# cisco/thor

Hardware: AMD Instinct MI355X
Metric: encoder Mpixels/s at fixed qp, bit-exact recon vs ref (higher is better)
Workload: dtype u8

## Files before the change

### include/thor_hip.h

```cpp
#ifndef THOR_HIP_H
#define THOR_HIP_H
#include <stddef.h>
#include <stdint.h>
#ifdef __cplusplus
extern "C" {
#endif

struct thor_encoder_info;
void encode_frame_lbd(struct thor_encoder_info* encoder_info);
void encode_frame_hbd(struct thor_encoder_info* encoder_info);

typedef struct thor_hip_params {
  int width, height, qp;
  int bitdepth, input_bitdepth;
  float frame_rate;
  float lambda_coeffI, lambda_coeffP;
  float early_skip_thr;
  int enable_tb_split, enable_pb_split, max_num_ref, HQperiod;
  int num_reorder_pics, interp_ref;
  int dqpP, dqpI;
  float mqpP;
  int intra_period, intra_rdo, encoder_speed;
  int deblocking, cdef, clpf, use_block_contexts, enable_bipred;
  int cfl_intra, cfl_inter;
  int dyadic_coding;
  float lambda_coeffB, lambda_coeffB0, lambda_coeffB1, lambda_coeffB2, lambda_coeffB3;
  int dqpB, dqpB0, dqpB1, dqpB2, dqpB3;
  float mqpB, mqpB0, mqpB1, mqpB2, mqpB3;
  int max_clpf_strength;
  int log2_sb_size;
} thor_hip_params;

typedef struct thor_hip_encoder thor_hip_encoder;

int thor_hip_params_from_config(thor_hip_params* p, const char* cfg_path);

int thor_hip_params_set(thor_hip_params* p, const char* name, const char* value);

int thor_hip_params_set_sb_size(thor_hip_params* p, int log2_sb_size);

int thor_hip_device_count(void);
thor_hip_encoder* thor_hip_open(const thor_hip_params* p, int num_streams, int device);
void thor_hip_close(thor_hip_encoder* e);

int thor_hip_begin_sequence(thor_hip_encoder* e, int stream, int skip, int num_frames, int file_frames);
int thor_hip_next_frame(thor_hip_encoder* e, int stream, int* display_index);

size_t thor_hip_frame_bytes(const thor_hip_encoder* e);
int thor_hip_stage_frame(thor_hip_encoder* e, int stream, int slot, const void* yuv);
int thor_hip_stage_frame_device(thor_hip_encoder* e, int stream, int slot, const void* dev_yuv);
int thor_hip_encode_staged(thor_hip_encoder* e, const int* slots);
typedef void (*thor_hip_frames_done_fn)(void* user, int first_stream, int num_streams);
int thor_hip_encode_staged_run(thor_hip_encoder* e, int nframes, thor_hip_frames_done_fn done, void* user);
int thor_hip_last_display_index(const thor_hip_encoder* e, int stream);
int thor_hip_encode_frame(thor_hip_encoder* e, const void* const* yuv_per_stream);

size_t thor_hip_stream_bytes(const thor_hip_encoder* e, int stream);
const uint8_t* thor_hip_stream_data(const thor_hip_encoder* e, int stream);
int thor_hip_get_recon(thor_hip_encoder* e, int stream, void* yuv_out);

enum { THOR_HIP_CHROMA_PLANAR = 0, THOR_HIP_CHROMA_UV = 1, THOR_HIP_CHROMA_VU = 2 };
typedef struct thor_hip_frame_layout {
  int    size;
  int    chroma;
  int    msb_aligned;
  int    pitch_y;
  int    pitch_c;
  size_t offset_u;
  size_t offset_v;
} thor_hip_frame_layout;
size_t thor_hip_layout_bytes(const thor_hip_encoder* e, const thor_hip_frame_layout* layout);
size_t thor_hip_layout_bytes_for(int width, int height, int input_bitdepth, const thor_hip_frame_layout* layout);
int thor_hip_stage_frame_layout(thor_hip_encoder* e, int stream, int slot, const void* frame, const thor_hip_frame_layout* layout, int on_device);
int thor_hip_get_recon_layout(thor_hip_encoder* e, int stream, void* frame, const thor_hip_frame_layout* layout, int on_device);

enum { THOR_HIP_RGB_RGBA = 0, THOR_HIP_RGB_BGRA = 1, THOR_HIP_RGB_ARGB = 2, THOR_HIP_RGB_ABGR = 3, THOR_HIP_RGB_RGB = 4, THOR_HIP_RGB_BGR = 5,
       THOR_HIP_RGB_PLANAR_RGB = 6 };
enum { THOR_HIP_MATRIX_BT601 = 0, THOR_HIP_MATRIX_BT709 = 1, THOR_HIP_MATRIX_BT2020 = 2 };
typedef struct thor_hip_rgb_format {
  int    size;
  int    order;
  int    depth;
  int    msb_aligned;
  int    matrix;
  int    full_range;
  int    chroma_site;
  int    pitch;
  size_t plane_stride;
} thor_hip_rgb_format;
size_t thor_hip_rgb_bytes(const thor_hip_encoder* e, const thor_hip_rgb_format* fmt);
size_t thor_hip_rgb_bytes_for(int width, int height, const thor_hip_rgb_format* fmt);
int thor_hip_stage_frame_rgb(thor_hip_encoder* e, int stream, int slot, const void* frame, const thor_hip_rgb_format* fmt, int on_device);
int thor_hip_get_recon_rgb(thor_hip_encoder* e, int stream, void* frame, const thor_hip_rgb_format* fmt, int on_device);

void thor_hip_kernel_time(thor_hip_encoder* e, double* sb_ms, long* sb_launches, double* filter_ms);
void thor_hip_kernel_time_reset(thor_hip_encoder* e);
void thor_hip_read_stats(thor_hip_encoder* e, unsigned long long out[4], int reset);
void thor_hip_set_frame_distortion(thor_hip_encoder* e, int on);
typedef struct thor_hip_frame_stats {
  int display_index;
  int frame_type;
  int qp;
  int num_bits;
  int num_ref;
  int ref_array[4];
  int ref_frame_num[4];
  int has_sse;
  unsigned long long sse[3];
  double psnr[3];
} thor_hip_frame_stats;
int thor_hip_frame_stats_count(const thor_hip_encoder* e, int stream);
int thor_hip_get_frame_stats(const thor_hip_encoder* e, int stream, int i, thor_hip_frame_stats* out);
int thor_hip_report(const thor_hip_encoder* e, int stream, char* buf, size_t n);
int thor_hip_stat_line(const thor_hip_encoder* e, int stream, int num_frames, char* buf, size_t n);

void thor_hip_read_prof(thor_hip_encoder* e, long long out[32]);

int thor_hip_sad_batch(const uint8_t* org, int w, int h, const uint8_t* ref_plane, int plane_w, int plane_h,
                       int rstride, int bx, int by, const int* cand, int n, uint32_t* out);
int thor_hip_interp_luma(const uint8_t* ref_plane, int plane_w, int plane_h, int rstride, int pad, int bx, int by,
                         int w, int h, const int16_t* mv, int n, int bipred, uint8_t* out);
int thor_hip_code_tu_batch(const uint8_t* org, const uint8_t* pred, int size, int qp, int coeff_type, int fast, int n,
                           int16_t* coefq, uint8_t* rec, int* cbp);
typedef struct thor_hip_cell {
  int16_t mv0x, mv0y, mv1x, mv1y;
  uint8_t mode, size, tbpb, cbp;
  int8_t ref0, ref1, dir;
  uint8_t pad;
} thor_hip_cell;
int thor_hip_deblock_frame(uint8_t* yuv, int width, int height, int qp, const thor_hip_cell* cells);

int thor_hip_sad_batch_hbd(const uint16_t* org, int w, int h, const uint16_t* ref_plane, int plane_w, int plane_h,
                           int rstride, int bx, int by, const int* cand, int n, uint32_t* out);
int thor_hip_interp_luma_hbd(const uint16_t* ref_plane, int plane_w, int plane_h, int rstride, int pad, int bx, int by,
                             int w, int h, const int16_t* mv, int n, int bipred, int bitdepth, uint16_t* out);
int thor_hip_code_tu_batch_hbd(const uint16_t* org, const uint16_t* pred, int size, int qp, int coeff_type, int fast, int n,
                               int bitdepth, int16_t* coefq, uint16_t* rec, int* cbp);
int thor_hip_deblock_frame_hbd(uint16_t* yuv, int width, int height, int qp, int bitdepth, const thor_hip_cell* cells);

int thor_hip_kat_intra(const void* plane, int width, int height, int stride, int bitdepth, int size, int tb_split, int n, const int* par,
                       const void* rblocks, void* out);
int thor_hip_kat_inter_yuv(const void* yuv, int width, int height, int bitdepth, int size, int n, const int* par, const int16_t* mv, void* out);
int thor_hip_kat_average(const void* a, const void* b, int size, int bitdepth, int n, void* out);
int thor_hip_kat_cfl(const void* y, void* uv, const void* ry, int n_luma, int bitdepth, int n);
int thor_hip_kat_cdef_dir(const void* blocks, int bitdepth, int n, int* dir, int* var);
int thor_hip_kat_cdef_filter(const void* plane, int width, int height, int stride, int bitdepth, int bsize, int n, const int* par, void* out);
int thor_hip_kat_cdef_frame(int n_jobs, const void* rec_yuv, const void* org_yuv, const uint8_t* mode, int width, int height, int bitdepth, const int* qp,
                            const int* speed, const int* cdef_bits, int8_t* dir, int* var, int* fb_compact, unsigned long long* mse, int* result, int* fb_sel, void* out_yuv);
int thor_hip_kat_clpf(const void* rec_yuv, const void* org_yuv, int width, int height, int bitdepth, int qp, const thor_hip_cell* cells,
                      const int* strength, int fb_log2, const uint8_t* fb_on, uint32_t* stats, void* out_yuv);
int thor_hip_kat_interpolate(const void* yuv0, const void* yuv1, int width, int height, int bitdepth, void* out_yuv);

int thor_hip_kat_motion_estimate(const void* cur, const void* ref, int width, int height, int bitdepth, int n, const int* par, const double* lambda,
                                 const int16_t* cand, int ncand_total, int* out);
int thor_hip_kat_motion_estimate_bi(const void* cur, const void* ref0, const void* ref1, int width, int height, int bitdepth, int n, const int* par,
                                    const double* lambda, const int16_t* cand, int* out, int16_t* list_out);
int thor_hip_kat_early_skip(const int* chroma, const void* org, const void* pred, const int* size, const int* qp, const float* thr, int bitdepth, int n, int* out);
int thor_hip_kat_block_ctx(const thor_hip_cell* cells, long long ncells, int cell_stride, int n, const int* par, int* out);
int thor_hip_kat_lds_block(void);
int thor_hip_kat_block_cost(int n, const int* par, const double* lambda, const void* org, const void* rec, long long nsamp, int bitdepth, unsigned long long* out);
int thor_hip_kat_intra_search(int n, const int* par, const void* plane, int width, int height, const void* org, long long nsamp, int bitdepth, int* out);
int thor_hip_kat_build_org8(int n, const int* par, const void* org, const void* pred, long long nsamp, int bitdepth, void* out_global, void* out_lds);
int thor_hip_kat_coeff_syntax(int n, const int* par, const int16_t* coef, int words, uint32_t* buf_single, uint32_t* buf_team, int* out);
int thor_hip_kat_block_syntax(int n, const int* par, const int16_t* pool, int npool, int words, uint32_t* buf_coop, uint32_t* buf_single, int* out);
int thor_hip_kat_gather_bits(int n, const uint32_t* src, int src_words, const int* src_off, const int* nbits, const long long* dst_bit, uint32_t* dst, int dst_words);

int thor_hip_frame_sse(const void* a, const void* b, int w, int h, int bitdepth, unsigned long long out[3]);
int thor_hip_kat_depth_up(const void* in, int w, int h, int bitdepth, int input_bitdepth, uint16_t* out);
int thor_hip_kat_depth_down(const uint16_t* in, int w, int h, int bitdepth, int input_bitdepth, void* out);
int thor_hip_frame_sse_depth(const void* a, const void* b, int w, int h, int bitdepth, int input_bitdepth, unsigned long long out[3]);
int thor_hip_kat_layout_in(const void* src, const thor_hip_frame_layout* layout, int w, int h, int input_bitdepth, int bitdepth, void* planar_out);
int thor_hip_kat_layout_out(const void* planar_in, const thor_hip_frame_layout* layout, int w, int h, int input_bitdepth, int bitdepth, void* dst);
int thor_hip_kat_rgb_in(const void* src, const thor_hip_rgb_format* fmt, int w, int h, int input_bitdepth, int bitdepth, void* planar_out);
int thor_hip_kat_rgb_out(const void* planar_in, const thor_hip_rgb_format* fmt, int w, int h, int input_bitdepth, int bitdepth, void* dst);

int thor_hip_superblock_kernel_info(int sample_bytes, int* num_regs, int* lds_bytes, int* private_bytes, int* workgroups_per_cu);
int thor_hip_superblock_kernel_in_use(void);

#ifdef __cplusplus
}
#endif
#endif
```

### thor_amd/binding.py

```python
import ctypes as C
import os
import subprocess
import numpy as np

REPO_ROOT = os.path.dirname(os.path.dirname(os.path.abspath(__file__)))
_LIB = None


def lib_path():
    return os.environ.get('THOR_HIP_LIB') or os.path.join(REPO_ROOT, 'thor_amd', 'libthor_hip.so')


HIPCC_FLAGS = ['--offload-arch=gfx950', '-O3', '-std=c++17', '-ffp-contract=off', '-fno-strict-aliasing', '-fPIC', '-pthread']
NATIVE_SOURCES = ['thor_hip.cpp', 'thor_hip_lat.cpp', 'thor_hip_wide.cpp', 'thor_hip_katbits.cpp']


def build_native(force=False):
    csrc = os.path.join(REPO_ROOT, 'thor_amd', 'csrc')
    out = os.path.join(REPO_ROOT, 'thor_amd', 'libthor_hip.so')
    hdrs = [os.path.join(csrc, f) for f in os.listdir(csrc)]
    hdrs += [os.path.join(REPO_ROOT, 'include', f) for f in os.listdir(os.path.join(REPO_ROOT, 'include'))]
    newest = max(os.path.getmtime(h) for h in hdrs)
    if force or not os.path.exists(out) or os.path.getmtime(out) < newest:
        hipcc = '/opt/rocm/bin/hipcc' if os.path.exists('/opt/rocm/bin/hipcc') else 'hipcc'
        import tempfile
        with tempfile.TemporaryDirectory() as d:
            objs = [os.path.join(d, f[:-4] + '.o') for f in NATIVE_SOURCES]
            procs = [subprocess.Popen([hipcc] + HIPCC_FLAGS + ['-c', '-o', o, os.path.join(csrc, f)]) for f, o in zip(NATIVE_SOURCES, objs)]
            rcs = [p.wait() for p in procs]
            if any(rcs):
                raise subprocess.CalledProcessError(max(rcs), 'hipcc -c ' + ' '.join(NATIVE_SOURCES))
            subprocess.check_call([hipcc, '--offload-arch=gfx950', '-shared', '-pthread', '-o', out] + objs)
    tool = os.path.join(REPO_ROOT, 'tools', 'thorenc_hip')
    tsrc = tool + '.c'
    if force or not os.path.exists(tool) or os.path.getmtime(tool) < os.path.getmtime(tsrc):
        subprocess.check_call(['gcc', '-O2', '-std=c99', '-D_POSIX_C_SOURCE=200809L', '-o', tool, tsrc,
                               '-L' + os.path.join(REPO_ROOT, 'thor_amd'), '-lthor_hip', '-Wl,-rpath,$ORIGIN/../thor_amd'])
    return out


class ThorParams(C.Structure):
    _fields_ = [('width', C.c_int), ('height', C.c_int), ('qp', C.c_int), ('bitdepth', C.c_int), ('input_bitdepth', C.c_int),
                ('frame_rate', C.c_float), ('lambda_coeffI', C.c_float), ('lambda_coeffP', C.c_float),
                ('early_skip_thr', C.c_float), ('enable_tb_split', C.c_int), ('enable_pb_split', C.c_int),
                ('max_num_ref', C.c_int), ('HQperiod', C.c_int), ('num_reorder_pics', C.c_int), ('interp_ref', C.c_int),
                ('dqpP', C.c_int), ('dqpI', C.c_int), ('mqpP', C.c_float), ('intra_period', C.c_int), ('intra_rdo', C.c_int),
                ('encoder_speed', C.c_int), ('deblocking', C.c_int), ('cdef', C.c_int), ('clpf', C.c_int),
                ('use_block_contexts', C.c_int), ('enable_bipred', C.c_int), ('cfl_intra', C.c_int), ('cfl_inter', C.c_int),
                ('dyadic_coding', C.c_int), ('lambda_coeffB', C.c_float), ('lambda_coeffB0', C.c_float), ('lambda_coeffB1', C.c_float),
                ('lambda_coeffB2', C.c_float), ('lambda_coeffB3', C.c_float), ('dqpB', C.c_int), ('dqpB0', C.c_int), ('dqpB1', C.c_int),
                ('dqpB2', C.c_int), ('dqpB3', C.c_int), ('mqpB', C.c_float), ('mqpB0', C.c_float), ('mqpB1', C.c_float),
                ('mqpB2', C.c_float), ('mqpB3', C.c_float), ('max_clpf_strength', C.c_int), ('log2_sb_size', C.c_int)]


FRAMES_DONE_FN = C.CFUNCTYPE(None, C.c_void_p, C.c_int, C.c_int)


class FrameStats(C.Structure):
    _fields_ = [('display_index', C.c_int), ('frame_type', C.c_int), ('qp', C.c_int), ('num_bits', C.c_int), ('num_ref', C.c_int),
                ('ref_array', C.c_int * 4), ('ref_frame_num', C.c_int * 4), ('has_sse', C.c_int), ('sse', C.c_ulonglong * 3),
                ('psnr', C.c_double * 3)]


CHROMA_PLANAR, CHROMA_UV, CHROMA_VU = 0, 1, 2


class FrameLayout(C.Structure):
    _fields_ = [('size', C.c_int), ('chroma', C.c_int), ('msb_aligned', C.c_int), ('pitch_y', C.c_int), ('pitch_c', C.c_int),
                ('offset_u', C.c_size_t), ('offset_v', C.c_size_t)]

    def __init__(self, chroma=CHROMA_PLANAR, msb_aligned=0, pitch_y=0, pitch_c=0, offset_u=0, offset_v=0):
        super().__init__(C.sizeof(FrameLayout), chroma, msb_aligned, pitch_y, pitch_c, offset_u, offset_v)

    @classmethod
    def planar(cls, pitch_y=0, pitch_c=0, offset_u=0, offset_v=0, msb_aligned=0):
        return cls(CHROMA_PLANAR, msb_aligned, pitch_y, pitch_c, offset_u, offset_v)

    @classmethod
    def nv12(cls, pitch=None, offset_uv=0):
        return cls(CHROMA_UV, 0, pitch or 0, pitch or 0, offset_uv)

    @classmethod
    def nv21(cls, pitch=None, offset_vu=0):
        return cls(CHROMA_VU, 0, pitch or 0, pitch or 0, offset_vu)

    @classmethod
    def p010(cls, pitch=None, offset_uv=0):
        return cls(CHROMA_UV, 1, pitch or 0, pitch or 0, offset_uv)


RGB_RGBA, RGB_BGRA, RGB_ARGB, RGB_ABGR, RGB_RGB, RGB_BGR, RGB_PLANAR = range(7)
MATRIX_BT601, MATRIX_BT709, MATRIX_BT2020 = 0, 1, 2


class RgbFormat(C.Structure):
    _fields_ = [('size', C.c_int), ('order', C.c_int), ('depth', C.c_int), ('msb_aligned', C.c_int), ('matrix', C.c_int), ('full_range', C.c_int),
                ('chroma_site', C.c_int), ('pitch', C.c_int), ('plane_stride', C.c_size_t)]

    def __init__(self, order=RGB_RGBA, depth=8, msb_aligned=0, matrix=MATRIX_BT709, full_range=0, chroma_site=1, pitch=0, plane_stride=0):
        super().__init__(C.sizeof(RgbFormat), order, depth, msb_aligned, matrix, full_range, chroma_site, pitch, plane_stride)

    @classmethod
    def rgba(cls, depth=8, matrix=MATRIX_BT709, full_range=0, chroma_site=1, pitch=0, msb_aligned=0):
        return cls(RGB_RGBA, depth, msb_aligned, matrix, full_range, chroma_site, pitch)

    @classmethod
    def bgra(cls, depth=8, matrix=MATRIX_BT709, full_range=0, chroma_site=1, pitch=0, msb_aligned=0):
        return cls(RGB_BGRA, depth, msb_aligned, matrix, full_range, chroma_site, pitch)

    @classmethod
    def rgb24(cls, depth=8, matrix=MATRIX_BT709, full_range=0, chroma_site=1, pitch=0, msb_aligned=0):
        return cls(RGB_RGB, depth, msb_aligned, matrix, full_range, chroma_site, pitch)

    @classmethod
    def bgr24(cls, depth=8, matrix=MATRIX_BT709, full_range=0, chroma_site=1, pitch=0, msb_aligned=0):
        return cls(RGB_BGR, depth, msb_aligned, matrix, full_range, chroma_site, pitch)

    @classmethod
    def planar(cls, depth=8, matrix=MATRIX_BT709, full_range=0, chroma_site=1, pitch=0, msb_aligned=0, plane_stride=0):
        return cls(RGB_PLANAR, depth, msb_aligned, matrix, full_range, chroma_site, pitch, plane_stride)


def lib():
    global _LIB
    if _LIB is None:
        p = lib_path()
        if not os.path.exists(p):
            raise RuntimeError(f'{p} is missing: run __graft_entry__.build() (hipcc --offload-arch=gfx950); there is no CPU path')
        L = C.CDLL(p)
        L.thor_hip_open.restype = C.c_void_p
        L.thor_hip_open.argtypes = [C.POINTER(ThorParams), C.c_int, C.c_int]
        L.thor_hip_close.argtypes = [C.c_void_p]
        L.thor_hip_begin_sequence.argtypes = [C.c_void_p, C.c_int, C.c_int, C.c_int, C.c_int]
        L.thor_hip_next_frame.argtypes = [C.c_void_p, C.c_int, C.POINTER(C.c_int)]
        L.thor_hip_stage_frame.argtypes = [C.c_void_p, C.c_int, C.c_int, C.c_void_p]
        L.thor_hip_stage_frame_device.argtypes = [C.c_void_p, C.c_int, C.c_int, C.c_void_p]
        L.thor_hip_encode_staged.argtypes = [C.c_void_p, C.POINTER(C.c_int)]
        L.thor_hip_encode_frame.argtypes = [C.c_void_p, C.POINTER(C.c_void_p)]
        L.thor_hip_encode_staged_run.argtypes = [C.c_void_p, C.c_int, FRAMES_DONE_FN, C.c_void_p]
        L.thor_hip_last_display_index.argtypes = [C.c_void_p, C.c_int]
        L.thor_hip_stream_bytes.restype = C.c_size_t
        L.thor_hip_stream_bytes.argtypes = [C.c_void_p, C.c_int]
        L.thor_hip_stream_data.restype = C.c_void_p
        L.thor_hip_stream_data.argtypes = [C.c_void_p, C.c_int]
        L.thor_hip_get_recon.argtypes = [C.c_void_p, C.c_int, C.c_void_p]
        L.thor_hip_frame_bytes.restype = C.c_size_t
        L.thor_hip_frame_bytes.argtypes = [C.c_void_p]
        L.thor_hip_kernel_time.argtypes = [C.c_void_p, C.POINTER(C.c_double), C.POINTER(C.c_long), C.POINTER(C.c_double)]
        L.thor_hip_kernel_time_reset.argtypes = [C.c_void_p]
        L.thor_hip_read_stats.argtypes = [C.c_void_p, C.POINTER(C.c_ulonglong), C.c_int]
        L.thor_hip_deblock_frame.argtypes = [C.c_void_p, C.c_int, C.c_int, C.c_int, C.c_void_p]
        L.thor_hip_deblock_frame_hbd.argtypes = [C.c_void_p, C.c_int, C.c_int, C.c_int, C.c_int, C.c_void_p]
        L.thor_hip_set_frame_distortion.argtypes = [C.c_void_p, C.c_int]
        L.thor_hip_frame_stats_count.argtypes = [C.c_void_p, C.c_int]
        L.thor_hip_get_frame_stats.argtypes = [C.c_void_p, C.c_int, C.c_int, C.POINTER(FrameStats)]
        L.thor_hip_report.argtypes = [C.c_void_p, C.c_int, C.c_char_p, C.c_size_t]
        L.thor_hip_stat_line.argtypes = [C.c_void_p, C.c_int, C.c_int, C.c_char_p, C.c_size_t]
        L.thor_hip_frame_sse.argtypes = [C.c_void_p, C.c_void_p, C.c_int, C.c_int, C.c_int, C.POINTER(C.c_ulonglong)]
        L.thor_hip_kat_depth_up.argtypes = [C.c_void_p, C.c_int, C.c_int, C.c_int, C.c_int, C.c_void_p]
        L.thor_hip_kat_depth_down.argtypes = [C.c_void_p, C.c_int, C.c_int, C.c_int, C.c_int, C.c_void_p]
        L.thor_hip_frame_sse_depth.argtypes = [C.c_void_p, C.c_void_p, C.c_int, C.c_int, C.c_int, C.c_int, C.POINTER(C.c_ulonglong)]
        LP = C.POINTER(FrameLayout)
        L.thor_hip_layout_bytes.restype = C.c_size_t
        L.thor_hip_layout_bytes.argtypes = [C.c_void_p, LP]
        L.thor_hip_layout_bytes_for.restype = C.c_size_t
        L.thor_hip_layout_bytes_for.argtypes = [C.c_int, C.c_int, C.c_int, LP]
        L.thor_hip_stage_frame_layout.argtypes = [C.c_void_p, C.c_int, C.c_int, C.c_void_p, LP, C.c_int]
        L.thor_hip_get_recon_layout.argtypes = [C.c_void_p, C.c_int, C.c_void_p, LP, C.c_int]
        L.thor_hip_kat_layout_in.argtypes = [C.c_void_p, LP, C.c_int, C.c_int, C.c_int, C.c_int, C.c_void_p]
        L.thor_hip_kat_layout_out.argtypes = [C.c_void_p, LP, C.c_int, C.c_int, C.c_int, C.c_int, C.c_void_p]
        RP = C.POINTER(RgbFormat)
        L.thor_hip_rgb_bytes.restype = C.c_size_t
        L.thor_hip_rgb_bytes.argtypes = [C.c_void_p, RP]
        L.thor_hip_rgb_bytes_for.restype = C.c_size_t
        L.thor_hip_rgb_bytes_for.argtypes = [C.c_int, C.c_int, RP]
        L.thor_hip_stage_frame_rgb.argtypes = [C.c_void_p, C.c_int, C.c_int, C.c_void_p, RP, C.c_int]
        L.thor_hip_get_recon_rgb.argtypes = [C.c_void_p, C.c_int, C.c_void_p, RP, C.c_int]
        L.thor_hip_kat_rgb_in.argtypes = [C.c_void_p, RP, C.c_int, C.c_int, C.c_int, C.c_int, C.c_void_p]
        L.thor_hip_kat_rgb_out.argtypes = [C.c_void_p, RP, C.c_int, C.c_int, C.c_int, C.c_int, C.c_void_p]
        L.thor_hip_params_from_config.argtypes = [C.POINTER(ThorParams), C.c_char_p]
        L.thor_hip_params_set.argtypes = [C.POINTER(ThorParams), C.c_char_p, C.c_char_p]
        L.thor_hip_params_set_sb_size.argtypes = [C.POINTER(ThorParams), C.c_int]
        _LIB = L
    return _LIB


def load_config(cfg_path=None, **overrides):
    p = ThorParams()
    rc = lib().thor_hip_params_from_config(C.byref(p), cfg_path.encode() if cfg_path else None)
    if rc:
        raise ValueError(f'{cfg_path}: unknown or unsupported option (rc={rc}); this path rejects what it cannot encode bit-exactly')
    for k, v in overrides.items():
        if k == 'log2_sb_size':
            rc = lib().thor_hip_params_set_sb_size(C.byref(p), int(v))
        else:
            rc = lib().thor_hip_params_set(C.byref(p), ('-' + k).encode(), str(v).encode())
        if rc:
            raise ValueError(f'option -{k} {v}: ' + {1: 'unknown', 2: 'not implemented by this path', 3: 'front-end option, not an encoder parameter'}.get(rc, f'rc={rc}'))
    return p


class Encoder:

    def __init__(self, params, num_streams=1, device=0):
        self.p = params
        self.S = num_streams
        self.h = lib().thor_hip_open(C.byref(params), num_streams, device)
        if not self.h:
            raise RuntimeError('thor_hip_open failed (unsupported parameters?)')
        self.dtype = _pix(params.input_bitdepth)
        self.sample_bytes = self.dtype().itemsize
        self.frame_bytes = lib().thor_hip_frame_bytes(self.h)

    def close(self):
        if self.h:
            lib().thor_hip_close(self.h)
            self.h = None

    def layout_bytes(self, layout):
        n = lib().thor_hip_layout_bytes(self.h, C.byref(layout))
        if not n:
            raise ValueError('frame layout refused (pitch below the row, pitch or offset no multiple of the sample size, msb_aligned with 8-bit input ...)')
        return n

    def stage(self, stream, slot, frame, layout=None):
        frame = np.ascontiguousarray(frame).view(np.uint8)
        if layout is not None:
            assert frame.size >= self.layout_bytes(layout)
            rc = lib().thor_hip_stage_frame_layout(self.h, stream, slot, frame.ctypes.data_as(C.c_void_p), C.byref(layout), 0)
            if rc:
                raise RuntimeError(f'thor_hip_stage_frame_layout rc={rc}')
            return
        assert frame.size == self.frame_bytes
        rc = lib().thor_hip_stage_frame(self.h, stream, slot, frame.ctypes.data_as(C.c_void_p))
        if rc:
            raise RuntimeError(f'thor_hip_stage_frame rc={rc}')

    def stage_device(self, stream, slot, dev_ptr, layout=None):
        if layout is not None:
            rc = lib().thor_hip_stage_frame_layout(self.h, stream, slot, C.c_void_p(dev_ptr), C.byref(layout), 1)
            if rc:
                raise RuntimeError(f'thor_hip_stage_frame_layout rc={rc}')
            return
        rc = lib().thor_hip_stage_frame_device(self.h, stream, slot, C.c_void_p(dev_ptr))
        if rc:
            raise RuntimeError(f'thor_hip_stage_frame_device rc={rc}')

    def rgb_bytes(self, fmt):
        n = lib().thor_hip_rgb_bytes(self.h, C.byref(fmt))
        if not n:
            raise ValueError('RGB format refused (unknown order / depth / matrix, msb_aligned with depth 8 or 16, pitch below the row ...)')
        return n

    def stage_rgb(self, stream, slot, array, fmt):
        frame = np.ascontiguousarray(array).view(np.uint8).reshape(-1)
        assert frame.size >= self.rgb_bytes(fmt)
        rc = lib().thor_hip_stage_frame_rgb(self.h, stream, slot, frame.ctypes.data_as(C.c_void_p), C.byref(fmt), 0)
        if rc:
            raise RuntimeError(f'thor_hip_stage_frame_rgb rc={rc}')

    def stage_rgb_device(self, stream, slot, dev_ptr, fmt):
        rc = lib().thor_hip_stage_frame_rgb(self.h, stream, slot, C.c_void_p(dev_ptr), C.byref(fmt), 1)
        if rc:
            raise RuntimeError(f'thor_hip_stage_frame_rgb rc={rc}')

    def recon_rgb(self, stream, fmt):
        out = np.zeros(self.rgb_bytes(fmt), dtype=np.uint8)
        rc = lib().thor_hip_get_recon_rgb(self.h, stream, out.ctypes.data_as(C.c_void_p), C.byref(fmt), 0)
        if rc:
            raise RuntimeError(f'thor_hip_get_recon_rgb rc={rc}')
        return out

    def recon_rgb_device(self, stream, dev_ptr, fmt):
        rc = lib().thor_hip_get_recon_rgb(self.h, stream, C.c_void_p(dev_ptr), C.byref(fmt), 1)
        if rc:
            raise RuntimeError(f'thor_hip_get_recon_rgb rc={rc}')

    def begin_sequence(self, stream, skip, num_frames, file_frames):
        rc = lib().thor_hip_begin_sequence(self.h, stream, skip, num_frames, file_frames)
        if rc:
            raise RuntimeError(f'thor_hip_begin_sequence rc={rc}')

    def next_frame(self, stream):
        d = C.c_int()
        return d.value if lib().thor_hip_next_frame(self.h, stream, C.byref(d)) else None

    def encode_run(self, nframes, on_done=None):
        err = []

        def _cb(_user, first, count):
            if on_done is not None and not err:
                try:
                    on_done(first, count)
                except BaseException as e:
                    err.append(e)
        cb = FRAMES_DONE_FN(_cb)
        rc = lib().thor_hip_encode_staged_run(self.h, nframes, cb, None)
        if err:
            raise err[0]
        if rc:
            raise RuntimeError(f'thor_hip_encode_staged_run rc={rc}')

    def last_display_index(self, stream):
        return lib().thor_hip_last_display_index(self.h, stream)

    def encode_clips(self, clips, want_recon=True, skips=None, file_frames=None, staggered=False):
        n = len(clips[0])
        for s in range(self.S):
            for f in range(n):
                self.stage(s, f, clips[s][f])
            sk = skips[s] if skips else 0
            self.begin_sequence(s, sk, n, file_frames if file_frames else sk + n)
        recs = [[None] * n for _ in range(self.S)]
        if staggered:
            def done(first, count):
                if want_recon:
                    for s in range(first, first + count):
                        recs[s][self.last_display_index(s)] = self.recon(s)
            self.encode_run(n, done)
            return [self.bitstream(s) for s in range(self.S)], recs
        while True:
            idx = [self.next_frame(s) for s in range(self.S)]
            if idx[0] is None:
                break
            self.encode_staged(idx)
            if want_recon:
                for s in range(self.S):
                    recs[s][idx[s]] = self.recon(s)
        return [self.bitstream(s) for s in range(self.S)], recs

    def encode_staged(self, slots):
        arr = (C.c_int * self.S)(*slots)
        rc = lib().thor_hip_encode_staged(self.h, arr)
        if rc:
            raise RuntimeError(f'thor_hip_encode_staged rc={rc}')

    def bitstream(self, stream):
        n = lib().thor_hip_stream_bytes(self.h, stream)
        return C.string_at(lib().thor_hip_stream_data(self.h, stream), n)

    def recon(self, stream, layout=None):
        if layout is not None:
            out = np.zeros(self.layout_bytes(layout), dtype=np.uint8)
            rc = lib().thor_hip_get_recon_layout(self.h, stream, out.ctypes.data_as(C.c_void_p), C.byref(layout), 0)
            if rc:
                raise RuntimeError(f'thor_hip_get_recon_layout rc={rc}')
            return out
        out = np.empty(self.frame_bytes, dtype=np.uint8)
        rc = lib().thor_hip_get_recon(self.h, stream, out.ctypes.data_as(C.c_void_p))
        if rc:
            raise RuntimeError(f'thor_hip_get_recon rc={rc}')
        return out

    def recon_device(self, stream, dev_ptr, layout):
        rc = lib().thor_hip_get_recon_layout(self.h, stream, C.c_void_p(dev_ptr), C.byref(layout), 1)
        if rc:
            raise RuntimeError(f'thor_hip_get_recon_layout rc={rc}')

    def recon_into(self, stream, ptr):
        rc = lib().thor_hip_get_recon(self.h, stream, C.c_void_p(ptr))
        if rc:
            raise RuntimeError(f'thor_hip_get_recon rc={rc}')

    def kernel_time(self):
        a, b, c = C.c_double(), C.c_long(), C.c_double()
        lib().thor_hip_kernel_time(self.h, C.byref(a), C.byref(b), C.byref(c))
        return a.value, b.value, c.value

    def kernel_time_reset(self):
        lib().thor_hip_kernel_time_reset(self.h)
        self.stats(reset=True)

    def stats(self, reset=False):
        a = (C.c_ulonglong * 4)()
        lib().thor_hip_read_stats(self.h, a, 1 if reset else 0)
        px, sb = max(int(a[3]), 1), max(int(a[2]), 1)
        return {'early_skip_pixel_fraction': round(int(a[0]) / px, 4), 'early_skip_sb128_fraction': round(int(a[1]) / sb, 4),
                'inter_superblocks': int(a[2]), 'inter_luma_pixels': int(a[3])}

    def set_frame_distortion(self, on=True):
        lib().thor_hip_set_frame_distortion(self.h, 1 if on else 0)

    def frame_stats(self, stream):
        L, out, f = lib(), [], FrameStats()
        for i in range(L.thor_hip_frame_stats_count(self.h, stream)):
            if L.thor_hip_get_frame_stats(self.h, stream, i, C.byref(f)):
                raise RuntimeError('thor_hip_get_frame_stats failed')
            nr = f.num_ref
            out.append({'display_index': f.display_index, 'type': 'IPB'[f.frame_type], 'qp': f.qp, 'num_bits': f.num_bits,
                        'ref_array': list(f.ref_array)[:nr], 'ref_frame_num': list(f.ref_frame_num)[:nr], 'has_sse': bool(f.has_sse),
                        'sse': [int(v) for v in f.sse], 'psnr': [float(v) for v in f.psnr]})
        return out

    def report(self, stream):
        n = lib().thor_hip_report(self.h, stream, None, 0)
        if n < 0:
            raise ValueError('bad stream')
        buf = C.create_string_buffer(n + 1)
        lib().thor_hip_report(self.h, stream, buf, n + 1)
        return buf.value.decode()

    def __enter__(self):
        return self

    def __exit__(self, *a):
        self.close()


def _vp(a):
    return a.ctypes.data_as(C.c_void_p)


def _pix(bitdepth):
    return np.uint16 if bitdepth > 8 else np.uint8


def sad_batch(org, ref_plane, bx, by, cand, bitdepth=8):
    T = _pix(bitdepth)
    org = np.ascontiguousarray(org, dtype=T); ref_plane = np.ascontiguousarray(ref_plane, dtype=T)
    cand = np.ascontiguousarray(cand, dtype=np.int32)
    out = np.zeros(len(cand), dtype=np.uint32)
    fn = lib().thor_hip_sad_batch_hbd if bitdepth > 8 else lib().thor_hip_sad_batch
    rc = fn(_vp(org), org.shape[1], org.shape[0], _vp(ref_plane), ref_plane.shape[1], ref_plane.shape[0], ref_plane.shape[1], bx, by,
            _vp(cand), len(cand), _vp(out))
    if rc:
        raise RuntimeError(f'thor_hip_sad_batch rc={rc}')
    return out


def interp_luma(ref_padded, pad, pic_w, pic_h, bx, by, w, h, mvs, bipred, bitdepth=8):
    T = _pix(bitdepth)
    ref_padded = np.ascontiguousarray(ref_padded, dtype=T); mvs = np.ascontiguousarray(mvs, dtype=np.int16)
    out = np.zeros((len(mvs), h, w), dtype=T)
    if bitdepth > 8:
        rc = lib().thor_hip_interp_luma_hbd(_vp(ref_padded), pic_w, pic_h, ref_padded.shape[1], pad, bx, by, w, h, _vp(mvs), len(mvs),
                                            bipred, bitdepth, _vp(out))
    else:
        rc = lib().thor_hip_interp_luma(_vp(ref_padded), pic_w, pic_h, ref_padded.shape[1], pad, bx, by, w, h, _vp(mvs), len(mvs),
                                        bipred, _vp(out))
    if rc:
        raise RuntimeError(f'thor_hip_interp_luma rc={rc}')
    return out


def code_tu_batch(org, pred, qp, coeff_type, fast, bitdepth=8):
    T = _pix(bitdepth)
    org = np.ascontiguousarray(org, dtype=T); pred = np.ascontiguousarray(pred, dtype=T)
    n, size = org.shape[0], org.shape[1]
    q = min(size, 16)
    coefq = np.zeros((n, q, q), dtype=np.int16); rec = np.zeros_like(org); cbp = np.zeros(n, dtype=np.int32)
    if bitdepth > 8:
        rc = lib().thor_hip_code_tu_batch_hbd(_vp(org), _vp(pred), size, qp, coeff_type, fast, n, bitdepth, _vp(coefq), _vp(rec), _vp(cbp))
    else:
        rc = lib().thor_hip_code_tu_batch(_vp(org), _vp(pred), size, qp, coeff_type, fast, n, _vp(coefq), _vp(rec), _vp(cbp))
    if rc:
        raise RuntimeError(f'thor_hip_code_tu_batch rc={rc}')
    return coefq, rec, cbp


def deblock_frame(yuv, width, height, qp, cells, bitdepth=8):
    yuv = np.ascontiguousarray(yuv, dtype=_pix(bitdepth)).copy()
    cells = np.ascontiguousarray(cells, dtype=np.uint8)
    assert yuv.size == width * height * 3 // 2 and cells.size == (width // 4) * (height // 4) * 16
    if bitdepth > 8:
        rc = lib().thor_hip_deblock_frame_hbd(_vp(yuv), width, height, qp, bitdepth, _vp(cells))
    else:
        rc = lib().thor_hip_deblock_frame(_vp(yuv), width, height, qp, _vp(cells))
    if rc:
        raise RuntimeError(f'thor_hip_deblock_frame rc={rc}')
    return yuv


def _kat(name, *args):
    fn = getattr(lib(), name)
    fn.restype = C.c_int
    rc = fn(*args)
    if rc:
        raise RuntimeError(f'{name} rc={rc}')


def kat_intra(plane, size, par, bitdepth=8, rblocks=None):
    T = _pix(bitdepth)
    plane = np.ascontiguousarray(plane, dtype=T); par = np.ascontiguousarray(par, dtype=np.int32)
    n = len(par)
    out = np.zeros((n, size, size), dtype=T)
    rb = np.ascontiguousarray(rblocks, dtype=T) if rblocks is not None else None
    _kat('thor_hip_kat_intra', _vp(plane), plane.shape[1], plane.shape[0], plane.shape[1], bitdepth, size, 1 if rb is not None else 0, n, _vp(par),
         _vp(rb) if rb is not None else None, _vp(out))
    return out


def kat_inter_yuv(yuv, width, height, size, par, mvs, bitdepth=8):
    T = _pix(bitdepth)
    yuv = np.ascontiguousarray(yuv, dtype=T); par = np.ascontiguousarray(par, dtype=np.int32); mvs = np.ascontiguousarray(mvs, dtype=np.int16)
    n = len(par)
    out = np.zeros((n, size * size * 3 // 2), dtype=T)
    _kat('thor_hip_kat_inter_yuv', _vp(yuv), width, height, bitdepth, size, n, _vp(par), _vp(mvs), _vp(out))
    return out


def kat_average(a, b, size, bitdepth=8):
    T = _pix(bitdepth)
    a = np.ascontiguousarray(a, dtype=T); b = np.ascontiguousarray(b, dtype=T)
    out = np.zeros_like(a)
    _kat('thor_hip_kat_average', _vp(a), _vp(b), size, bitdepth, len(a), _vp(out))
    return out


def kat_cfl(y, uv, ry, n_luma, bitdepth=8):
    T = _pix(bitdepth)
    y = np.ascontiguousarray(y, dtype=T); ry = np.ascontiguousarray(ry, dtype=T); uv = np.array(uv, dtype=T, order='C')
    _kat('thor_hip_kat_cfl', _vp(y), _vp(uv), _vp(ry), n_luma, bitdepth, len(y))
    return uv


def kat_cdef_dir(blocks, bitdepth=8):
    T = _pix(bitdepth)
    blocks = np.ascontiguousarray(blocks, dtype=T)
    n = len(blocks)
    d = np.zeros(n, dtype=np.int32); v = np.zeros(n, dtype=np.int32)
    _kat('thor_hip_kat_cdef_dir', _vp(blocks), bitdepth, n, _vp(d), _vp(v))
    return d, v


def kat_cdef_filter(plane, bsize, par, bitdepth=8):
    T = _pix(bitdepth)
    plane = np.ascontiguousarray(plane, dtype=T); par = np.ascontiguousarray(par, dtype=np.int32)
    out = np.zeros((len(par), bsize, bsize), dtype=T)
    _kat('thor_hip_kat_cdef_filter', _vp(plane), plane.shape[1], plane.shape[0], plane.shape[1], bitdepth, bsize, len(par), _vp(par), _vp(out))
    return out


def kat_cdef_frame(rec, org, mode, width, height, qp, speed, cdef_bits, bitdepth=8):
    T = _pix(bitdepth)
    rec = np.ascontiguousarray(rec, dtype=T); org = np.ascontiguousarray(org, dtype=T); mode = np.ascontiguousarray(mode, dtype=np.uint8)
    S = len(rec)
    nfb = ((width + 63) // 64) * ((height + 63) // 64)
    qp, speed, cdef_bits = (np.ascontiguousarray(a, dtype=np.int32) for a in (qp, speed, cdef_bits))
    assert rec.shape == org.shape == (S, width * height * 3 // 2) and mode.shape == (S, height // 4, width // 4) and len(qp) == len(speed) == len(cdef_bits) == S
    d = np.zeros((S, height // 8, width // 8), dtype=np.int8); v = np.zeros((S, height // 8, width // 8), dtype=np.int32)
    fbc = np.zeros((S, nfb), dtype=np.int32); fbs = np.zeros((S, nfb), dtype=np.int32)
    mse = np.zeros((S, 2, nfb, 64), dtype=np.uint64); res = np.zeros((S, 34), dtype=np.int32)
    out = np.zeros_like(rec)
    _kat('thor_hip_kat_cdef_frame', S, _vp(rec), _vp(org), _vp(mode), width, height, bitdepth, _vp(qp), _vp(speed), _vp(cdef_bits), _vp(d), _vp(v), _vp(fbc), _vp(mse), _vp(res), _vp(fbs),
         _vp(out))
    return dict(dir=d, var=v, fb_compact=fbc, fb_sel=fbs, mse=mse, nb_bits=res[:, 0], strengths=res[:, 1:9], uv_strengths=res[:, 9:17], sb_count=res[:, 17], out=out)


def kat_clpf(rec, org, width, height, qp, cells, strength, fb_log2, fb_on, bitdepth=8):
    T = _pix(bitdepth)
    rec = np.ascontiguousarray(rec, dtype=T); org = np.ascontiguousarray(org, dtype=T)
    cells = np.ascontiguousarray(cells, dtype=np.uint8); fb_on = np.ascontiguousarray(fb_on, dtype=np.uint8)
    st = np.ascontiguousarray(strength, dtype=np.int32)
    nblk = (width // 8) * (height // 8) + 2 * (width // 16) * (height // 16)
    stats = np.zeros((nblk, 4), dtype=np.uint32)
    out = np.zeros_like(rec)
    _kat('thor_hip_kat_clpf', _vp(rec), _vp(org), width, height, bitdepth, qp, _vp(cells), _vp(st), fb_log2, _vp(fb_on), _vp(stats), _vp(out))
    return stats, out


def kat_interpolate(yuv0, yuv1, width, height, bitdepth=8):
    T = _pix(bitdepth)
    a = np.ascontiguousarray(yuv0, dtype=T); b = np.ascontiguousarray(yuv1, dtype=T)
    out = np.zeros_like(a)
    _kat('thor_hip_kat_interpolate', _vp(a), _vp(b), width, height, bitdepth, _vp(out))
    return out


def kat_motion_estimate(cur, ref, par, lam, cand, bitdepth=8):
    T = _pix(bitdepth)
    cur = np.ascontiguousarray(cur, dtype=T); ref = np.ascontiguousarray(ref, dtype=T)
    par = np.ascontiguousarray(par, dtype=np.int32); lam = np.ascontiguousarray(lam, dtype=np.float64); cand = np.ascontiguousarray(cand, dtype=np.int16).reshape(-1, 2)
    assert cur.shape == ref.shape and par.shape[1] == 17 and len(lam) == len(par)
    out = np.full((len(par), 3), -1, dtype=np.int32)
    _kat('thor_hip_kat_motion_estimate', _vp(cur), _vp(ref), cur.shape[1], cur.shape[0], bitdepth, len(par), _vp(par), _vp(lam), _vp(cand), len(cand), _vp(out))
    return out


def kat_motion_estimate_bi(cur, ref0, ref1, par, lam, cand, bitdepth=8):
    T = _pix(bitdepth)
    cur, ref0, ref1 = (np.ascontiguousarray(a, dtype=T) for a in (cur, ref0, ref1))
    par = np.ascontiguousarray(par, dtype=np.int32); lam = np.ascontiguousarray(lam, dtype=np.float64); cand = np.ascontiguousarray(cand, dtype=np.int16)
    assert cur.shape == ref0.shape == ref1.shape and par.shape[1] == 17 and len(lam) == len(par) and cand.size == 12 * len(par)
    out = np.full((len(par), 3), -1, dtype=np.int32)
    lists = np.zeros((len(par), 6, 2), dtype=np.int16)
    _kat('thor_hip_kat_motion_estimate_bi', _vp(cur), _vp(ref0), _vp(ref1), cur.shape[1], cur.shape[0], bitdepth, len(par), _vp(par), _vp(lam), _vp(cand), _vp(out), _vp(lists))
    return out, lists


def kat_early_skip(chroma, org, pred, size, qp, thr, bitdepth=8):
    T = _pix(bitdepth)
    org = np.ascontiguousarray(org, dtype=T); pred = np.ascontiguousarray(pred, dtype=T)
    chroma, size, qp = (np.ascontiguousarray(a, dtype=np.int32) for a in (chroma, size, qp))
    thr = np.ascontiguousarray(thr, dtype=np.float32)
    n = len(org)
    assert org.shape == pred.shape == (n, 32, 32) and len(chroma) == len(size) == len(qp) == len(thr) == n
    out = np.full(n, -1, dtype=np.int32)
    _kat('thor_hip_kat_early_skip', _vp(chroma), _vp(org), _vp(pred), _vp(size), _vp(qp), _vp(thr), bitdepth, n, _vp(out))
    return out


def kat_block_ctx(cells, cell_stride, par):
    cells = np.ascontiguousarray(cells, dtype=np.uint8); par = np.ascontiguousarray(par, dtype=np.int32)
    assert cells.ndim == 2 and cells.shape[1] == 16 and par.ndim == 2 and par.shape[1] == 6
    out = np.full((len(par), 23), -77, dtype=np.int32)
    _kat('thor_hip_kat_block_ctx', _vp(cells), C.c_longlong(len(cells)), cell_stride, len(par), _vp(par), _vp(out))
    return out


def kat_lds_block():
    fn = lib().thor_hip_kat_lds_block
    fn.restype = C.c_int
    return fn()


def kat_block_cost(par, lam, org, rec, bitdepth=8):
    T = _pix(bitdepth)
    org = np.ascontiguousarray(org, dtype=T).ravel(); rec = np.ascontiguousarray(rec, dtype=T).ravel()
    par = np.ascontiguousarray(par, dtype=np.int32); lam = np.ascontiguousarray(lam, dtype=np.float64)
    assert par.ndim == 2 and par.shape[1] == 7 and len(lam) == len(par) and len(org) == len(rec)
    out = np.zeros((len(par), 4), dtype=np.uint64)
    _kat('thor_hip_kat_block_cost', len(par), _vp(par), _vp(lam), _vp(org), _vp(rec), C.c_longlong(len(org)), bitdepth, _vp(out))
    return out


def kat_intra_search(par, plane, org, bitdepth=8):
    T = _pix(bitdepth)
    plane = np.ascontiguousarray(plane, dtype=T); org = np.ascontiguousarray(org, dtype=T).ravel()
    par = np.ascontiguousarray(par, dtype=np.int32)
    assert plane.ndim == 2 and par.ndim == 2 and par.shape[1] == 6
    out = np.full((len(par), 2), -77, dtype=np.int32)
    _kat('thor_hip_kat_intra_search', len(par), _vp(par), _vp(plane), plane.shape[1], plane.shape[0], _vp(org), C.c_longlong(len(org)), bitdepth, _vp(out))
    return out


def kat_build_org8(par, org, pred, bitdepth=8, fill=0):
    T = _pix(bitdepth)
    org = np.ascontiguousarray(org, dtype=T).ravel(); pred = np.ascontiguousarray(pred, dtype=T).ravel()
    par = np.ascontiguousarray(par, dtype=np.int32)
    assert par.ndim == 2 and par.shape[1] == 4 and len(org) == len(pred)
    og = np.full(len(org), fill, dtype=T); ol = np.full(len(org), fill, dtype=T)
    _kat('thor_hip_kat_build_org8', len(par), _vp(par), _vp(org), _vp(pred), C.c_longlong(len(org)), bitdepth, _vp(og), _vp(ol))
    return og, ol


def kat_coeff_syntax(par, coef, words, buf_single, buf_team):
    par = np.ascontiguousarray(par, dtype=np.int32); coef = np.ascontiguousarray(coef, dtype=np.int16)
    n = len(par)
    b1 = np.ascontiguousarray(buf_single, dtype=np.uint32).copy(); bt = np.ascontiguousarray(buf_team, dtype=np.uint32).copy()
    assert par.shape == (n, 4) and coef.shape == (n, 256) and b1.shape == (n, words) and bt.shape == (n, words)
    out = np.zeros((n, 6), dtype=np.int32)
    _kat('thor_hip_kat_coeff_syntax', n, _vp(par), _vp(coef), words, _vp(b1), _vp(bt), _vp(out))
    return out, b1, bt


def kat_block_syntax(par, pool, words, fill=0):
    par = np.ascontiguousarray(par, dtype=np.int32); pool = np.ascontiguousarray(pool, dtype=np.int16)
    n = len(par)
    assert par.shape == (n, 57) and pool.ndim == 2 and pool.shape[1] == 256
    bc = np.full((n, words), fill, dtype=np.uint32); b1 = np.full((n, words), fill, dtype=np.uint32)
    out = np.zeros((n, 10), dtype=np.int32)
    _kat('thor_hip_kat_block_syntax', n, _vp(par), _vp(pool), len(pool), words, _vp(bc), _vp(b1), _vp(out))
    return out, bc, b1


def kat_gather_bits(src, src_off, nbits, dst_bit, dst_words):
    src = np.ascontiguousarray(src, dtype=np.uint32); src_off = np.ascontiguousarray(src_off, dtype=np.int32)
    nbits = np.ascontiguousarray(nbits, dtype=np.int32); dst_bit = np.ascontiguousarray(dst_bit, dtype=np.int64)
    dst = np.zeros(dst_words, dtype=np.uint32)
    _kat('thor_hip_kat_gather_bits', len(nbits), _vp(src), len(src), _vp(src_off), _vp(nbits), _vp(dst_bit), _vp(dst), dst_words)
    return dst


def frame_sse(a, b, width, height, bitdepth=8):
    T = _pix(bitdepth)
    a = np.ascontiguousarray(a, dtype=T).reshape(-1); b = np.ascontiguousarray(b, dtype=T).reshape(-1)
    if a.size != width * height * 3 // 2 or b.size != a.size:
        raise ValueError('frame size does not match width x height 4:2:0')
    out = (C.c_ulonglong * 3)()
    rc = lib().thor_hip_frame_sse(_vp(a), _vp(b), width, height, bitdepth, out)
    if rc:
        raise RuntimeError(f'thor_hip_frame_sse returned {rc}')
    return [int(v) for v in out]


def _depth_frame(a, depth, width, height):
    a = np.ascontiguousarray(a, dtype=_pix(depth)).reshape(-1)
    if a.size != width * height * 3 // 2:
        raise ValueError('frame size does not match width x height 4:2:0')
    return a


def kat_depth_up(frame, width, height, bitdepth, input_bitdepth):
    a = _depth_frame(frame, input_bitdepth, width, height)
    out = np.zeros(a.size, dtype=np.uint16)
    _kat('thor_hip_kat_depth_up', _vp(a), width, height, bitdepth, input_bitdepth, _vp(out))
    return out


def kat_depth_down(frame, width, height, bitdepth, input_bitdepth):
    a = _depth_frame(frame, 16, width, height)
    out = np.zeros(a.size, dtype=_pix(input_bitdepth))
    _kat('thor_hip_kat_depth_down', _vp(a), width, height, bitdepth, input_bitdepth, _vp(out))
    return out


def frame_sse_depth(a, b, width, height, bitdepth, input_bitdepth):
    T = 16 if bitdepth > input_bitdepth else bitdepth
    a = _depth_frame(a, T, width, height); b = _depth_frame(b, T, width, height)
    out = (C.c_ulonglong * 3)()
    _kat('thor_hip_frame_sse_depth', _vp(a), _vp(b), width, height, bitdepth, input_bitdepth, out)
    return [int(v) for v in out]


def layout_bytes(layout, width, height, input_bitdepth):
    return lib().thor_hip_layout_bytes_for(width, height, input_bitdepth, C.byref(layout))


def kat_layout_in(src, layout, width, height, input_bitdepth, bitdepth):
    assert src.dtype == np.uint8 and src.flags.c_contiguous and src.size >= layout_bytes(layout, width, height, input_bitdepth) > 0
    out = np.zeros(width * height * 3 // 2, dtype=_pix(bitdepth))
    _kat('thor_hip_kat_layout_in', _vp(src), C.byref(layout), width, height, input_bitdepth, bitdepth, _vp(out))
    return out


def kat_layout_out(planar, layout, width, height, input_bitdepth, bitdepth, dst):
    a = _depth_frame(planar, bitdepth, width, height)
    assert dst.dtype == np.uint8 and dst.flags.c_contiguous and dst.size == layout_bytes(layout, width, height, input_bitdepth) + 64 > 64
    _kat('thor_hip_kat_layout_out', _vp(a), C.byref(layout), width, height, input_bitdepth, bitdepth, _vp(dst))
    return dst


def rgb_bytes(fmt, width, height):
    return lib().thor_hip_rgb_bytes_for(width, height, C.byref(fmt))


def kat_rgb_in(src, fmt, width, height, input_bitdepth, bitdepth):
    assert src.dtype == np.uint8 and src.flags.c_contiguous and src.size >= rgb_bytes(fmt, width, height) > 0
    out = np.zeros(width * height * 3 // 2, dtype=_pix(bitdepth))
    _kat('thor_hip_kat_rgb_in', _vp(src), C.byref(fmt), width, height, input_bitdepth, bitdepth, _vp(out))
    return out


def kat_rgb_out(planar, fmt, width, height, input_bitdepth, bitdepth, dst):
    a = _depth_frame(planar, bitdepth, width, height)
    assert dst.dtype == np.uint8 and dst.flags.c_contiguous and dst.size == rgb_bytes(fmt, width, height) + 64 > 64
    _kat('thor_hip_kat_rgb_out', _vp(a), C.byref(fmt), width, height, input_bitdepth, bitdepth, _vp(dst))
    return dst
```

### thor_amd/csrc/hip_kat_block.h

```cpp
#pragma once
#include "tk_kat_block.h"
namespace tk {
__global__ __launch_bounds__(64) void k_kat_block_ctx(const DbCell* cells, int cs, const int* par, int* out) {
  const int it = (int)blockIdx.x;
  int o[kKatCtxOut];
  kat_ctx_item(cells, cs, par + kKatCtxPar * it, o);
  if (threadIdx.x == 0)
    for (int k = 0; k < kKatCtxOut; k++) out[(size_t)kKatCtxOut * it + k] = o[k];
}
template <typename PIX>
__global__ __launch_bounds__(kWgThreads, (sizeof(PIX) == 1 ? (int)kOcc : 2)) void k_kat_block_cost(const int* par, const double* lam, const int* lay, const PIX* orgp, const PIX* recp,
                                                                                                   int bitdepth, unsigned char* big, unsigned long long* out) {
  __shared__ FrameJob<PIX> sJ;
  __shared__ WgShared sh;
  __shared__ SmallWs<PIX> sws;
  __shared__ TeamWs<PIX> s_view;
  const int lane = (int)threadIdx.x, it = (int)blockIdx.x;
  const Team t = mk_team(lane, 64, sh.tabs.izz);
  const int* q = par + kKatCostPar * it;
  const int size = __builtin_amdgcn_readfirstlane(q[0]), bw = __builtin_amdgcn_readfirstlane(q[1]), bh = __builtin_amdgcn_readfirstlane(q[2]);
  const int nbits = __builtin_amdgcn_readfirstlane(q[3]), off = __builtin_amdgcn_readfirstlane(q[4]), sy = __builtin_amdgcn_readfirstlane(q[6]);
  const int n = size * size, c = n >> 2, sc = size >> 1;
  const PIX* gy = orgp + lay[3 * it];
  const PIX* gu = orgp + lay[3 * it + 1];
  const PIX* gv = orgp + lay[3 * it + 2];
  const PIX* ry = recp + off;
  const int lds_blk = size <= kLdsBlk;
  TeamWs<PIX> w = make_ws(&sws, &sh, (BigWs<PIX>*)big);
  ws_select(&w, size);
  if (lds_blk) {
    PIX* ob = (PIX*)sh.org_raw;
    for (int k = lane; k < bw * bh; k += 64) ob[(k / bw) * size + k % bw] = gy[(k / bw) * sy + k % bw];
    for (int k = lane; k < (bw >> 1) * (bh >> 1); k += 64) {
      const int i = k / (bw >> 1), j = k % (bw >> 1);
      ob[n + i * sc + j] = gu[i * (sy >> 1) + j];
      ob[n + c + i * sc + j] = gv[i * (sy >> 1) + j];
    }
    for (int k = lane; k < n; k += 64) w.rec_y[k] = ry[k];
    for (int k = lane; k < c; k += 64) { w.rec_u[k] = ry[n + k]; w.rec_v[k] = ry[n + c + k]; }
    w.org_y = ob; w.org_u = ob + n; w.org_v = ob + n + c; w.org_sy = size; w.org_sc = sc;
  } else {
    w.rec_y = const_cast<PIX*>(ry); w.rec_u = const_cast<PIX*>(ry) + n; w.rec_v = const_cast<PIX*>(ry) + n + c;
    w.org_y = gy; w.org_u = gu; w.org_v = gv; w.org_sy = sy; w.org_sc = sy >> 1;
  }
  lds_st(&s_view, w);
  if (lane == 0) {
    sJ.cfg.bitdepth = bitdepth;
    sh.stack[0].size = size; sh.stack[0].bw = bw; sh.stack[0].bh = bh;
  }
  __syncthreads();
  WsP<PIX> ws = ldsc(&s_view);
  JobR<PIX> J = *ldsc(&sJ);
  const double lambda = lam[it];
  const unsigned long long ssd_g = ssd_total(t, ssd_part<SP_GLOBAL>(t, gy, sy, ry, size, bw, bh));
  unsigned long long ssd_l = ~0ull, cost, cost_y;
  if (lds_blk) {
    ssd_l = ssd_total(t, ssd_part<SP_LDS>(t, w.org_y, size, w.rec_y, size, bw, bh));
    cost = rd_cost<PIX, SP_LDS>(t, J, ws, sh.stack[0], nbits, lambda);
    cost_y = rd_cost<PIX, SP_LDS>(t, J, ws, sh.stack[0], nbits, lambda, (long long)ssd_l);
  } else {
    cost = rd_cost<PIX, SP_GLOBAL>(t, J, ws, sh.stack[0], nbits, lambda);
    cost_y = rd_cost<PIX, SP_GLOBAL>(t, J, ws, sh.stack[0], nbits, lambda, (long long)ssd_g);
  }
  if (lane == 0) {
    unsigned long long* o = out + (size_t)kKatCostOut * it;
    o[0] = ssd_g; o[1] = ssd_l; o[2] = cost; o[3] = cost_y;
  }
}
template <typename PIX>
__global__ __launch_bounds__(kWgThreads, (sizeof(PIX) == 1 ? (int)kOcc : 2)) void k_kat_intra_search(const int* par, const int* slot, const PIX* plane, int fw, int fh, int bitdepth,
                                                                                                     const PIX* orgp, unsigned char* big, int* out) {
  __shared__ FrameJob<PIX> sJ;
  __shared__ WgShared sh;
  __shared__ SmallWs<PIX> sws;
  __shared__ TeamWs<PIX> s_view;
  const int lane = (int)threadIdx.x, it = (int)blockIdx.x;
  const Team t = mk_team(lane, 64, sh.tabs.izz);
  const int* q = par + kKatIntraPar * it;
  const int ypos = __builtin_amdgcn_readfirstlane(q[0]), xpos = __builtin_amdgcn_readfirstlane(q[1]), size = __builtin_amdgcn_readfirstlane(q[2]);
  const int sb = __builtin_amdgcn_readfirstlane(q[3]), nm = __builtin_amdgcn_readfirstlane(q[4]), off = __builtin_amdgcn_readfirstlane(q[5]);
  const PIX* go = orgp + off;
  const int lds_blk = size <= kLdsBlk;
  TeamWs<PIX> w = make_ws(&sws, &sh, (BigWs<PIX>*)big + __builtin_amdgcn_readfirstlane(slot[it]));
  ws_select(&w, size);
  if (lds_blk) {
    PIX* ob = (PIX*)sh.org_raw;
    for (int k = lane; k < size * size; k += 64) ob[k] = go[k];
    w.org_y = ob;
  } else {
    w.org_y = go;
  }
  w.org_sy = size;
  lds_st(&s_view, w);
  if (lane == 0) {
    sJ.cfg.width = fw; sJ.cfg.height = fh; sJ.cfg.bitdepth = bitdepth; sJ.cfg.sb_shift = sb == kMaxSb ? 0 : 1;
    sJ.rec.y = const_cast<PIX*>(plane); sJ.rec.sy = fw;
    sh.stack[0].size = size; sh.stack[0].ypos = ypos; sh.stack[0].xpos = xpos; sh.stack[0].bw = size; sh.stack[0].bh = size;
  }
  __syncthreads();
  WsP<PIX> ws = ldsc(&s_view);
  JobR<PIX> J = *ldsc(&sJ);
  int mode = -1;
  const unsigned sad = lds_blk ? intra_sad_search<PIX, SP_LDS>(t, J, ws, sh.stack[0], nm, &mode) : intra_sad_search<PIX, SP_GLOBAL>(t, J, ws, sh.stack[0], nm, &mode);
  if (lane == 0) { out[kKatIntraOut * it] = mode; out[kKatIntraOut * it + 1] = (int)sad; }
}
template <typename PIX>
__global__ __launch_bounds__(64) void k_kat_build_org8(const int* par, const int* lay, const PIX* orgp, const PIX* predp, int bitdepth, unsigned char* big, PIX* outg, PIX* outl) {
  __shared__ WgShared sh;
  __shared__ SmallWs<PIX> sws;
  const int lane = (int)threadIdx.x, it = (int)blockIdx.x;
  const Team t = mk_team(lane, 64, sh.tabs.izz);
  const int* q = par + kKatOrg8Par * it;
  const int size = __builtin_amdgcn_readfirstlane(q[0]), off = __builtin_amdgcn_readfirstlane(q[1]), sy = __builtin_amdgcn_readfirstlane(q[3]);
  const int n = size * size;
  const PIX* gy = orgp + lay[it];
  const PIX* gp = predp + off;
  build_org8<PIX, SP_GLOBAL>(t, outg + off, gy, sy, gp, size, bitdepth);
  if (size <= kLdsBlk) {
    TeamWs<PIX> w = make_ws(&sws, &sh, (BigWs<PIX>*)big);
    ws_select(&w, size);
    PIX* ob = (PIX*)sh.org_raw;
    for (int k = lane; k < n; k += 64) { ob[k] = gy[(k / size) * sy + k % size]; w.pred_y[k] = gp[k]; }
    __syncthreads();
    build_org8<PIX, SP_LDS>(t, w.org8, ob, size, w.pred_y, size, bitdepth);
    __syncthreads();
    for (int k = lane; k < n; k += 64) outl[off + k] = w.org8[k];
  }
}
}

namespace {
template <typename PIX>
int kat_intra_search(int n, const int* par, const PIX* plane, int fw, int fh, const PIX* org, long long nsamp, int bitdepth, int* out) {
  if (n <= 0 || n > 4096 || !par || !plane || !org || !out || fw < 8 || fh < 8 || fw > 4096 || fh > 4096 || fw % 8 || fh % 8 || nsamp <= 0 || nsamp > (1ll << 30)) return 1;
  std::vector<int> slot(n, 0);
  int nbig = 0;
  for (int i = 0; i < n; i++) {
    if (int r = kat_intra_check(par + kKatIntraPar * i, fw, fh, nsamp)) return r;
    if (par[kKatIntraPar * i + 2] > kLdsBlk) slot[i] = nbig++;
  }
  if (!ensure_init_any()) return 3;
  DevBuf<int> d_par((size_t)kKatIntraPar * n, par), d_slot(n, slot.data()), d_o((size_t)kKatIntraOut * n);
  DevBuf<PIX> d_plane((size_t)fw * fh, plane), d_org((size_t)nsamp, org);
  DevBuf<unsigned char> d_big(sizeof(BigWs<PIX>) * (size_t)(nbig > 0 ? nbig : 1));
  hipLaunchKernelGGL(k_kat_intra_search<PIX>, dim3(n), dim3(64), 0, g_stream, d_par, d_slot, d_plane, fw, fh, bitdepth, d_org, d_big, d_o);
  HIPCHECK(hipGetLastError());
  backend::d2h(out, d_o, (size_t)kKatIntraOut * n * 4);
  return 0;
}
template <typename PIX>
int kat_build_org8(int n, const int* par, const PIX* org, const PIX* pred, long long nsamp, int bitdepth, PIX* outg, PIX* outl) {
  const int S = (int)sizeof(PIX);
  if (n <= 0 || !par || !org || !pred || !outg || !outl || nsamp <= 0 || nsamp > (1ll << 28)) return 1;
  for (int i = 0; i < n; i++)
    if (int r = kat_org8_check(par + kKatOrg8Par * i, nsamp, S)) return r;
  std::vector<PIX> planes;
  std::vector<int> lay(n);
  for (int i = 0; i < n; i++) {
    const int* q = par + kKatOrg8Par * i;
    const int size = q[0], sk = q[2] / S, st = q[3];
    const size_t base = (planes.size() * S + 15) / 16 * 16 / S;
    planes.resize(base + sk + (size_t)(size - 1) * st + size, (PIX)0);
    lay[i] = (int)(base + sk);
    for (int r = 0; r < size; r++) memcpy(&planes[base + sk + (size_t)r * st], org + q[1] + (size_t)r * size, (size_t)size * S);
  }
  if (planes.size() > (1u << 30)) return 2;
  if (!ensure_init_any()) return 3;
  DevBuf<int> d_par((size_t)kKatOrg8Par * n, par), d_lay(n, lay.data());
  DevBuf<PIX> d_org(planes.size(), planes.data()), d_pred((size_t)nsamp, pred), d_g((size_t)nsamp, outg), d_l((size_t)nsamp, outl);
  DevBuf<unsigned char> d_big(sizeof(BigWs<PIX>));
  hipLaunchKernelGGL(k_kat_build_org8<PIX>, dim3(n), dim3(64), 0, g_stream, d_par, d_lay, d_org, d_pred, bitdepth, d_big, d_g, d_l);
  HIPCHECK(hipGetLastError());
  backend::d2h(outg, d_g, (size_t)nsamp * S);
  backend::d2h(outl, d_l, (size_t)nsamp * S);
  return 0;
}
template <typename PIX>
int kat_block_cost(int n, const int* par, const double* lambda, const PIX* org, const PIX* rec, long long nsamp, int bitdepth, unsigned long long* out) {
  const int S = (int)sizeof(PIX);
  if (n <= 0 || !par || !lambda || !org || !rec || !out || nsamp <= 0 || nsamp > (1ll << 30)) return 1;
  for (int i = 0; i < n; i++)
    if (int r = kat_cost_check(par + kKatCostPar * i, lambda[i], nsamp, S)) return r;
  std::vector<PIX> planes;
  std::vector<int> lay((size_t)3 * n);
  for (int i = 0; i < n; i++) {
    const int* q = par + kKatCostPar * i;
    const int size = q[0], bw = q[1], bh = q[2], skew = q[5], sy = q[6];
    const PIX* src = org + q[4];
    for (int pl = 0; pl < 3; pl++) {
      const int w = pl ? bw / 2 : bw, h = pl ? bh / 2 : bh, st = pl ? sy / 2 : sy, cst = pl ? size / 2 : size;
      const int sk = (pl ? skew / 2 : skew) / S;
      const PIX* s = src + (pl == 0 ? 0 : pl == 1 ? size * size : size * size * 5 / 4);
      const size_t base = (planes.size() * S + 15) / 16 * 16 / S;
      planes.resize(base + sk + (size_t)(h - 1) * st + w, (PIX)0);
      lay[3 * i + pl] = (int)(base + sk);
      for (int r = 0; r < h; r++) memcpy(&planes[base + sk + (size_t)r * st], s + (size_t)r * cst, (size_t)w * S);
    }
  }
  if (planes.size() > (1u << 30)) return 2;
  if (!ensure_init_any()) return 3;
  DevBuf<int> d_par((size_t)kKatCostPar * n, par), d_lay((size_t)3 * n, lay.data());
  DevBuf<double> d_lam(n, lambda);
  DevBuf<PIX> d_org(planes.size(), planes.data()), d_rec((size_t)nsamp, rec);
  DevBuf<unsigned char> d_big(sizeof(BigWs<PIX>));
  DevBuf<unsigned long long> d_o((size_t)kKatCostOut * n);
  hipLaunchKernelGGL(k_kat_block_cost<PIX>, dim3(n), dim3(64), 0, g_stream, d_par, d_lam, d_lay, d_org, d_rec, bitdepth, d_big, d_o);
  HIPCHECK(hipGetLastError());
  backend::d2h(out, d_o, (size_t)kKatCostOut * n * 8);
  return 0;
}
}

extern "C" int thor_hip_kat_block_ctx(const thor_hip_cell* cells, long long ncells, int cell_stride, int n, const int* par, int* out) {
  static_assert(sizeof(thor_hip_cell) == sizeof(DbCell), "thor_hip_cell must mirror tk::DbCell");
  if (!cells || !par || !out || n <= 0 || ncells <= 0 || ncells > (1ll << 26) || cell_stride < 2 || cell_stride > 2048) return 1;
  for (int i = 0; i < n; i++) {
    if (par[kKatCtxPar * i + 3] != 4 * cell_stride) return 1;
    if (int r = kat_ctx_check(par + kKatCtxPar * i, ncells)) return r;
  }
  if (!ensure_init_any()) return 3;
  const size_t pad = (size_t)cell_stride + 1;
  DevBuf<DbCell> d_cells(pad + (size_t)ncells);
  backend::h2d(d_cells.get() + pad, cells, (size_t)ncells * sizeof(DbCell));
  DevBuf<int> d_par((size_t)kKatCtxPar * n, par), d_o((size_t)kKatCtxOut * n);
  hipLaunchKernelGGL(k_kat_block_ctx, dim3(n), dim3(64), 0, g_stream, d_cells.get() + pad, cell_stride, d_par, d_o);
  HIPCHECK(hipGetLastError());
  backend::d2h(out, d_o, (size_t)kKatCtxOut * n * 4);
  return 0;
}
extern "C" int thor_hip_kat_lds_block(void) { return kLdsBlk; }
extern "C" int thor_hip_kat_block_cost(int n, const int* par, const double* lambda, const void* org, const void* rec, long long nsamp, int bitdepth, unsigned long long* out) {
  KAT_BD(kat_block_cost<uint8_t>(n, par, lambda, (const uint8_t*)org, (const uint8_t*)rec, nsamp, 8, out),
         kat_block_cost<uint16_t>(n, par, lambda, (const uint16_t*)org, (const uint16_t*)rec, nsamp, bitdepth, out));
}
extern "C" int thor_hip_kat_intra_search(int n, const int* par, const void* plane, int width, int height, const void* org, long long nsamp, int bitdepth, int* out) {
  KAT_BD(kat_intra_search<uint8_t>(n, par, (const uint8_t*)plane, width, height, (const uint8_t*)org, nsamp, 8, out),
         kat_intra_search<uint16_t>(n, par, (const uint16_t*)plane, width, height, (const uint16_t*)org, nsamp, bitdepth, out));
}
extern "C" int thor_hip_kat_build_org8(int n, const int* par, const void* org, const void* pred, long long nsamp, int bitdepth, void* out_global, void* out_lds) {
  KAT_BD(kat_build_org8<uint8_t>(n, par, (const uint8_t*)org, (const uint8_t*)pred, nsamp, 8, (uint8_t*)out_global, (uint8_t*)out_lds),
         kat_build_org8<uint16_t>(n, par, (const uint16_t*)org, (const uint16_t*)pred, nsamp, bitdepth, (uint16_t*)out_global, (uint16_t*)out_lds));
}
```

### thor_amd/csrc/tk_block_queue.h

```cpp
#pragma once
#include "tk_block_md.h"

namespace tk {
TK_DEV BlkParam blank_param() {
  BlkParam p;
  p.mode = M_SKIP; p.intra_mode = 0; p.skip_idx = 0; p.pb_part = P_NONE; p.ref0 = p.ref1 = 0; p.dir = 0;
  p.tb_param = 0; p.tb_split = 0; p.cbp_y = p.cbp_u = p.cbp_v = 0;
  for (int i = 0; i < 4; i++) { p.mv0[i] = mk_mv(0, 0); p.mv1[i] = mk_mv(0, 0); }
  return p;
}

template <typename PIX, int SP>
TK_DEV void snapshot_trial(const Team t, WsP<PIX> ws, int size, const BlkParam& p) {
  BigWs<PIX>* g = ws->big;
  const int sc = size >> 1;
  copy_block<SP_GLOBAL, SP>(t, g->best_y, size, ws->rec_y, size, size, size);
  copy_block<SP_GLOBAL, SP>(t, g->best_u, sc, ws->rec_u, sc, sc, sc);
  copy_block<SP_GLOBAL, SP>(t, g->best_v, sc, ws->rec_v, sc, sc, sc);
  if (TKU(p.cbp_y) | TKU(p.cbp_u) | TKU(p.cbp_v)) {
    const int tbs = TKU(p.tb_split);
    const int qy = tbs ? tmin(size >> 1, (int)kMaxQuant) : tmin(size, (int)kMaxQuant);
    const int ny = (tbs ? 4 : 1) * qy * qy;
    const int csplit = tbs && sc > 4;
    const int qc = csplit ? tmin(sc >> 1, (int)kMaxQuant) : tmin(sc, (int)kMaxQuant);
    const int nc = (csplit ? 4 : 1) * qc * qc;
    const int16_t *cy = ws->coef_y, *cu = ws->coef_u, *cv = ws->coef_v;
    TK_GLOBAL int16_t* dy = gptr(g->best_cy);
    TK_GLOBAL int16_t* du = gptr(g->best_cu);
    TK_GLOBAL int16_t* dv = gptr(g->best_cv);
    for (int k = t.rank; k < ny; k += t.size) dy[k] = cy[k];
    for (int k = t.rank; k < nc; k += t.size) { du[k] = cu[k]; dv[k] = cv[k]; }
  }
}

template <typename PIX> struct MdCtx {
  Wg wg;
  WgShared* sh;
  Node* nd;
  unsigned long long mykey;
};

template <typename PIX, int SP>
TK_DEV int par_trial(const Team t, JobR<PIX> J, WsP<PIX> ws, MdCtx<PIX>& M, BlkParam& p, unsigned order, int reuse_pred) {
  int untouched = 0;
  const unsigned cost = rdo_trial<PIX, SP>(t, J, ws, *M.nd, p, J.lambda, reuse_pred, 0xffffffffu, &M.sh->bestkey, order, nullptr, &untouched);
  if (cost == (unsigned)kCostInit) return !untouched;
  const unsigned long long key = ((unsigned long long)cost << 32) | order;
  if (key < M.mykey) {
    M.mykey = key;
    if (t.rank == 0) {
      lds_st(&M.sh->wbest[M.wg.wave], normalize_best(*M.nd, p));
      *ldsc(&M.sh->wkey[M.wg.wave]) = key;
      wg_min64(&M.sh->bestkey, key);
    }
    snapshot_trial<PIX, SP>(t, ws, tk_uniform(ldsc(M.nd)->size), p);
    t.sync();
  }
  return 1;
}

TK_DEV void wg_wait_at_least(const Team t, int* p, int at_least) {
  const unsigned long long w0 = wg_clock();
  for (unsigned spins = 1;; spins++) {
    const int d = wg_load_acquire(p);
    if (team_bcast0(t, d) >= at_least) break;
    if ((spins & 1023u) == 0 && tk_uniform64(wg_clock() - w0) > (unsigned long long)kWgWaitLimit) wg_wait_failed();
    wg_pause();
  }
}
template <typename PIX, int SP>
TK_DEVNI int md_bijoint_telescope(const Team t, JobR<PIX> J, WsP<PIX> ws, MdCtx<PIX>& M) {
  const auto& c = J.cfg;
  WgShared* const sh_ = tk_uniform_ptr(M.sh);
  int mine = 0;
  if (t.rank == 0) mine = wg_cas(&sh_->bj_state, 0, 1);
  if (!team_bcast0(t, mine)) return 0;
  const NodePos nd = node_pos(M.nd);
  const int ri0 = J.interp_ref ? 1 : 0, ri1 = J.interp_ref ? 2 : 1;
  const Plane3<PIX> f0 = lds_ld(&J.ref[ri0]);
  const Plane3<PIX> f1 = lds_ld(&J.ref[ri1]);
  MeArgs a;
  a.cb_size = nd.size; a.ostride = ws->org_sy; a.width = nd.size; a.height = nd.size; a.rstride = f0.sy; a.sign = 0;
  a.fwidth = c.width; a.fheight = c.height; a.xpos = nd.xpos; a.ypos = nd.ypos; a.enable_bipred = 1;
  a.bitdepth = c.bitdepth; a.lam = J.sqrt_lambda; a.speed = c.encoder_speed; a.pu_x = nd.xpos; a.pu_y = nd.ypos;
  mv_t mvb = mk_mv(0, 0);
  const mv_t ctr = lds_ld(&sh_->ref_mv[ri0][0][0]);
  const unsigned sad = motion_estimate_bi<PIX, SP>(t, ws->mep, ws->org_y, f0.y + nd.ypos * f0.sy + nd.xpos, f1.y + nd.ypos * f1.sy + nd.xpos, a, ctr,
                                                   lds_ld(&sh_->mvp), ri0, &mvb, 1);
  t.sync();
  if (t.rank == 0) {
    *ldsc(&sh_->bj_sad) = sad;
    lds_st(&sh_->bj_mv, mvb);
    wg_store_release(&sh_->bj_state, 2);
  }
  t.sync();
  return 1;
}

template <typename PIX, int SP>
TK_DEVNI void md_item_bipred(const Team t, JobR<PIX> J, WsP<PIX> ws, MdCtx<PIX>& M) {
  const auto& c = J.cfg;
  Node& nd_ = *M.nd;
  const NodePos nd = node_pos(&nd_);
  const int size = nd.size;
  const int max_tb = c.enable_tb_split == 1 ? 2 : 1;
  const mv_t mvp = lds_ld(&M.sh->mvp);
  mv_t mv_center[kMaxRefs];
  for (int r = 0; r < kMaxRefs; r++) mv_center[r] = lds_ld(&M.sh->mv_center[r]);
  int r0, r1;
  mv_t a0[4], a1[4];
  search_bipred<PIX, SP>(t, J, ws, nd_, 0, mv_center, mvp, &r0, &r1, a0, a1);
  BlkParam p = blank_param();
  p.mode = M_BIPRED; p.pb_part = P_NONE;
  p.ref0 = (int8_t)r0; p.ref1 = (int8_t)r1;
  for (int i = 0; i < 4; i++) { p.mv0[i] = a0[i]; p.mv1[i] = a1[i]; }
  for (int tb = 0, have_pred = 0; tb <= max_tb - 1; tb++) {
    p.tb_param = (int8_t)tb;
    have_pred |= par_trial<PIX, SP>(t, J, ws, M, p, 54u + (unsigned)tb, have_pred);
  }
  if (J.frame_type == F_B) {
    const int ri0 = J.interp_ref ? 1 : 0, ri1 = J.interp_ref ? 2 : 1;
    const Plane3<PIX> f0 = lds_ld(&J.ref[ri0]);
    const Plane3<PIX> f1 = lds_ld(&J.ref[ri1]);
    const PIX* oy = ws->org_y;
    MeArgs a;
    a.cb_size = size; a.ostride = ws->org_sy; a.width = size; a.height = size; a.rstride = f0.sy; a.sign = 0;
    a.fwidth = c.width; a.fheight = c.height; a.xpos = nd.xpos; a.ypos = nd.ypos; a.enable_bipred = 1;
    a.bitdepth = c.bitdepth; a.lam = J.sqrt_lambda; a.speed = c.encoder_speed; a.pu_x = nd.xpos; a.pu_y = nd.ypos;
    WgShared* const sh_ = tk_uniform_ptr(M.sh);
    if (!md_bijoint_telescope<PIX, SP>(t, J, ws, M)) wg_wait_at_least(t, &sh_->bj_state, 2);
    mv_t mvb = lds_ld(&sh_->bj_mv);
    const unsigned sad0 = (unsigned)tk_uniform((int)*ldsc(&sh_->bj_sad));
    motion_estimate_bi<PIX, SP>(t, ws->mep, oy, f0.y + nd.ypos * f0.sy + nd.xpos, f1.y + nd.ypos * f1.sy + nd.xpos, a, mv_center[ri0], mvp, ri0, &mvb, 2, sad0);
    p.mode = M_BIPRED; p.pb_part = P_NONE;
    p.ref0 = (int8_t)ri0; p.ref1 = (int8_t)ri1;
    for (int i = 0; i < 4; i++) { p.mv0[i] = mvb; p.mv1[i] = mvb; }
    p.tb_param = 0;
    par_trial<PIX, SP>(t, J, ws, M, p, 56u, 0);
  }
}

template <typename PIX, int SP>
TK_DEVNI void md_item_ref(const Team t, JobR<PIX> J, WsP<PIX> ws, MdCtx<PIX>& M, int r) {
  const auto& c = J.cfg;
  const NodePos nd = node_pos(M.nd);
  const int size = nd.size;
  const int max_pb = c.enable_pb_split ? 4 : 1;
  const mv_t mvp = lds_ld(&M.sh->mvp);
  const PIX* oy = ws->org_y;
  if (t.rank == 0) add_mvcand(ws->mep, r, mvp);
  t.sync();
  mv_t mv_center = mvp;
  if (t.rank == 0) ldsc(ws->mep)->cwin_valid = 0;
  t.sync();
  for (int part = 0; part < max_pb; part++) {
    mv_t mv_all[4];
    search_inter<PIX, SP>(t, J, ws, nd.ypos, nd.xpos, size, oy, ws->org_sy, r, mv_center, mvp, mv_all, part, J.sign[r]);
    add_cands4(t, ws, r, mv_all);
    if (part == 0) {
      mv_center = mv_all[0];
      if (max_pb > 1) {
        const Plane3<PIX> rp = lds_ld(&J.ref[r]);
        me_stage_cb_window<PIX>(t, ws->mep, rp.y + nd.ypos * rp.sy + nd.xpos, rp.sy, nd.xpos, nd.ypos, size, mv_center, J.sign[r], c.width, c.height, r);
      }
    }
    if (t.rank == 0) {
      for (int i = 0; i < 4; i++) lds_st(&M.sh->ref_mv[r][part][i], mv_all[i]);
      if (part == max_pb - 1) lds_st(&M.sh->mv_center[r], mv_center);
      wg_fetch_add(&M.sh->parts_done[r], 1);
    }
    t.sync();
  }
  if (t.rank == 0) ldsc(ws->mep)->cwin_valid = 0;
  t.sync();
}

template <typename PIX, int SP>
TK_DEVNI void md_item_trial(const Team t, JobR<PIX> J, WsP<PIX> ws, MdCtx<PIX>& M, int r, int part) {
  const auto& c = J.cfg;
  const int max_tb = c.enable_tb_split == 1 ? 2 : 1;
  r = tk_uniform(r); part = tk_uniform(part);
  WgShared* const sh_ = tk_uniform_ptr(M.sh);
  TK_PROFMD_MARK(pwt_);
  wg_wait_at_least(t, &sh_->parts_done[r], part + 1);
  if (TK_PROFMD_ON(2)) TK_PROFMD_ACC(ws, 20, pwt_);
  mv_t mv_all[4][4];
  for (int q = 0; q <= part; q++)
    for (int i = 0; i < 4; i++) mv_all[q][i] = lds_ld(&sh_->ref_mv[r][q][i]);
  int dup = 0;
  for (int q = 0; q < part && c.enable_pb_split; q++) {
    int eq = 1;
    for (int i = 0; i < 4; i++) eq = eq && mv_all[q][i].x == mv_all[part][i].x && mv_all[q][i].y == mv_all[part][i].y;
    dup = dup || eq;
  }
  if (tk_uniform(dup)) return;
  BlkParam p = blank_param();
  p.mode = M_INTER;
  p.ref0 = p.ref1 = (int8_t)r;
  p.pb_part = (int8_t)part;
  for (int i = 0; i < 4; i++) { p.mv0[i] = mv_all[part][i]; p.mv1[i] = mv_all[part][i]; }
  for (int tb = -1, have_pred = 0; tb <= max_tb - 1; tb++) {
    p.tb_param = (int8_t)tb;
    have_pred |= par_trial<PIX, SP>(t, J, ws, M, p, 6u + 12u * (unsigned)r + 3u * (unsigned)part + (unsigned)(tb + 1), have_pred);
  }
}

template <typename PIX, int SP>
TK_DEVNI void bipred_par(const Wg wg, const Team t, JobR<PIX> J, WsP<PIX> ws, MdCtx<PIX>& M) {
  const auto& c = J.cfg;
  WgShared* sh_ = M.sh;
  const auto sh = ldsc(sh_);
  const NodePos nd = node_pos(M.nd);
  const auto lists = ldsc(lds_ld(&ws->mep->lists));
  const int size = nd.size;
  const int num_iter = c.encoder_speed == 0 ? 2 : 1;
  const int max_tb = c.enable_tb_split == 1 ? 2 : 1;
  const mv_t mvp = lds_ld(&sh_->mvp);
  int prev_ref[2] = {-1, -1}, prev_cnt[2][kMaxRefs];
  mv_t prev_mv[2][4];
  mv_t min0[4], min1[4];
  for (int i = 0; i < 4; i++) { min0[i] = mvp; min1[i] = mvp; }
  int ref0 = 0, ref1 = 0;
  unsigned min_sad = 1u << 30;
  if (wg.wave == 0 && t.rank == 0) sh->bp_org8 = ws->org8;
  t.sync();
  wg.barrier();
  PIX* const org8 = (PIX*)sh->bp_org8;
  const int whole = nd.bw == size && nd.bh == size;
  for (int n = 0; n < num_iter; n++)
    for (int list = 1; list >= 0; list--) {
      const int buf = (2 * n + (1 - list)) & 1;
      const mv_t* mo = list ? min0 : min1;
      const int ref_o = list ? ref0 : ref1;
      int same = n > 0 && prev_ref[list] == ref_o;
      for (int i = 0; i < 4; i++) same = same && prev_mv[list][i].x == mo[i].x && prev_mv[list][i].y == mo[i].y;
      for (int r = 0; r < J.num_ref; r++) {
        const int cnt = lists->mvcand_num[r];
        same = same && prev_cnt[list][r] == cnt;
        prev_cnt[list][r] = cnt;
      }
      prev_ref[list] = ref_o;
      for (int i = 0; i < 4; i++) prev_mv[list][i] = mo[i];
      if (tk_uniform(same)) continue;
      if (whole) {
        const Plane3<PIX> rp = lds_ld(&J.ref[ref_o]);
        const int sgn = J.sign[ref_o];
        const mv_t mvc_ = clip_mv(mo[0], nd.ypos, nd.xpos, c.width, c.height, size, size, sgn);
        const SubPel sp = luma_setup(mvc_, sgn, size, size, c.width, c.height, nd.xpos, nd.ypos, c.enable_bipred);
        const PIX* ry = rp.y + nd.ypos * rp.sy + nd.xpos;
        const int rows = (size + wg.nwaves - 1) / wg.nwaves, r0 = tmin(size, wg.wave * rows), r1 = tmin(size, r0 + rows);
        const auto o8 = spc<SP>(org8);
        const auto oys = spc<SP>(ws->org_y);
        const int osy = ws->org_sy;
        const Pow2 pw = mk_pow2(size);
        for (int k = r0 * size + t.rank; k < r1 * size; k += t.size) {
          int i, j;
          split2(pw, k, i, j);
          o8[k] = (PIX)sat_pix(2 * (int)oys[i * osy + j] - luma_sample(ry, rp.sy, i, j, sp, c.enable_bipred, c.bitdepth), c.bitdepth);
        }
      } else if (wg.wave == 0) {
        pred_inter_yuv<SP>(t, lds_ld(&J.ref[ref_o]), ws->pred_y, ws->pred_u, ws->pred_v, nd.ypos, nd.xpos, size, nd.bw, nd.bh, mo, J.sign[ref_o], c.width,
                           c.height, c.enable_bipred, 0, c.bitdepth, 1);
        t.sync();
        build_org8<PIX, SP>(t, org8, ws->org_y, ws->org_sy, ws->pred_y, size, c.bitdepth);
      }
      t.sync();
      wg.barrier();
      for (int r = wg.wave; r < J.num_ref; r += wg.nwaves) {
        mv_t mv_all[4];
        const unsigned sad = search_inter<PIX, SP>(t, J, ws, nd.ypos, nd.xpos, size, org8, size, r, lds_ld(&sh_->mv_center[r]), mvp, mv_all, 0, J.sign[r]);
        add_cands4(t, ws, r, mv_all);
        if (t.rank == 0) { sh->bp_sad2[buf][r] = sad; for (int i = 0; i < 4; i++) lds_st(&sh_->bp_mv2[buf][r][i], mv_all[i]); }
      }
      t.sync();
      wg.barrier();
      for (int r = 0; r < J.num_ref; r++) {
        const unsigned sd = (unsigned)tk_uniform((int)sh->bp_sad2[buf][r]);
        if (sd < min_sad) {
          min_sad = sd;
          if (list) { ref1 = r; for (int i = 0; i < 4; i++) min1[i] = lds_ld(&sh_->bp_mv2[buf][r][i]); }
          else { ref0 = r; for (int i = 0; i < 4; i++) min0[i] = lds_ld(&sh_->bp_mv2[buf][r][i]); }
        }
      }
    }
  for (int tb = 0; tb <= max_tb - 1; tb++)
    if (wg.wave == tb % wg.nwaves) {
      BlkParam p = blank_param();
      p.mode = M_BIPRED; p.pb_part = P_NONE;
      p.ref0 = (int8_t)ref0; p.ref1 = (int8_t)ref1;
      for (int i = 0; i < 4; i++) { p.mv0[i] = min0[i]; p.mv1[i] = min1[i]; }
      p.tb_param = (int8_t)tb;
      par_trial<PIX, SP>(t, J, ws, M, p, 54u + (unsigned)tb, 0);
    }
}

template <typename PIX, int SP>
TK_MDW void md_worker_sp(const Wg wg, const Team t, JobR<PIX> J, WsP<PIX> ws) {
  WgShared* sh_ = ws->sh;
  const auto sh = ldsc(sh_);
  MdCtx<PIX> M;
  M.wg = wg; M.sh = sh_; M.nd = &sh_->stack[sh->node]; M.mykey = ~0ull;
  if (t.rank == 0) sh->wsnap[wg.wave] = (void*)ws->big;
  const auto ndl = ldsc(M.nd);
  ws_select(ws, tk_uniform(ndl->size));
  org_select(t, J, ws, tk_uniform(ndl->size), ndl->ypos, ndl->xpos, ndl->bw, ndl->bh, 0);
  const auto& c = J.cfg;
  const int max_tb = c.enable_tb_split == 1 ? 2 : 1;
  const int n_items = sh->n_items;
#if TK_PROF_MD
  long long pmd_acc_[4] = {0, 0, 0, 0};
#endif
  for (;;) {
    int i = 0;
    if (t.rank == 0) i = wg_fetch_add(&sh_->next_item, 1);
    i = team_bcast0(t, i);
    if (i >= n_items) break;
    const int kind = team_bcast0(t, sh->items[i].kind), ia = team_bcast0(t, sh->items[i].a), ib = team_bcast0(t, sh->items[i].b);
    TK_PROFMD_MARK(pk_);
    if (kind == MD_SKIP) {
      BlkParam p = blank_param();
      set_cand(p, lds_ld(&M.nd->skip[ia]), ia, M_SKIP);
      par_trial<PIX, SP>(t, J, ws, M, p, (unsigned)ia, 0);
    } else if (kind == MD_MERGE) {
      BlkParam p = blank_param();
      set_cand(p, lds_ld(&M.nd->merge[ia]), ia, M_MERGE);
      for (int tb = 0, have_pred = 0; tb <= max_tb - 1; tb++) {
        p.tb_param = (int8_t)tb;
        have_pred |= par_trial<PIX, SP>(t, J, ws, M, p, 2u + 2u * (unsigned)ia + (unsigned)tb, have_pred);
      }
    } else if (kind == MD_INTRA) {
      BlkParam p = blank_param();
      p.mode = M_INTRA; p.intra_mode = (int8_t)ia; p.tb_param = (int8_t)ib;
      par_trial<PIX, SP>(t, J, ws, M, p, 57u + 2u * (unsigned)ia + (unsigned)ib, 0);
    } else if (kind == MD_REF) {
      md_item_ref<PIX, SP>(t, J, ws, M, ia);
      t.sync();
      int done = 0;
      if (t.rank == 0) done = wg_fetch_add(&sh_->refs_done, 1) + 1;
      done = team_bcast0(t, done);
      if (done == sh->n_ref_items && sh->do_bipred == 1) {
        md_item_bipred<PIX, SP>(t, J, ws, M);
      }
    } else if (kind == MD_TRIAL) {
      md_item_trial<PIX, SP>(t, J, ws, M, ia, ib);
    } else if (kind == MD_BIJOINT) {
      wg_wait_at_least(t, &sh_->parts_done[J.interp_ref ? 1 : 0], 1);
      md_bijoint_telescope<PIX, SP>(t, J, ws, M);
    }
#if TK_PROF_MD
    if (TK_PROFMD_ON(1)) {
      const int slot_ = (kind == MD_SKIP || kind == MD_MERGE) ? 0 : kind == MD_INTRA ? 1 : (kind == MD_REF || kind == MD_BIJOINT) ? 2 : 3;
      if (TK_PROFMD_ON(8)) { const long long d_ = TK_CYC() - pk_; pmd_acc_[0] += slot_ == 0 ? d_ : 0; pmd_acc_[1] += slot_ == 1 ? d_ : 0; pmd_acc_[2] += slot_ == 2 ? d_ : 0; pmd_acc_[3] += slot_ == 3 ? d_ : 0; }
      else TK_PROF_ACC(ws, 16 + slot_, pk_);
    }
#endif
  }
#if TK_PROF_MD
  if (TK_PROFMD_ON(8) && t.rank == 0) for (int q_ = 0; q_ < 4; q_++) ws->prof[16 + q_] += pmd_acc_[q_];
#endif
  if (tk_uniform(sh->do_bipred) == 2) {
    t.sync();
    TK_PROF_MARK(pb_);
    wg.barrier();
    bipred_par<PIX, SP>(wg, t, J, ws, M);
    TK_PROF_ACC(ws, 27, pb_);
  }
}
template <typename PIX>
TK_DEV void md_worker(const Wg wg, const Team t, JobR<PIX> J, WsP<PIX> ws) {
  const auto sh = ldsc(ws->sh);
  const int size = tk_uniform(ldsc(&ws->sh->stack[sh->node])->size);
  if (size <= kLdsBlk) md_worker_sp<PIX, SP_LDS>(wg, t, J, ws);
  else md_worker_sp<PIX, SP_GLOBAL>(wg, t, J, ws);
}

template <typename PIX>
TK_DEV void wg_helper_loop(const Wg wg, const Team t, JobR<PIX> J, WsP<PIX> ws) {
  for (;;) {
    TK_PROF_MARK(ph_);
    wg.barrier();
    TK_PROF_ACC(ws, 28, ph_);
    const int cmd = team_bcast0(t, ws->sh->cmd);
    if (cmd == WG_CMD_EXIT) { wg.barrier(); break; }
#ifdef THOR_PROF
    { TK_PROF_MARK(pw_); md_worker(wg, t, J, ws); TK_PROF_ACC(ws, 5, pw_); }
#else
    md_worker(wg, t, J, ws);
#endif
    t.sync();
    wg.barrier();
  }
}

template <typename PIX>
TK_MDW unsigned mode_decision_par(const Wg wg, const Team t, JobR<PIX> J, WsP<PIX> ws, int node, int* win_wave) {
  const auto& c = J.cfg;
  WgShared* sh_ = ws->sh;
  const auto sh = ldsc(sh_);
  const auto nd = ldsc(&sh_->stack[node]);
  const int max_tb = c.enable_tb_split == 1 ? 2 : 1;
  const int inter = J.frame_type != F_I;
  TK_PROFMD_MARK(pqs_);
  mv_t mvp = mk_mv(0, 0);
  if (inter) mvp = get_mv_pred(J.cells, J.cell_stride, nd->ypos, nd->xpos, c.width, c.height, nd->size, sb_size_of(c));
  t.sync();
  if (t.rank == 0) {
    int n = 0;
    auto push = [&](int kind, int a, int b) { sh->items[n].kind = (int8_t)kind; sh->items[n].a = (int8_t)a; sh->items[n].b = (int8_t)b; sh->items[n].pad = 0; n++; };
    static_assert(2 + 2 + kMaxRefs + 1 + 2 * kNumIntraModes + 4 * kMaxRefs <= kMdMaxItems, "work queue too small");
    static_assert(6 + 12 * kMaxRefs <= 54, "evaluation-order layout: the reference trials must end before the bi-prediction trials");
    if (inter) {
      for (int k = 0; k < nd->syn.num_skip; k++) push(MD_SKIP, k, 0);
      for (int k = 0; k < nd->syn.num_merge; k++) push(MD_MERGE, k, 0);
      for (int r = 0; r < J.num_ref; r++) push(MD_REF, r, 0);
      if (J.num_ref > 1 && c.enable_bipred && J.frame_type == F_B) push(MD_BIJOINT, 0, 0);
      nd->syn.mvp.x = mvp.x; nd->syn.mvp.y = mvp.y;
    }
    for (int m = 0; m < J.num_intra_modes; m++)
      for (int tb = 0; tb <= max_tb - 1; tb++) push(MD_INTRA, m, tb);
    if (inter)
      for (int part = 0; part < (c.enable_pb_split ? 4 : 1); part++)
        for (int r = 0; r < J.num_ref; r++) { push(MD_TRIAL, r, part); sh->parts_done[r] = 0; }
    sh->n_items = n; sh->next_item = 0;
    sh->refs_done = 0; sh->n_ref_items = inter ? J.num_ref : 0;
    sh->do_bipred = (inter && J.num_ref > 1 && c.enable_bipred) ? (J.frame_type == F_P ? 2 : 1) : 0;
    sh->bj_state = 0;
    sh->node = node; lds_st(&sh_->mvp, mvp);
    sh->bestkey = ~0ull;
    for (int w = 0; w < kWaves; w++) sh->wkey[w] = ~0ull;
    sh->cmd = WG_CMD_MD;
  }
  t.sync();
  if (TK_PROFMD_ON(4)) TK_PROFMD_ACC(ws, 21, pqs_);
  wg.barrier();
#ifdef THOR_PROF
  { TK_PROF_MARK(pw_); md_worker(wg, t, J, ws); TK_PROF_ACC(ws, 5, pw_); t.sync(); wg.barrier(); TK_PROF_ACC(ws, 29, pw_); }
#else
  md_worker(wg, t, J, ws);
  t.sync();
  wg.barrier();
#endif
  unsigned long long best = ~0ull;
  int bw = 0;
  for (int w = 0; w < wg.nwaves; w++) {
    const unsigned long long k = sh->wkey[w];
    if (k < best) { best = k; bw = w; }
  }
  if (best == ~0ull) return kCostInit;
  if (t.rank == 0) lds_st(&sh_->stack[node].best, lds_ld(&sh_->wbest[bw]));
  t.sync();
  *win_wave = bw;
  return (unsigned)(best >> 32);
}
}
```

### thor_amd/csrc/tk_block_rd.h

```cpp
#pragma once
#include "tk_block_ctx.h"

namespace tk {
template <typename PIX> struct SsdT { typedef unsigned long long type; };
template <> struct SsdT<uint8_t> { typedef unsigned type; };
TK_DEV unsigned udot4_u8(unsigned a, unsigned b, unsigned c) {
#if TK_HOST
  for (int k = 0; k < 4; k++) c += ((a >> (8 * k)) & 0xffu) * ((b >> (8 * k)) & 0xffu);
  return c;
#else
  return __builtin_amdgcn_udot4(a, b, c, false);
#endif
}
TK_DEV unsigned udot2_u16(unsigned a, unsigned b, unsigned c) {
#if TK_HOST
  return c + (a & 0xffffu) * (b & 0xffffu) + (a >> 16) * (b >> 16);
#else
  typedef unsigned short __attribute__((ext_vector_type(2))) u16x2;
  u16x2 x, y;
  __builtin_memcpy(&x, &a, 4); __builtin_memcpy(&y, &b, 4);
  return __builtin_amdgcn_udot2(x, y, c, false);
#endif
}
template <int SP, typename PIX, int NW> TK_DEV unsigned ssd_rows(const Team t, const PIX* a_, int as, const PIX* b_, int bs, int w, int h) {
  const int spp = 4 * NW / (int)sizeof(PIX);
  const int ppr = w / spp;
  const int lg = (ppr & (ppr - 1)) ? -1 : ilog2((unsigned)ppr);
  unsigned sq = 0, ab = 0;
  for (int k = t.rank; k < ppr * h; k += t.size) {
    int i, j;
    if (lg >= 0) { i = k >> lg; j = k & (ppr - 1); } else { i = k / ppr; j = k - i * ppr; }
    uint32_t x[NW], y[NW];
#if TK_HOST
    __builtin_memcpy(x, a_ + i * as + j * spp, 4 * NW);
    __builtin_memcpy(y, b_ + i * bs + j * spp, 4 * NW);
#else
    typedef uint32_t __attribute__((ext_vector_type(NW))) vec_t;
    const vec_t xv = *(typename SpT<SP, const vec_t>::ptr)(spc<SP>(a_) + i * as + j * spp);
    const vec_t yv = *(typename SpT<SP, const vec_t>::ptr)(spc<SP>(b_) + i * bs + j * spp);
    __builtin_memcpy(x, &xv, 4 * NW);
    __builtin_memcpy(y, &yv, 4 * NW);
#endif
    TK_UNROLL
    for (int q = 0; q < NW; q++) {
      if constexpr (sizeof(PIX) == 1) { sq = udot4_u8(x[q], x[q], udot4_u8(y[q], y[q], sq)); ab = udot4_u8(x[q], y[q], ab); }
      else { sq = udot2_u16(x[q], x[q], udot2_u16(y[q], y[q], sq)); ab = udot2_u16(x[q], y[q], ab); }
    }
  }
  return sq - 2u * ab;
}
template <int SP, typename PIX>
TK_DEV typename SsdT<PIX>::type ssd_part(const Team t, const PIX* a_, int as, const PIX* b_, int bs, int w, int h) {
  a_ = tk_uniform_ptr(a_); b_ = tk_uniform_ptr(b_); as = tk_uniform(as); bs = tk_uniform(bs); w = tk_uniform(w); h = tk_uniform(h);
#ifndef TK_NOVEC
  if (!(TK_HOST && sizeof(PIX) == 2 && (w * h) / t.size > 256)) {
    const int S = (int)sizeof(PIX);
    const unsigned al = (unsigned)(uintptr_t)a_ | (unsigned)(uintptr_t)b_ | (unsigned)(as * S) | (unsigned)(bs * S) | (unsigned)(w * S);
    if (!(al & 15u)) return ssd_rows<SP, PIX, 4>(t, a_, as, b_, bs, w, h);
    if (!(al & 7u)) return ssd_rows<SP, PIX, 2>(t, a_, as, b_, bs, w, h);
    if (!(al & 3u)) return ssd_rows<SP, PIX, 1>(t, a_, as, b_, bs, w, h);
  }
#endif
  const auto a = spc<SP>(a_);
  const auto b = spc<SP>(b_);
  typename SsdT<PIX>::type local = 0;
  if ((w & (w - 1)) == 0) {
    const Pow2 pw = mk_pow2(w);
    for (int k = t.rank; k < w * h; k += t.size) {
      int i, j;
      split2(pw, k, i, j);
      int d = (int)a[i * as + j] - (int)b[i * bs + j];
      local += (typename SsdT<PIX>::type)(d * d);
    }
  } else {
    for (int k = t.rank; k < w * h; k += t.size) {
      int i = k / w, j = k - i * w;
      int d = (int)a[i * as + j] - (int)b[i * bs + j];
      local += (typename SsdT<PIX>::type)(d * d);
    }
  }
  return local;
}
TK_DEV unsigned long long ssd_total(const Team t, unsigned v) { return (unsigned long long)(unsigned)team_sum(t, (int)v); }
TK_DEV unsigned long long ssd_total(const Team t, unsigned long long v) { return team_sum64(t, v); }

template <typename PIX, int SP>
TK_DEVNI unsigned rd_cost(const Team t, JobR<PIX> J, WsP<PIX> ws, const Node& nd_, int nbits, double lambda,
                         long long ssd_y = -1) {
  TK_PROF_T0();
  const auto nd = ldsc(&nd_);
  const int size = TKU(nd->size), bw = TKU(nd->bw), bh = TKU(nd->bh);
  const int sc = size >> 1;
  typename SsdT<PIX>::type part = 0;
  if (ssd_y < 0) part += ssd_part<SP>(t, ws->org_y, ws->org_sy, ws->rec_y, size, bw, bh);
  part += ssd_part<SP>(t, ws->org_u, ws->org_sc, ws->rec_u, sc, bw >> 1, bh >> 1);
  part += ssd_part<SP>(t, ws->org_v, ws->org_sc, ws->rec_v, sc, bw >> 1, bh >> 1);
  const unsigned long long ssd = ssd_total(t, part) + (ssd_y >= 0 ? (unsigned long long)ssd_y : 0ull);
  unsigned long long cost = (ssd >> (J.cfg.bitdepth * 2 - 16)) + (unsigned long long)(long long)mul_add_nofma(lambda, (double)nbits, 0.5);
  if (cost > (1ull << 30)) cost = 1ull << 30;
  TK_PROF_ADD(ws, PF_COST);
  return (unsigned)cost;
}

template <typename PIX, int SP>
TK_DEVNI void improve_uv(const Team t, WsP<PIX> ws, const PIX* y_, PIX* u_, PIX* v_, const PIX* ry_, int n, int cstride,
                       int stride, int bitdepth) {
  const auto y = spc<SP>(y_); const auto u = spc<SP>(u_); const auto v = spc<SP>(v_); const auto ry = spc<SP>(ry_);
  (void)ws;
  const int nc = n >> 1, lognc = ilog2(nc), cs = cstride >> 1;
  long long tot8[8];
  typedef typename SsdT<PIX>::type sum_t;
  long long sq;
  {
    sum_t local = 0;
    for (int k = t.rank; k < n * n; k += t.size) {
      int i, j;
      split2(mk_pow2(n), k, i, j);
      int d = (int)ry[i * stride + j] - (int)y[i * n + j];
      local += (sum_t)(d * d);
    }
    sq = (long long)ssd_total(t, local);
  }
  if ((sq >> (2 * ilog2(n))) <= (64ll << (2 * (bitdepth - 8)))) { t.sync(); return; }
  {
    sum_t ls[8] = {0, 0, 0, 0, 0, 0, 0, 0};
    for (int k = t.rank; k < nc * nc; k += t.size) {
      int i, j;
      split2(mk_pow2(nc), k, i, j);
      int us = u[i * cs + j], vs = v[i * cs + j];
      int ys = (y[(i * 2) * n + j * 2] + y[(i * 2) * n + j * 2 + 1] + y[(i * 2 + 1) * n + j * 2] + y[(i * 2 + 1) * n + j * 2 + 1] + 2) >> 2;
      ls[0] += ys; ls[1] += us; ls[2] += vs;
      ls[3] += (unsigned)(ys * ys); ls[4] += (unsigned)(ys * us); ls[5] += (unsigned)(ys * vs);
      ls[6] += (unsigned)(us * us); ls[7] += (unsigned)(vs * vs);
    }
    for (int q = 0; q < 8; q++) ls[q] = (sum_t)ssd_total(t, ls[q]);
    tot8[0] = (long long)ls[0]; tot8[1] = (long long)ls[1]; tot8[2] = (long long)ls[2]; tot8[3] = (long long)ls[3];
    tot8[4] = (long long)ls[4]; tot8[5] = (long long)ls[5]; tot8[6] = (long long)ls[6]; tot8[7] = (long long)ls[7];
  }
  const long long ysum = tot8[0], usum = tot8[1], vsum = tot8[2], yysum = tot8[3], yusum = tot8[4],
                  yvsum = tot8[5], uusum = tot8[6], vvsum = tot8[7];
  const long long ssyy = yysum - ((ysum * ysum) >> (lognc * 2));
  const long long ssuu = uusum - ((usum * usum) >> (lognc * 2));
  const long long ssvv = vvsum - ((vsum * vsum) >> (lognc * 2));
  const long long ssyu = yusum - ((ysum * usum) >> (lognc * 2));
  const long long ssyv = yvsum - ((ysum * vsum) >> (lognc * 2));
  if (!ssyy) return;
  for (int pl = 0; pl < 2; pl++) {
    const long long ssyc = pl ? ssyv : ssyu, sscc = pl ? ssvv : ssuu, csum = pl ? vsum : usum;
    const auto c = pl ? v : u;
    if (ssyc * ssyc * 2 > ssyy * sscc) {
      long long a64 = (ssyc << 16) / ssyy;
      long long b64 = ((csum << 16) - a64 * ysum) >> (lognc * 2);
      const long long alim = 1ll << (31 - bitdepth);
      int a = (int)(a64 < -alim ? -alim : (a64 > alim ? alim : a64));
      long long bb = b64 + (1 << 15);
      int b = (int)(bb < -(1ll << 31) ? -(1ll << 31) : (bb > ((1ll << 31) - 1) ? ((1ll << 31) - 1) : bb));
      for (int k = t.rank; k < nc * nc; k += t.size) {
        int i, j;
        split2(mk_pow2(nc), k, i, j);
        int s = 2;
        for (int q = 0; q < 4; q++) {
          int r = ry[(i * 2 + (q >> 1)) * stride + j * 2 + (q & 1)];
          int m = (int)((unsigned)a * (unsigned)r + (unsigned)b);
          s += sat_pix(m >> 16, bitdepth);
        }
        c[i * cs + j] = (PIX)(s >> 2);
      }
    }
  }
  t.sync();
}

template <typename PIX, int SP>
TK_DEV void predict_inter(const Team t, JobR<PIX> J, WsP<PIX> ws, const Node& nd_, const BlkParam& p,
                          int split) {
  const auto ndl = ldsc(&nd_);
  struct { int ypos, xpos, size, bw, bh; } nd = {TKU(ndl->ypos), TKU(ndl->xpos), TKU(ndl->size), TKU(ndl->bw), TKU(ndl->bh)};
  TK_PROF_T0();
  const auto& c = J.cfg;
  const int bi = (p.mode == M_BIPRED) || ((p.mode == M_SKIP || p.mode == M_MERGE) && p.dir == 2);
  if (bi) {
    pred_inter_yuv<SP>(t, lds_ld(&J.ref[p.ref0]), ws->p0_y, ws->p0_u, ws->p0_v, nd.ypos, nd.xpos, nd.size, nd.bw, nd.bh, p.mv0,
                   J.sign[p.ref0], c.width, c.height, c.enable_bipred, split, c.bitdepth);
    pred_inter_yuv<SP>(t, lds_ld(&J.ref[p.ref1]), ws->p1_y, ws->p1_u, ws->p1_v, nd.ypos, nd.xpos, nd.size, nd.bw, nd.bh, p.mv1,
                   J.sign[p.ref1], c.width, c.height, c.enable_bipred, split, c.bitdepth);
    t.sync();
    average_yuv<SP>(t, ws->pred_y, ws->pred_u, ws->pred_v, ws->p0_y, ws->p0_u, ws->p0_v, ws->p1_y, ws->p1_u, ws->p1_v,
                nd.size, nd.bw, nd.bh);
  } else {
    pred_inter_yuv<SP>(t, lds_ld(&J.ref[p.ref0]), ws->pred_y, ws->pred_u, ws->pred_v, nd.ypos, nd.xpos, nd.size, nd.bw, nd.bh,
                   p.mv0, J.sign[p.ref0], c.width, c.height, c.enable_bipred, split, c.bitdepth);
  }
  t.sync();
  TK_PROF_ADD(ws, PF_PRED_INTER);
}

struct PruneCtx {
  unsigned thr;
  const unsigned long long* bestkey;
  unsigned order;
  double lambda;
  long long ssd_y;
  int ybits[4];
  int have_ybits;
  int pruned;
  long long ssd_part;
  int bits_part;
  int head_bits;
};

TK_DEV int prune_active(const PruneCtx* pc) { return pc && (pc->bestkey || pc->thr != 0xffffffffu); }
TK_DEV int prune_hit(const PruneCtx* pc, unsigned long long lb) {
  if (pc->bestkey) return ((lb << 32) | (unsigned long long)pc->order) > wg_load64(pc->bestkey);
  return lb >= (unsigned long long)pc->thr;
}

template <typename PIX, int SP>
TK_DEV int prune_after_quadrant(const Team t, JobR<PIX> J, WsP<PIX> ws, int nd_size, int intra, int tu, int i, int j,
                                int s2, int bit, const int16_t* coef, PruneCtx* pc) {
  if (!prune_active(pc)) return 0;
  t.sync();
  pc->ssd_part += (long long)ssd_total(t, ssd_part<SP>(t, ws->org_y + i * ws->org_sy + j, ws->org_sy, ws->rec_y + i * nd_size + j, nd_size, s2, s2));
  pc->ybits[tu] = bit ? coeff_bits_team<SP_LDS>(t, coef, s2, intra << 1) : 0;
  pc->bits_part += pc->ybits[tu];
  if (tu == 3) { pc->ssd_y = pc->ssd_part; pc->have_ybits = 1; }
  unsigned long long lb = ((unsigned long long)pc->ssd_part >> (J.cfg.bitdepth * 2 - 16)) + (unsigned long long)(long long)mul_add_nofma(pc->lambda, (double)(pc->bits_part + pc->head_bits), 0.5);
  if (lb > (1ull << 30)) lb = 1ull << 30;
#if TK_HOST
  { extern long long g_prune_stat[8]; g_prune_stat[4] += 1; if (prune_hit(pc, lb)) g_prune_stat[5 + (tu == 3)] += 1; }
#endif
  if (team_bcast0(t, prune_hit(pc, lb))) { pc->pruned = 1; return 1; }
  return 0;
}

template <typename PIX, int SP>
TK_DEV int prune_after_luma(const Team t, JobR<PIX> J, WsP<PIX> ws, int size, int bw, int bh, const BlkParam& p, int cbp_y,
                            int tb_split, PruneCtx* pc) {
  if (!prune_active(pc)) return 0;
  if (pc->pruned) return 1;
  if (pc->have_ybits) return 0;
  t.sync();
  const unsigned long long ssd = ssd_total(t, ssd_part<SP>(t, ws->org_y, ws->org_sy, ws->rec_y, size, bw, bh));
  pc->ssd_y = (long long)ssd;
  const int coeff_type = (p.mode == M_INTRA) << 1;
  int bits = 0;
  if (!tb_split) {
    pc->ybits[0] = cbp_y ? coeff_bits_team<SP_LDS>(t, ws->coef_y, size, coeff_type) : 0;
    bits = pc->ybits[0];
  } else {
    const int qy = size / 2 < kMaxQuant ? size / 2 : kMaxQuant;
    for (int tu = 0; tu < 4; tu++) {
      pc->ybits[tu] = ((cbp_y >> (3 - tu)) & 1) ? coeff_bits_team<SP_LDS>(t, ws->coef_y + tu * qy * qy, size / 2, coeff_type) : 0;
      bits += pc->ybits[tu];
    }
  }
  pc->have_ybits = 1;
  unsigned long long lb = (ssd >> (J.cfg.bitdepth * 2 - 16)) + (unsigned long long)(long long)mul_add_nofma(pc->lambda, (double)(bits + pc->head_bits), 0.5);
  if (lb > (1ull << 30)) lb = 1ull << 30;
#if TK_HOST
  { extern long long g_prune_stat[8]; g_prune_stat[p.mode == M_INTRA ? 0 : 2] += 1; if (prune_hit(pc, lb)) g_prune_stat[p.mode == M_INTRA ? 1 : 3] += 1; }
#endif
  if (team_bcast0(t, prune_hit(pc, lb))) { pc->pruned = 1; return 1; }
  return 0;
}

template <typename PIX, int SP, int SC>
TK_DEV int code_inter_plane(const Team t, JobR<PIX> J, WsP<PIX> ws, const PIX* org, int ostride,
                            const PIX* pred, PIX* rec, int size, int qp, int coeff_type, int tb_split, int16_t* coef,
                            int nd_size = 0, PruneCtx* pc = nullptr) {
  const int bd = J.cfg.bitdepth;
  if (!tb_split) {
    int fast = (size == 64 && J.cfg.encoder_speed > 0) || J.cfg.encoder_speed > 1;
    return code_tu_sp<PIX, SP, SC>(t, ws->xfp, org, ostride, pred, size, rec, size, size, qp, coeff_type, fast, coef, bd);
  }
  const int s2 = size / 2;
  int cbp = 0, index = 0;
  for (int i = 0; i < size; i += s2)
    for (int j = 0; j < size; j += s2) {
      int fast = size == 64 || J.cfg.encoder_speed > 1;
      int bit = code_tu_sp<PIX, SP, SC>(t, ws->xfp, org + i * ostride + j, ostride, pred + i * size + j, size, rec + i * size + j, size,
                        s2, qp, coeff_type, fast, coef + index, bd);
      cbp = (cbp << 1) + bit;
      if (nd_size && prune_after_quadrant<PIX, SP>(t, J, ws, nd_size, 0, (i ? 2 : 0) + (j ? 1 : 0), i, j, s2, bit, coef + index, pc)) return cbp;
      index += tmin(s2, 16) * tmin(s2, 16);
    }
  return cbp;
}

template <typename PIX, int SP>
TK_DEVNI int encode_block(const Team t, JobR<PIX> J, WsP<PIX> ws, Node& nd_, BlkParam& p, BitSink& bs,
                          int reuse_pred = 0, PruneCtx* pc = nullptr) {
  const auto& c = J.cfg;
  const NodePos nd = node_pos(&nd_);
  const int size = nd.size, sizeC = size >> 1;
  const int yc = nd.ypos >> 1, xc = nd.xpos >> 1;
  const int qpY = TKU(J.qp), qpC = TK_TAB.chroma_qp[qpY];
  const int tb_split = TKU(p.tb_param) > 0 ? TKU(p.tb_param) : 0;
  const int zero_block = TKU(p.tb_param) == -1;
  const int ftI = (TKU(J.frame_type) == F_I) << 1;
  const int bd = TKU(c.bitdepth);
  p.tb_split = (int8_t)tb_split;
  const int bigc = SP == SP_GLOBAL && tb_split && sizeC >= 32;
  ws->coef_u = bigc ? ws->coef_u_big : ws->coef_u_small;
  ws->coef_v = bigc ? ws->coef_v_big : ws->coef_v_small;
  const PIX* oy = ws->org_y;
  const PIX* ou = ws->org_u;
  const PIX* ov = ws->org_v;
  const int osy = TKU(ws->org_sy), osc = TKU(ws->org_sc);
  int cbp_y = 0, cbp_u = 0, cbp_v = 0;

  if (TKU(p.mode) == M_INTRA) {
    const int ur = upright_avail(nd.ypos, nd.xpos, size, size, c.width, sb_size_of(c));
    const int dl = downleft_avail(nd.ypos, nd.xpos, size, size, c.height, sb_size_of(c));
    const PIX* fy = J.rec.y + nd.ypos * J.rec.sy + nd.xpos;
    const PIX* fu = J.rec.u + yc * J.rec.sc + xc;
    const PIX* fv = J.rec.v + yc * J.rec.sc + xc;
    if (tb_split) {
      const int s2 = size / 2;
      int index = 0;
      for (int i = 0; i < size; i += s2)
        for (int j = 0; j < size; j += s2) {
          make_edges<SP>(t, ws->edgep, fy, J.rec.sy, ws->rec_y + i * size + j, size, i, j, nd.ypos, nd.xpos, s2, ur, dl, 1, bd);
          pred_intra<SP>(t, ws->edgep, nd.ypos + i, nd.xpos + j, s2, ws->pred_y + i * size + j, size, p.intra_mode, bd);
          t.sync();
          int bit = code_tu_sp<PIX, SP, SP_LDS>(t, ws->xfp, oy + i * osy + j, osy, ws->pred_y + i * size + j, size,
                            ws->rec_y + i * size + j, size, s2, qpY, ftI | 0, c.encoder_speed > 1, ws->coef_y + index, bd);
          cbp_y = (cbp_y << 1) + bit;
          if (prune_after_quadrant<PIX, SP>(t, J, ws, size, 1, (i ? 2 : 0) + (j ? 1 : 0), i, j, s2, bit, ws->coef_y + index, pc)) return 0;
          index += tmin(s2, 16) * tmin(s2, 16);
        }
    } else {
      make_edges<SP>(t, ws->edgep, fy, J.rec.sy, (const PIX*)nullptr, 0, 0, 0, nd.ypos, nd.xpos, size, ur, dl, 0, bd);
      pred_intra<SP>(t, ws->edgep, nd.ypos, nd.xpos, size, ws->pred_y, size, p.intra_mode, bd);
      t.sync();
      cbp_y = code_tu_sp<PIX, SP, SP_LDS>(t, ws->xfp, oy, osy, ws->pred_y, size, ws->rec_y, size, size, qpY, ftI | 0,
                      c.encoder_speed > 1, ws->coef_y, bd);
    }
    if (prune_after_luma<PIX, SP>(t, J, ws, size, nd.bw, nd.bh, p, cbp_y, tb_split, pc)) return 0;
    const int csplit = tb_split && sizeC > 4;
    if (csplit) {
      const int s2 = sizeC / 2;
      int index = 0;
      for (int i = 0; i < sizeC; i += s2)
        for (int j = 0; j < sizeC; j += s2) {
          make_edges<SP>(t, ws->edgep, fu, J.rec.sc, ws->rec_u + i * sizeC + j, sizeC, i, j, yc, xc, s2, ur, dl, 1, bd);
          pred_intra<SP>(t, ws->edgep, yc + i, xc + j, s2, ws->pred_u + i * sizeC + j, sizeC, p.intra_mode, bd);
          t.sync();
          make_edges<SP>(t, ws->edgep, fv, J.rec.sc, ws->rec_v + i * sizeC + j, sizeC, i, j, yc, xc, s2, ur, dl, 1, bd);
          pred_intra<SP>(t, ws->edgep, yc + i, xc + j, s2, ws->pred_v + i * sizeC + j, sizeC, p.intra_mode, bd);
          t.sync();
          if (c.cfl_intra)
            improve_uv<PIX, SP>(t, ws, ws->pred_y + i * sizeC + j, ws->pred_u + i * sizeC + j, ws->pred_v + i * sizeC + j,
                       ws->rec_y + (i << 1) * size + (j << 1), s2 << 1, sizeC << 1, size, bd);
          int bu, bv;
          if (bigc) {
            bu = code_tu_sp<PIX, SP, SP_GLOBAL>(t, ws->xfp, ou + i * osc + j, osc, ws->pred_u + i * sizeC + j, sizeC,
                             ws->rec_u + i * sizeC + j, sizeC, s2, qpC, ftI | 1, c.encoder_speed > 1, ws->coef_u + index, bd);
            bv = code_tu_sp<PIX, SP, SP_GLOBAL>(t, ws->xfp, ov + i * osc + j, osc, ws->pred_v + i * sizeC + j, sizeC,
                             ws->rec_v + i * sizeC + j, sizeC, s2, qpC, ftI | 1, c.encoder_speed > 1, ws->coef_v + index, bd);
          } else {
            bu = code_tu_sp<PIX, SP, SP_LDS>(t, ws->xfp, ou + i * osc + j, osc, ws->pred_u + i * sizeC + j, sizeC,
                             ws->rec_u + i * sizeC + j, sizeC, s2, qpC, ftI | 1, c.encoder_speed > 1, ws->coef_u + index, bd);
            bv = code_tu_sp<PIX, SP, SP_LDS>(t, ws->xfp, ov + i * osc + j, osc, ws->pred_v + i * sizeC + j, sizeC,
                             ws->rec_v + i * sizeC + j, sizeC, s2, qpC, ftI | 1, c.encoder_speed > 1, ws->coef_v + index, bd);
          }
          cbp_u = (cbp_u << 1) + bu;
          cbp_v = (cbp_v << 1) + bv;
          index += tmin(s2, 16) * tmin(s2, 16);
        }
    } else {
      make_edges<SP>(t, ws->edgep, fu, J.rec.sc, (const PIX*)nullptr, 0, 0, 0, yc, xc, sizeC, ur, dl, 0, bd);
      pred_intra<SP>(t, ws->edgep, yc, xc, sizeC, ws->pred_u, sizeC, p.intra_mode, bd);
      t.sync();
      make_edges<SP>(t, ws->edgep, fv, J.rec.sc, (const PIX*)nullptr, 0, 0, 0, yc, xc, sizeC, ur, dl, 0, bd);
      pred_intra<SP>(t, ws->edgep, yc, xc, sizeC, ws->pred_v, sizeC, p.intra_mode, bd);
      t.sync();
      if (c.cfl_intra) improve_uv<PIX, SP>(t, ws, ws->pred_y, ws->pred_u, ws->pred_v, ws->rec_y, size, size, size, bd);
      cbp_u = code_tu_sp<PIX, SP, SP_LDS>(t, ws->xfp, ou, osc, ws->pred_u, sizeC, ws->rec_u, sizeC, sizeC, qpC, ftI | 1,
                      c.encoder_speed > 1, ws->coef_u, bd);
      cbp_v = code_tu_sp<PIX, SP, SP_LDS>(t, ws->xfp, ov, osc, ws->pred_v, sizeC, ws->rec_v, sizeC, sizeC, qpC, ftI | 1,
                      c.encoder_speed > 1, ws->coef_v, bd);
    }
  } else {
    const int split = (TKU(p.mode) == M_INTER || TKU(p.mode) == M_BIPRED) ? c.enable_pb_split : 0;
    if (!(reuse_pred == 2 || (reuse_pred && !c.cfl_inter))) predict_inter<PIX, SP>(t, J, ws, nd_, p, split);
    if (TKU(p.mode) == M_SKIP || zero_block) {
      copy_block<SP, SP>(t, ws->rec_y, size, ws->pred_y, size, nd.bw, nd.bh);
      copy_block<SP, SP>(t, ws->rec_u, sizeC, ws->pred_u, sizeC, nd.bw >> 1, nd.bh >> 1);
      copy_block<SP, SP>(t, ws->rec_v, sizeC, ws->pred_v, sizeC, nd.bw >> 1, nd.bh >> 1);
      t.sync();
    } else {
      cbp_y = code_inter_plane<PIX, SP, SP_LDS>(t, J, ws, oy, osy, ws->pred_y, ws->rec_y, size, qpY, ftI | 0, tb_split, ws->coef_y, size, pc);
      if (prune_after_luma<PIX, SP>(t, J, ws, size, nd.bw, nd.bh, p, cbp_y, tb_split, pc)) return 0;
      if (c.cfl_inter) improve_uv<PIX, SP>(t, ws, ws->pred_y, ws->pred_u, ws->pred_v, ws->rec_y, size, size, size, bd);
      const int csplit = tb_split && sizeC > 4;
      if (bigc) {
        cbp_u = code_inter_plane<PIX, SP, SP_GLOBAL>(t, J, ws, ou, osc, ws->pred_u, ws->rec_u, sizeC, qpC, ftI | 1, csplit, ws->coef_u);
        cbp_v = code_inter_plane<PIX, SP, SP_GLOBAL>(t, J, ws, ov, osc, ws->pred_v, ws->rec_v, sizeC, qpC, ftI | 1, csplit, ws->coef_v);
      } else {
        cbp_u = code_inter_plane<PIX, SP, SP_LDS>(t, J, ws, ou, osc, ws->pred_u, ws->rec_u, sizeC, qpC, ftI | 1, csplit, ws->coef_u);
        cbp_v = code_inter_plane<PIX, SP, SP_LDS>(t, J, ws, ov, osc, ws->pred_v, ws->rec_v, sizeC, qpC, ftI | 1, csplit, ws->coef_v);
      }
    }
  }
  p.cbp_y = (uint8_t)cbp_y;
  p.cbp_u = (uint8_t)cbp_u;
  p.cbp_v = (uint8_t)cbp_v;
  TK_PROF_T0();
  const SynCtx syn = lds_ld(&nd_.syn);
  const int* yb = (pc && pc->have_ybits) ? pc->ybits : nullptr;
  int nb_ = bigc ? bs_block_t<false, SP_GLOBAL>(bs, syn, p, ws->coef_y, ws->coef_u, ws->coef_v, &t, yb)
                 : bs_block_t<false, SP_LDS>(bs, syn, p, ws->coef_y, ws->coef_u, ws->coef_v, &t, yb);
  TK_PROF_ADD(ws, PF_BITS);
  return nb_;
}

template <typename PIX, int SP>
TK_DEV unsigned rdo_trial(const Team t, JobR<PIX> J, WsP<PIX> ws, Node& nd, BlkParam& p, double lambda,
                          int reuse_pred = 0, unsigned prune_thr = 0xffffffffu, const unsigned long long* bestkey = nullptr,
                          unsigned order = 0, int* nbits_out = nullptr, int* untouched = nullptr) {
  BitSink cnt;
  cnt.buf = nullptr; cnt.pos = 0; cnt.cap = 0; cnt.emit = 0; cnt.ovf = 0;
  PruneCtx pc;
  pc.thr = prune_thr; pc.bestkey = bestkey; pc.order = order; pc.lambda = lambda; pc.ssd_y = -1; pc.have_ybits = 0; pc.pruned = 0; pc.ssd_part = 0; pc.bits_part = 0;
  pc.head_bits = 0;
  if (bestkey || prune_thr != 0xffffffffu) {
    BitSink hb = cnt;
    bs_block_head_t<false>(hb, uniform_syn(lds_ld(&nd.syn)), uniform_blk(p));
    pc.head_bits = hb.pos;
    unsigned long long lb0 = (unsigned long long)(long long)mul_add_nofma(lambda, (double)hb.pos, 0.5);
    if (lb0 > (1ull << 30)) lb0 = 1ull << 30;
#if TK_HOST
    { extern long long g_prune_stat[8]; g_prune_stat[7] += prune_hit(&pc, lb0); }
#endif
    if (team_bcast0(t, prune_hit(&pc, lb0))) {
      if (untouched) *untouched = 1;
      return kCostInit;
    }
  }
  int nbits = encode_block<PIX, SP>(t, J, ws, nd, p, cnt, reuse_pred, &pc);
  if (nbits_out) *nbits_out = nbits;
  if (pc.pruned) return kCostInit;
  return rd_cost<PIX, SP>(t, J, ws, nd, nbits, lambda, pc.ssd_y);
}

TK_DEV BlkParam normalize_best(const Node& nd, const BlkParam& p) {
  BlkParam b = p;
  if (p.mode == M_SKIP || p.mode == M_MERGE) {
    const InterPred c = lds_ld((p.mode == M_SKIP) ? &nd.skip[p.skip_idx] : &nd.merge[p.skip_idx]);
    b.ref0 = c.ref0; b.ref1 = c.ref1; b.dir = c.dir;
    for (int i = 0; i < 4; i++) { b.mv0[i] = c.mv0; b.mv1[i] = c.mv1; }
  } else if (p.mode == M_INTRA) {
    b.ref0 = b.ref1 = 0; b.dir = -1;
    for (int i = 0; i < 4; i++) { b.mv0[i] = mk_mv(0, 0); b.mv1[i] = mk_mv(0, 0); }
  } else if (p.mode == M_INTER) b.dir = 0;
  else b.dir = 2;
  return b;
}
TK_DEV void keep_best(Node& nd, const BlkParam& p) { lds_st(&nd.best, normalize_best(nd, p)); }

TK_DEV void set_cand(BlkParam& p, const InterPred& c, int idx, int mode) {
  p.mode = (int8_t)mode;
  p.skip_idx = (int8_t)idx;
  p.ref0 = c.ref0; p.ref1 = c.ref1; p.dir = c.dir;
  for (int i = 0; i < 4; i++) { p.mv0[i] = c.mv0; p.mv1[i] = c.mv1; }
}
}
```

### thor_amd/csrc/tk_block_ws.h

```cpp
#pragma once
#include "tk_common.h"
#include "tk_bits.h"
#include "tk_pred.h"
#include "tk_xform.h"
#include "tk_me.h"

namespace tk {
struct Node {
  int size, ypos, xpos, bw, bh;
  int stage, child;
  int md_done;
  unsigned cost_this;
  unsigned cost_small;
  int bitpos0;
  int encode_this_size, encode_rect;
  SynCtx syn;
  InterPred skip[2], merge[2];
  BlkParam best;
};
struct NodePos { int size, ypos, xpos, bw, bh; };
TK_DEV NodePos node_pos(const Node* n) {
  const auto l = ldsc(n);
  return {TKU(l->size), TKU(l->ypos), TKU(l->xpos), TKU(l->bw), TKU(l->bh)};
}

enum { kProfSlots = 32 };
enum { kMdMaxItems = 48 };
#ifndef TK_LDSBLK
#define TK_LDSBLK 16
#endif
enum { kLdsBlk = TK_LDSBLK };
enum { MD_SKIP = 0, MD_MERGE, MD_REF, MD_INTRA, MD_BIPRED, MD_TRIAL, MD_BIJOINT };
enum { WG_CMD_EXIT = 0, WG_CMD_MD = 1 };
struct MdItem { int8_t kind, a, b, pad; };
struct WgShared {
  XformTabs tabs;
  MeLists lists;
  Node stack[5];
  int cmd;
  int next_item, n_items;
  int refs_done, n_ref_items;
  int do_bipred;
  int parts_done[kMaxRefs];
  mv_t ref_mv[kMaxRefs][4][4];
  const void* bp_org8;
  unsigned bp_sad2[2][kMaxRefs];
  mv_t bp_mv2[2][kMaxRefs][4];
  int bj_state;
  unsigned bj_sad;
  mv_t bj_mv;
  int node;
  mv_t mvp;
  mv_t mv_center[kMaxRefs];
  unsigned long long bestkey;
  unsigned long long wkey[kWaves];
  BlkParam wbest[kWaves];
  void* wsnap[kWaves];
  MdItem items[kMdMaxItems];
  alignas(16) unsigned char org_raw[kLdsBlk * kLdsBlk * 3];
};
template <typename PIX> struct WinExtra { enum { bytes = sizeof(PIX) == 1 ? (TK_OCC == 2 ? 7680 : 944) : 5376 }; };
template <typename PIX> struct SmallWs {
  XformWs xf;
  alignas(16) unsigned char win_extra[WinExtra<PIX>::bytes];
  MeWs me;
  IntraEdge<PIX> edge;
  int16_t coef_y[4 * 256], coef_u[256], coef_v[256];
  unsigned long long acc[12];
  alignas(16) PIX lbuf[7 * kLdsBlk * kLdsBlk];
#if defined(THOR_PROF)
  long long prof[kProfSlots];
#else
  long long prof[1];
#endif
};
static_assert(offsetof(SmallWs<uint8_t>, lbuf) % 16 == 0 && offsetof(SmallWs<uint16_t>, lbuf) % 16 == 0 && sizeof(SmallWs<uint8_t>) % 16 == 0 &&
              sizeof(SmallWs<uint16_t>) % 16 == 0 && offsetof(WgShared, org_raw) % 16 == 0, "LDS sample blocks must be 16-byte aligned");
template <typename PIX> struct BigWs {
  PIX pred_y[kMaxSb * kMaxSb], pred_u[kMaxSb * kMaxSb / 4], pred_v[kMaxSb * kMaxSb / 4];
  PIX p0_y[kMaxSb * kMaxSb], p0_u[kMaxSb * kMaxSb / 4], p0_v[kMaxSb * kMaxSb / 4];
  PIX p1_y[kMaxSb * kMaxSb], p1_u[kMaxSb * kMaxSb / 4], p1_v[kMaxSb * kMaxSb / 4];
  PIX rec_y[kMaxSb * kMaxSb], rec_u[kMaxSb * kMaxSb / 4], rec_v[kMaxSb * kMaxSb / 4];
  PIX org8[kMaxSb * kMaxSb];
  int16_t coef_u_big[4 * 256], coef_v_big[4 * 256];
  PIX best_y[kMaxSb * kMaxSb], best_u[kMaxSb * kMaxSb / 4], best_v[kMaxSb * kMaxSb / 4];
  int16_t best_cy[4 * 256], best_cu[4 * 256], best_cv[4 * 256];
};
template <typename PIX> struct TeamWs {
  XformWs* xfp;
  MeWs* mep;
  IntraEdge<PIX>* edgep;
  int16_t *coef_y, *coef_u, *coef_v;
  int16_t *coef_u_small, *coef_v_small, *coef_u_big, *coef_v_big;
  unsigned long long* acc;
  WgShared* sh;
  Node* stack;
  long long* prof;
  PIX *pred_y, *pred_u, *pred_v, *p0_y, *p0_u, *p0_v, *p1_y, *p1_u, *p1_v, *rec_y, *rec_u, *rec_v, *org8;
  BigWs<PIX>* big;
  PIX* lbuf;
  const PIX *org_y, *org_u, *org_v;
  int org_sy, org_sc;
};
#if TK_HOST
template <typename PIX> using WsP = TeamWs<PIX>*;
template <typename PIX> using JobR = const FrameJob<PIX>&;
#else
template <typename PIX> using WsP = TK_LDS TeamWs<PIX>*;
template <typename PIX> using JobR = const TK_LDS FrameJob<PIX>&;
#endif
template <class WP> TK_DEV void ws_select(WP w, int size) {
  if (size <= kLdsBlk) {
    auto b = w->lbuf;
    const int n = size * size, c = n >> 2;
    w->pred_y = b; w->pred_u = b + n; w->pred_v = b + n + c; b += n + 2 * c;
    w->p0_y = b; w->p0_u = b + n; w->p0_v = b + n + c; b += n + 2 * c;
    w->p1_y = b; w->p1_u = b + n; w->p1_v = b + n + c; b += n + 2 * c;
    w->rec_y = b; w->rec_u = b + n; w->rec_v = b + n + c; b += n + 2 * c;
    w->org8 = b;
  } else {
    auto g = w->big;
    w->pred_y = g->pred_y; w->pred_u = g->pred_u; w->pred_v = g->pred_v;
    w->p0_y = g->p0_y; w->p0_u = g->p0_u; w->p0_v = g->p0_v;
    w->p1_y = g->p1_y; w->p1_u = g->p1_u; w->p1_v = g->p1_v;
    w->rec_y = g->rec_y; w->rec_u = g->rec_u; w->rec_v = g->rec_v; w->org8 = g->org8;
  }
}
template <typename PIX>
TK_DEV void org_select(const Team t, JobR<PIX> J, WsP<PIX> w, int size, int ypos, int xpos, int bw, int bh, int load) {
  if (size <= kLdsBlk) {
    PIX* b = (PIX*)w->sh->org_raw;
    const int n = size * size, sc = size >> 1;
    if (load) {
      t.sync();
      const Div2 dw = mk_div(bw), dc = mk_div(bw >> 1);
      const TK_GLOBAL PIX* gy = gptr(J.orig.y + ypos * J.orig.sy + xpos);
      const TK_GLOBAL PIX* gu = gptr(J.orig.u + (ypos >> 1) * J.orig.sc + (xpos >> 1));
      const TK_GLOBAL PIX* gv = gptr(J.orig.v + (ypos >> 1) * J.orig.sc + (xpos >> 1));
      const auto bl = ldsc(b);
      for (int k = t.rank; k < bw * bh; k += t.size) { int i, j; split2(dw, k, i, j); bl[i * size + j] = gy[i * J.orig.sy + j]; }
      for (int k = t.rank; k < (bw >> 1) * (bh >> 1); k += t.size) {
        int i, j;
        split2(dc, k, i, j);
        bl[n + i * sc + j] = gu[i * J.orig.sc + j];
        bl[n + (n >> 2) + i * sc + j] = gv[i * J.orig.sc + j];
      }
      t.sync();
    }
    w->org_y = b; w->org_u = b + n; w->org_v = b + n + (n >> 2);
    w->org_sy = size; w->org_sc = sc;
  } else {
    w->org_y = J.orig.y + ypos * J.orig.sy + xpos;
    w->org_u = J.orig.u + (ypos >> 1) * J.orig.sc + (xpos >> 1);
    w->org_v = J.orig.v + (ypos >> 1) * J.orig.sc + (xpos >> 1);
    w->org_sy = J.orig.sy; w->org_sc = J.orig.sc;
  }
}

template <typename PIX> TK_DEV TeamWs<PIX> make_ws(SmallWs<PIX>* s, WgShared* sh, BigWs<PIX>* g) {
  TeamWs<PIX> w;
  w.xfp = &s->xf; w.mep = &s->me; w.edgep = &s->edge;
  w.sh = sh; s->xf.tabs = &sh->tabs; s->me.lists = &sh->lists;
  static_assert(offsetof(SmallWs<PIX>, win_extra) == offsetof(SmallWs<PIX>, xf) + sizeof(XformWs), "win_extra must directly follow the transform workspace");
  s->me.win = (uint32_t*)s->xf.in;
  s->me.win_cap = (int)(sizeof(XformWs) - offsetof(XformWs, in)) + (int)WinExtra<PIX>::bytes;
  s->me.cwin_valid = 0;
  w.coef_y = s->coef_y; w.coef_u = s->coef_u; w.coef_v = s->coef_v;
  w.coef_u_small = s->coef_u; w.coef_v_small = s->coef_v; w.coef_u_big = g->coef_u_big; w.coef_v_big = g->coef_v_big;
  w.acc = s->acc; w.stack = sh->stack; w.prof = s->prof;
  s->xf.prof = s->prof; s->me.prof = s->prof;
  w.big = g; w.lbuf = s->lbuf;
  w.org_y = w.org_u = w.org_v = nullptr; w.org_sy = w.org_sc = 0;
  ws_select(&w, kMaxSb);
  return w;
}

#if TK_PROF_MD
#ifndef THOR_PROF_MD_PARTS
#define THOR_PROF_MD_PARTS 7
#endif
#define TK_PROFMD_MARK(v) TK_PROF_MARK(v)
#define TK_PROFMD_ACC(ws, id, v) TK_PROF_ACC(ws, id, v)
#define TK_PROFMD_CNT(ws, id) TK_PROF_CNT(ws, id)
#define TK_PROFMD_ON(bit) ((THOR_PROF_MD_PARTS) & (bit))
#else
#define TK_PROFMD_ON(bit) 0
#define TK_PROFMD_MARK(v) do {} while (0)
#define TK_PROFMD_ACC(ws, id, v) do {} while (0)
#define TK_PROFMD_CNT(ws, id) do {} while (0)
#endif
enum { PF_SB = 0, PF_ESKIP, PF_ME_FULL, PF_ME_SUB, PF_PRED_INTER, PF_PRED_INTRA, PF_TU, PF_BITS, PF_COST, PF_FINAL,
       PF_CFL, PF_BIPRED_PREP, PF_QUANT };
}
```

### thor_amd/csrc/tk_kat_block.h

```cpp
#pragma once
#include "tk_block_search.h"

namespace tk {
enum { kKatCtxPar = 6, kKatCtxOut = 23 };
TK_DEV void kat_ctx_item(const DbCell* cells, int cs, const int* q, int* o) {
  const int ypos = q[0], xpos = q[1], size = q[2], fw = q[3], fh = q[4], sb = q[5];
  const mv_t p = get_mv_pred(cells, cs, ypos, xpos, fw, fh, size, sb);
  InterPred c[2];
  c[0] = zero_pred(); c[1] = zero_pred();
  const int n = get_mv_cands(cells, cs, ypos, xpos, fw, fh, size, sb, c);
  o[0] = p.x; o[1] = p.y; o[2] = n;
  for (int k = 0; k < 2; k++) {
    const InterPred z = k < n ? c[k] : zero_pred();
    int* r = o + 3 + 7 * k;
    r[0] = z.mv0.x; r[1] = z.mv0.y; r[2] = z.mv1.x; r[3] = z.mv1.y; r[4] = z.ref0; r[5] = z.ref1; r[6] = z.dir;
  }
  for (int enable = 0; enable < 2; enable++) {
    SynCtx s;
    find_contexts(cells, cs, ypos, xpos, fh, fw, size, enable, &s);
    o[17 + 2 * enable] = s.ctx_cbp; o[18 + 2 * enable] = s.ctx_index;
  }
  o[21] = upright_avail(ypos, xpos, size, size, fw, sb);
  o[22] = downleft_avail(ypos, xpos, size, size, fh, sb);
}
static inline int kat_ctx_check(const int* q, long long ncells) {
  const int ypos = q[0], xpos = q[1], size = q[2], fw = q[3], fh = q[4], sb = q[5];
  if ((sb != 64 && sb != 128) || size < 8 || size > sb || (size & (size - 1)) || fw < 8 || fh < 8 || fw > 8192 || fh > 8192 || fw % 8 || fh % 8) return 1;
  if (ypos < 0 || xpos < 0 || ypos >= fh || xpos >= fw || ypos % size || xpos % size) return 1;
  const long long cs = fw / 4, bi = (long long)(ypos / 4) * cs + xpos / 4;
  return bi + cs * (size / 4) <= ncells ? 0 : 2;
}

enum { kKatCostPar = 7, kKatCostOut = 4 };
static inline int kat_cost_check(const int* q, double lambda, long long nsamp, int sample_bytes) {
  const int size = q[0], bw = q[1], bh = q[2], nbits = q[3], off = q[4], skew = q[5], stride = q[6];
  if (size < 8 || size > kMaxSb || (size & (size - 1)) || bw < 8 || bh < 8 || bw > size || bh > size || bw % 8 || bh % 8) return 1;
  if (nbits < 0 || nbits > (1 << 20) || !(lambda >= 0.0 && lambda <= 1e6)) return 1;
  if (skew < 0 || skew >= 16 || skew % sample_bytes || stride < bw || stride > 4096 || stride % 2) return 1;
  if (off < 0 || off % 16 || (long long)off + size * size * 3 / 2 > nsamp) return 2;
  return 0;
}

enum { kKatIntraPar = 6, kKatIntraOut = 2 };
static inline int kat_intra_check(const int* q, int fw, int fh, long long nsamp) {
  const int ypos = q[0], xpos = q[1], size = q[2], sb = q[3], nm = q[4], off = q[5];
  if ((sb != 64 && sb != 128) || size < 8 || size > 64 || (size & (size - 1)) || (nm != 4 && nm != 10)) return 1;
  if (ypos < 0 || xpos < 0 || ypos % size || xpos % size || ypos + size > fh || xpos + size > fw) return 2;
  if (off < 0 || off % 16 || (long long)off + size * size > nsamp) return 2;
  return 0;
}
enum { kKatOrg8Par = 4 };
static inline int kat_org8_check(const int* q, long long nsamp, int sample_bytes) {
  const int size = q[0], off = q[1], skew = q[2], stride = q[3];
  if (size < 8 || size > kMaxSb || (size & (size - 1)) || skew < 0 || skew >= 16 || skew % sample_bytes || stride < size || stride > 4096) return 1;
  if (off < 0 || off % 16 || (long long)off + size * size > nsamp) return 2;
  return 0;
}
}
```

### thor_amd/csrc/tk_pred.h

```cpp
#pragma once
#include "tk_common.h"

namespace tk {

TK_DEV constexpr unsigned long long pack_taps6(int a, int b, int c, int d, int e, int f) {
  return (unsigned long long)(unsigned)(a & 0xff) | ((unsigned long long)(unsigned)(b & 0xff) << 8) | ((unsigned long long)(unsigned)(c & 0xff) << 16) |
         ((unsigned long long)(unsigned)(d & 0xff) << 24) | ((unsigned long long)(unsigned)(e & 0xff) << 32) | ((unsigned long long)(unsigned)(f & 0xff) << 40);
}
TK_DEV unsigned long long luma_taps8(int bipred, int frac) {
  const unsigned long long z = pack_taps6(0, 0, 64, 0, 0, 0);
  const unsigned long long s1 = pack_taps6(1, -7, 55, 19, -5, 1), s2 = pack_taps6(1, -7, 38, 38, -7, 1), s3 = pack_taps6(1, -5, 19, 55, -7, 1);
  const unsigned long long b1 = pack_taps6(2, -10, 59, 17, -5, 1), b2 = pack_taps6(1, -8, 39, 39, -8, 1), b3 = pack_taps6(1, -5, 17, 59, -10, 2);
  const unsigned long long s = frac == 1 ? s1 : frac == 2 ? s2 : s3, b = frac == 1 ? b1 : frac == 2 ? b2 : b3;
  return frac == 0 ? z : (bipred ? b : s);
}
TK_DEV int luma_tap(int bipred, int frac, int m) { return (int)(int8_t)(luma_taps8(bipred, frac) >> (8 * m)); }
TK_DEV unsigned chroma_taps8(int frac) {
  auto pk = [](int a, int b, int c, int d) -> unsigned { return (unsigned)(a & 0xff) | ((unsigned)(b & 0xff) << 8) | ((unsigned)(c & 0xff) << 16) | ((unsigned)(d & 0xff) << 24); };
  const unsigned lo = frac == 0 ? pk(0, 64, 0, 0) : frac == 1 ? pk(-2, 58, 10, -2) : frac == 2 ? pk(-4, 54, 16, -2) : pk(-4, 44, 28, -4);
  const unsigned hi = frac == 4 ? pk(-4, 36, 36, -4) : frac == 5 ? pk(-4, 28, 44, -4) : frac == 6 ? pk(-2, 16, 54, -4) : pk(-2, 10, 58, -2);
  return frac < 4 ? lo : hi;
}
TK_DEV int chroma_tap(int frac, int m) { return (int)(int8_t)(chroma_taps8(frac) >> (8 * m)); }

TK_DEV mv_t clip_mv(mv_t mv, int ypos, int xpos, int fwidth, int fheight, int bwidth, int bheight, int sign) {
  const int ext = kPadY - 16;
  int mvy = sign ? -mv.y : mv.y;
  int mvx = sign ? -mv.x : mv.x;
  if (ypos + mvy / 4 < -ext) mvy = 4 * (-ext - ypos);
  if (ypos + mvy / 4 + bheight > fheight + ext) mvy = 4 * (fheight + ext - ypos - bheight);
  if (xpos + mvx / 4 < -ext) mvx = 4 * (-ext - xpos);
  if (xpos + mvx / 4 + bwidth > fwidth + ext) mvx = 4 * (fwidth + ext - xpos - bwidth);
  return mk_mv(sign ? -mvx : mvx, sign ? -mvy : mvy);
}

struct SubPel {
  int hor_int, ver_int, hor_frac, ver_frac;
  int th[6], tv[6];
  unsigned long long ph, pv;
};
TK_DEV SubPel luma_setup(mv_t mv, int sign, int width, int height, int pic_w, int pic_h, int xpos, int ypos, int bipred = 0) {
  int mx = sign ? -mv.x : mv.x, my = sign ? -mv.y : mv.y;
  SubPel s;
  s.ver_frac = my & 3;
  s.hor_frac = mx & 3;
  int vi = my >> 2, hi = mx >> 2;
  vi = tmin(vi, pic_h - ypos);
  vi = tmax(vi, -xpos - height);
  hi = tmin(hi, pic_w - xpos);
  hi = tmax(hi, -xpos - width);
  s.ver_int = vi;
  s.hor_int = hi;
  const unsigned long long ph = luma_taps8(bipred, s.hor_frac), pv = luma_taps8(bipred, s.ver_frac);
  s.ph = ph; s.pv = pv;
  for (int m = 0; m < 6; m++) {
    s.th[m] = (int)(int8_t)(ph >> (8 * m));
    s.tv[m] = (int)(int8_t)(pv >> (8 * m));
  }
  return s;
}

template <typename PIX> TK_DEV void load6(const PIX* p, int r[6]) {
  if (sizeof(PIX) == 1) {
    const unsigned long long v = gload64(p);
    for (int m = 0; m < 6; m++) r[m] = (int)((v >> (8 * m)) & 0xffu);
  } else {
    const unsigned long long v0 = gload64(p);
    const unsigned v1 = gload32((const char*)p + 8);
    for (int m = 0; m < 4; m++) r[m] = (int)((v0 >> (16 * m)) & 0xffffu);
    r[4] = (int)(v1 & 0xffffu);
    r[5] = (int)(v1 >> 16);
  }
}

template <typename PIX> TK_DEV void load4(const PIX* p, int r[4]) {
  if (sizeof(PIX) == 1) {
    const unsigned v = gload32(p);
    for (int m = 0; m < 4; m++) r[m] = (int)((v >> (8 * m)) & 0xffu);
  } else {
    const unsigned long long v = gload64(p);
    for (int m = 0; m < 4; m++) r[m] = (int)((v >> (16 * m)) & 0xffffu);
  }
}

template <typename PIX>
TK_DEV int luma_sample(const PIX* ref, int stride, int i, int j, const SubPel& s, int bipred, int bitdepth) {
  const TK_GLOBAL PIX* p = gptr(ref) + (i + s.ver_int) * stride + (j + s.hor_int);
  if (s.ver_frac == 0 && s.hor_frac == 0) return p[0];
  if (s.ver_frac == 2 && s.hor_frac == 2 && bipred < 2) {
    int a[4], b[4], c[4], d[4];
    load4((const PIX*)(p - stride - 1), a); load4((const PIX*)(p - 1), b); load4((const PIX*)(p + stride - 1), c); load4((const PIX*)(p + 2 * stride - 1), d);
    int sum = a[1] + a[2] + b[0] + 2 * b[1] + 2 * b[2] + b[3] + c[0] + 2 * c[1] + 2 * c[2] + c[3] + d[1] + d[2];
    return sat_pix((sum + 8) >> 4, bitdepth);
  }
  if (s.hor_frac == 0) {
    int sum = 0;
    for (int m = 0; m < 6; m++) sum += s.tv[m] * p[(m - 2) * stride];
    return sat_pix((sum * 64 + 2048) >> 12, bitdepth);
  }
  if (s.ver_frac == 0) {
    int r[6];
    load6((const PIX*)(p - 2), r);
    int sum = 0;
    for (int m = 0; m < 6; m++) sum += s.th[m] * r[m];
    return sat_pix((sum * 64 + 2048) >> 12, bitdepth);
  }
  int r[6][6];
  for (int m = 0; m < 6; m++) load6((const PIX*)(p + (m - 2) * stride - 2), r[m]);
  int sum = 0;
  for (int n = 0; n < 6; n++) {
    int col = 0;
    for (int m = 0; m < 6; m++) col += s.tv[m] * r[m][n];
    sum += s.th[n] * col;
  }
  return sat_pix((sum + 2048) >> 12, bitdepth);
}

template <typename PIX> struct WinRow;
template <> struct WinRow<uint8_t> { unsigned long long a; };
template <> struct WinRow<uint16_t> { unsigned long long a, b; };
TK_DEV void win_load(const uint8_t* p, WinRow<uint8_t>& r) { r.a = gload64(p); }
TK_DEV void win_load(const uint16_t* p, WinRow<uint16_t>& r) { r.a = gload64(p); r.b = gload64(p + 4); }
TK_DEV WinRow<uint8_t> win_pick(const WinRow<uint8_t>& r0, const WinRow<uint8_t>& r1, const WinRow<uint8_t>& r2, int dy, int dx) {
  WinRow<uint8_t> o;
  o.a = (dy == 0 ? r0.a : (dy == 1 ? r1.a : r2.a)) >> (8 * dx);
  return o;
}
TK_DEV WinRow<uint16_t> win_pick(const WinRow<uint16_t>& r0, const WinRow<uint16_t>& r1, const WinRow<uint16_t>& r2, int dy, int dx) {
  const unsigned long long a = dy == 0 ? r0.a : (dy == 1 ? r1.a : r2.a), b = dy == 0 ? r0.b : (dy == 1 ? r1.b : r2.b);
  WinRow<uint16_t> o;
  if (dx == 0) { o.a = a; o.b = b; }
  else { o.a = (a >> (16 * dx)) | (b << (64 - 16 * dx)); o.b = b >> (16 * dx); }
  return o;
}
TK_DEV int win_at(const WinRow<uint8_t>& r, int n) { return (int)((r.a >> (8 * n)) & 0xffu); }
TK_DEV int win_at(const WinRow<uint16_t>& r, int n) { return n < 4 ? (int)((r.a >> (16 * n)) & 0xffffu) : (int)((r.b >> (16 * (n - 4))) & 0xffffu); }

template <typename PIX> TK_DEV int luma_sample_win(const WinRow<PIX> w[6], const SubPel& s, int bipred, int bitdepth) {
  if (s.ver_frac == 0 && s.hor_frac == 0) return win_at(w[2], 2);
  if (s.ver_frac == 2 && s.hor_frac == 2 && bipred < 2) {
    int sum = win_at(w[1], 2) + win_at(w[1], 3) + win_at(w[2], 1) + 2 * win_at(w[2], 2) + 2 * win_at(w[2], 3) + win_at(w[2], 4) +
              win_at(w[3], 1) + 2 * win_at(w[3], 2) + 2 * win_at(w[3], 3) + win_at(w[3], 4) + win_at(w[4], 2) + win_at(w[4], 3);
    return sat_pix((sum + 8) >> 4, bitdepth);
  }
  if (s.hor_frac == 0) {
    int sum = 0;
    for (int m = 0; m < 6; m++) sum += s.tv[m] * win_at(w[m], 2);
    return sat_pix((sum * 64 + 2048) >> 12, bitdepth);
  }
  if (s.ver_frac == 0) {
    int sum = 0;
    for (int n = 0; n < 6; n++) sum += s.th[n] * win_at(w[2], n);
    return sat_pix((sum * 64 + 2048) >> 12, bitdepth);
  }
  int sum = 0;
  for (int n = 0; n < 6; n++) {
    int col = 0;
    for (int m = 0; m < 6; m++) col += s.tv[m] * win_at(w[m], n);
    sum += s.th[n] * col;
  }
  return sat_pix((sum + 2048) >> 12, bitdepth);
}

TK_DEV int dot4_i8(int a, int b, int c) {
#if TK_HOST
  for (int k = 0; k < 4; k++) c += (int)(int8_t)(a >> (8 * k)) * (int)(int8_t)(b >> (8 * k));
  return c;
#else
  return __builtin_amdgcn_sdot4(a, b, c, false);
#endif
}
struct SubK8 {
  unsigned long long th8;
  int tv[6];
  int centre, dy, dx;
};
TK_DEV SubK8 subk8_make(const SubPel& s, int dy, int dx, int bipred) {
  SubK8 k;
  k.th8 = s.ph << (8 * dx);
  for (int m = 0; m < 6; m++) k.tv[m] = (int)(int8_t)(s.pv >> (8 * m));
  k.centre = s.ver_frac == 2 && s.hor_frac == 2 && bipred < 2;
  k.dy = dy; k.dx = dx;
  return k;
}
TK_DEV int mul24(int a, int b) {
#if TK_HOST
  return a * b;
#else
  return __mul24(a, b);
#endif
}
template <int DY> TK_DEV int subk8_sample_dy(const unsigned long long* wr, const SubK8& k) {
  if (k.centre) {
    const unsigned long long wA = 0x0000000001010000ull << (8 * k.dx), wB = 0x0000000102020100ull << (8 * k.dx);
    int sum = 128 * 16;
    sum = dot4_i8((int)(unsigned)wA, (int)(unsigned)wr[DY + 1], dot4_i8((int)(unsigned)(wA >> 32), (int)(unsigned)(wr[DY + 1] >> 32), sum));
    sum = dot4_i8((int)(unsigned)wB, (int)(unsigned)wr[DY + 2], dot4_i8((int)(unsigned)(wB >> 32), (int)(unsigned)(wr[DY + 2] >> 32), sum));
    sum = dot4_i8((int)(unsigned)wB, (int)(unsigned)wr[DY + 3], dot4_i8((int)(unsigned)(wB >> 32), (int)(unsigned)(wr[DY + 3] >> 32), sum));
    sum = dot4_i8((int)(unsigned)wA, (int)(unsigned)wr[DY + 4], dot4_i8((int)(unsigned)(wA >> 32), (int)(unsigned)(wr[DY + 4] >> 32), sum));
    return sat_pix((sum + 8) >> 4, 8);
  }
  int sum = 0;
  TK_UNROLL
  for (int m = 0; m < 6; m++) {
    const unsigned long long row = wr[DY + m];
    const int h = dot4_i8((int)(unsigned)k.th8, (int)(unsigned)row, dot4_i8((int)(unsigned)(k.th8 >> 32), (int)(unsigned)(row >> 32), 128 * 64));
    sum += mul24(k.tv[m], h);
  }
  return sat_pix((sum + 2048) >> 12, 8);
}
TK_DEV int subk8_sample(const unsigned long long* wr, const SubK8& k) {
  if (k.dy == 0) return subk8_sample_dy<0>(wr, k);
  if (k.dy == 1) return subk8_sample_dy<1>(wr, k);
  return subk8_sample_dy<2>(wr, k);
}

template <int DY> TK_DEV int subk8_strip_dy(const unsigned long long* wb, const SubK8& k, const int* o, int sad) {
  auto ad = [](int x, int y) -> int { const unsigned a = (unsigned)x, b = (unsigned)y; return (int)((a > b ? a : b) - (a < b ? a : b)); };
  if (k.centre) {
    const unsigned long long wA = 0x0000000001010000ull << (8 * k.dx), wB = 0x0000000102020100ull << (8 * k.dx);
    int ra[12], rb[12];
    TK_UNROLL
    for (int q = 1; q < 12; q++) {
      const unsigned long long row = wb[DY + q];
      ra[q] = dot4_i8((int)(unsigned)wA, (int)(unsigned)row, dot4_i8((int)(unsigned)(wA >> 32), (int)(unsigned)(row >> 32), 0));
      rb[q] = dot4_i8((int)(unsigned)wB, (int)(unsigned)row, dot4_i8((int)(unsigned)(wB >> 32), (int)(unsigned)(row >> 32), 0));
    }
    TK_UNROLL
    for (int p = 0; p < 8; p++) sad += ad(o[p], sat_pix((128 * 16 + ra[p + 1] + rb[p + 2] + rb[p + 3] + ra[p + 4] + 8) >> 4, 8));
    return sad;
  }
  int hs[13];
  TK_UNROLL
  for (int q = 0; q < 13; q++) {
    const unsigned long long row = wb[DY + q];
    hs[q] = dot4_i8((int)(unsigned)k.th8, (int)(unsigned)row, dot4_i8((int)(unsigned)(k.th8 >> 32), (int)(unsigned)(row >> 32), 128 * 64));
  }
  TK_UNROLL
  for (int p = 0; p < 8; p++) {
    int sum = 0;
    TK_UNROLL
    for (int m = 0; m < 6; m++) sum += mul24(k.tv[m], hs[p + m]);
    sad += ad(o[p], sat_pix((sum + 2048) >> 12, 8));
  }
  return sad;
}
TK_DEV int subk8_strip(const unsigned long long* wb, const SubK8& k, const int* o, int sad) {
  if (k.dy == 0) return subk8_strip_dy<0>(wb, k, o, sad);
  if (k.dy == 1) return subk8_strip_dy<1>(wb, k, o, sad);
  return subk8_strip_dy<2>(wb, k, o, sad);
}

struct SubK16 {
  uint32_t th2[3];
  int tv[6];
  int centre, dy, dx;
};
TK_DEV SubK16 subk16_make(const SubPel& s, int dy, int dx, int bipred) {
  SubK16 k;
  for (int q = 0; q < 3; q++) k.th2[q] = (uint32_t)(uint16_t)(int16_t)s.th[2 * q] | ((uint32_t)(uint16_t)(int16_t)s.th[2 * q + 1] << 16);
  for (int m = 0; m < 6; m++) k.tv[m] = s.tv[m];
  k.centre = s.ver_frac == 2 && s.hor_frac == 2 && bipred < 2;
  k.dy = dy; k.dx = dx;
  return k;
}
TK_DEV int dot2_i16(uint32_t a, uint32_t b, int c) {
#if TK_HOST
  return c + (int)(int16_t)(a & 0xffffu) * (int)(int16_t)(b & 0xffffu) + (int)(int16_t)(a >> 16) * (int)(int16_t)(b >> 16);
#else
  typedef short __attribute__((ext_vector_type(2))) s16x2;
  s16x2 x, y;
  __builtin_memcpy(&x, &a, 4); __builtin_memcpy(&y, &b, 4);
  return __builtin_amdgcn_sdot2(x, y, c, false);
#endif
}
template <int DX> TK_DEV uint32_t row_pair16(const uint32_t* d, int q) {
  if constexpr (DX == 0) return d[q];
  else if constexpr (DX == 2) return d[q + 1];
  else {
#if TK_HOST
    return (d[q] >> 16) | (d[q + 1] << 16);
#else
    return __builtin_amdgcn_alignbyte(d[q + 1], d[q], 2);
#endif
  }
}
template <int DY, int DX> TK_DEV int subk16_sample_t(const uint32_t (*rows)[4], const SubK16& k, int bitdepth) {
  if (k.centre) {
    int sum = 8;
    sum = dot2_i16(0x00010001u, row_pair16<DX>(rows[DY + 1], 1), sum);
    sum = dot2_i16(0x00010001u, row_pair16<DX>(rows[DY + 4], 1), sum);
    TK_UNROLL
    for (int m = 2; m <= 3; m++) {
      sum = dot2_i16(0x00010000u, row_pair16<DX>(rows[DY + m], 0), sum);
      sum = dot2_i16(0x00020002u, row_pair16<DX>(rows[DY + m], 1), sum);
      sum = dot2_i16(0x00000001u, row_pair16<DX>(rows[DY + m], 2), sum);
    }
    return sat_pix(sum >> 4, bitdepth);
  }
  int sum = 2048;
  TK_UNROLL
  for (int m = 0; m < 6; m++) {
    const uint32_t* d = rows[DY + m];
    const int h = dot2_i16(k.th2[0], row_pair16<DX>(d, 0), dot2_i16(k.th2[1], row_pair16<DX>(d, 1), dot2_i16(k.th2[2], row_pair16<DX>(d, 2), 0)));
    sum += mul24(k.tv[m], h);
  }
  return sat_pix(sum >> 12, bitdepth);
}
TK_DEV int subk16_sample(const uint32_t (*rows)[4], const SubK16& k, int bitdepth) {
  switch (k.dy * 3 + k.dx) {
    case 0: return subk16_sample_t<0, 0>(rows, k, bitdepth);
    case 1: return subk16_sample_t<0, 1>(rows, k, bitdepth);
    case 2: return subk16_sample_t<0, 2>(rows, k, bitdepth);
    case 3: return subk16_sample_t<1, 0>(rows, k, bitdepth);
    case 4: return subk16_sample_t<1, 1>(rows, k, bitdepth);
    case 5: return subk16_sample_t<1, 2>(rows, k, bitdepth);
    case 6: return subk16_sample_t<2, 0>(rows, k, bitdepth);
    case 7: return subk16_sample_t<2, 1>(rows, k, bitdepth);
    default: return subk16_sample_t<2, 2>(rows, k, bitdepth);
  }
}

template <int DY, int DX> TK_DEV int subk16_strip_t(const uint32_t (*wb)[4], const SubK16& k, const int* o, int sad, int bitdepth) {
  if (k.centre) {
    int ra[12], rb[12];
    TK_UNROLL
    for (int q = 1; q < 12; q++) {
      const uint32_t* d = wb[DY + q];
      ra[q] = dot2_i16(0x00010001u, row_pair16<DX>(d, 1), 0);
      rb[q] = dot2_i16(0x00010000u, row_pair16<DX>(d, 0), dot2_i16(0x00020002u, row_pair16<DX>(d, 1), dot2_i16(0x00000001u, row_pair16<DX>(d, 2), 0)));
    }
    TK_UNROLL
    for (int p = 0; p < 8; p++) sad += iabs(o[p] - sat_pix((8 + ra[p + 1] + rb[p + 2] + rb[p + 3] + ra[p + 4]) >> 4, bitdepth));
    return sad;
  }
  int hs[13];
  TK_UNROLL
  for (int q = 0; q < 13; q++) {
    const uint32_t* d = wb[DY + q];
    hs[q] = dot2_i16(k.th2[0], row_pair16<DX>(d, 0), dot2_i16(k.th2[1], row_pair16<DX>(d, 1), dot2_i16(k.th2[2], row_pair16<DX>(d, 2), 0)));
  }
  TK_UNROLL
  for (int p = 0; p < 8; p++) {
    int sum = 2048;
    TK_UNROLL
    for (int m = 0; m < 6; m++) sum += mul24(k.tv[m], hs[p + m]);
    sad += iabs(o[p] - sat_pix(sum >> 12, bitdepth));
  }
  return sad;
}
TK_DEV int subk16_strip(const uint32_t (*wb)[4], const SubK16& k, const int* o, int sad, int bitdepth) {
  switch (k.dy * 3 + k.dx) {
    case 0: return subk16_strip_t<0, 0>(wb, k, o, sad, bitdepth);
    case 1: return subk16_strip_t<0, 1>(wb, k, o, sad, bitdepth);
    case 2: return subk16_strip_t<0, 2>(wb, k, o, sad, bitdepth);
    case 3: return subk16_strip_t<1, 0>(wb, k, o, sad, bitdepth);
    case 4: return subk16_strip_t<1, 1>(wb, k, o, sad, bitdepth);
    case 5: return subk16_strip_t<1, 2>(wb, k, o, sad, bitdepth);
    case 6: return subk16_strip_t<2, 0>(wb, k, o, sad, bitdepth);
    case 7: return subk16_strip_t<2, 1>(wb, k, o, sad, bitdepth);
    default: return subk16_strip_t<2, 2>(wb, k, o, sad, bitdepth);
  }
}

template <int SP, typename PIX>
TK_DEV void pred_luma(const Team t, PIX* dst_, int dstride, const PIX* ref, int rstride, int width, int height, mv_t mv,
                      int sign, int bipred, int pic_w, int pic_h, int xpos, int ypos, int bitdepth) {
  const auto dst = spc<SP>(dst_);
  SubPel s = luma_setup(mv, sign, width, height, pic_w, pic_h, xpos, ypos, bipred);
  const Div2 pw = mk_div(width);
  for (int k = t.rank; k < width * height; k += t.size) {
    int i, j;
    split2(pw, k, i, j);
    dst[i * dstride + j] = (PIX)luma_sample(ref, rstride, i, j, s, bipred, bitdepth);
  }
}

template <int SP, typename PIX>
TK_DEV void pred_chroma(const Team t, PIX* dst_, int dstride, const PIX* ref, int rstride, int width, int height,
                        mv_t mv, int sign, int pic_w2, int pic_h2, int xpos, int ypos, int bitdepth) {
  const auto dst = spc<SP>(dst_);
  int mx = sign ? -mv.x : mv.x, my = sign ? -mv.y : mv.y;
  int vf = my & 7, hf = mx & 7;
  int vi = my >> 3, hi = mx >> 3;
  vi = tmin(vi, pic_h2 - ypos);
  vi = tmax(vi, -xpos - height);
  hi = tmin(hi, pic_w2 - xpos);
  hi = tmax(hi, -xpos - width);
  int th[4], tv[4];
  {
    const unsigned ph = chroma_taps8(hf), pv = chroma_taps8(vf);
    for (int n = 0; n < 4; n++) { th[n] = (int)(int8_t)(ph >> (8 * n)); tv[n] = (int)(int8_t)(pv >> (8 * n)); }
  }
  for (int k = t.rank; k < width * height; k += t.size) {
    int i, j;
    split2(mk_div(width), k, i, j);
    const TK_GLOBAL PIX* p = gptr(ref) + (i + vi) * rstride + (j + hi);
    int v;
    if (vf == 0 && hf == 0) {
      v = p[0];
    } else {
      int sum = 0;
      for (int n = 0; n < 4; n++) {
        const TK_GLOBAL PIX* q = p + (n - 1) * rstride;
        int row = th[0] * q[-1] + th[1] * q[0] + th[2] * q[1] + th[3] * q[2];
        sum += tv[n] * row;
      }
      v = sat_pix((sum + 2048) >> 12, bitdepth);
    }
    dst[i * dstride + j] = (PIX)v;
  }
}

#if defined(TK_PIY_INLINE)
#define TK_PIY TK_DEV
#else
#define TK_PIY TK_DEVNI
#endif
template <int SP, typename PIX>
TK_PIY void pred_inter_yuv(const Team t, const Plane3<PIX> ref, PIX* py, PIX* pu, PIX* pv, int ypos, int xpos,
                           int size, int bw, int bh, const mv_t* mv_arr, int sign, int pic_w, int pic_h,
                           int enable_bipred, int split, int bitdepth, int luma_only = 0) {
  const int div = split + 1;
  const int bwidth = bw / div, bheight = bh / div;
  const int pstride = size;
  const int yc = ypos >> 1, xc = xpos >> 1;
  const PIX* ry = ref.y + ypos * ref.sy + xpos;
  const PIX* ru = ref.u + yc * ref.sc + xc;
  const PIX* rv = ref.v + yc * ref.sc + xc;
  for (int index = 0; index < div * div; index++) {
    int idx = index & 1, idy = (index >> 1) & 1;
    int offpY = idy * bheight * pstride + idx * bwidth;
    int offpC = ((idy * bheight * pstride) >> 2) + ((idx * bwidth) >> 1);
    int offrY = idy * bheight * ref.sy + idx * bwidth;
    int offrC = ((idy * bheight * ref.sc) >> 1) + ((idx * bwidth) >> 1);
    mv_t mv = clip_mv(mv_arr[index], ypos, xpos, pic_w, pic_h, bwidth, bheight, sign);
    pred_luma<SP>(t, py + offpY, pstride, ry + offrY, ref.sy, bwidth, bheight, mv, sign, enable_bipred, pic_w, pic_h,
              xpos, ypos, bitdepth);
    if (luma_only) continue;
    pred_chroma<SP>(t, pu + offpC, pstride >> 1, ru + offrC, ref.sc, bwidth >> 1, bheight >> 1, mv, sign, pic_w >> 1,
                pic_h >> 1, xc, yc, bitdepth);
    pred_chroma<SP>(t, pv + offpC, pstride >> 1, rv + offrC, ref.sc, bwidth >> 1, bheight >> 1, mv, sign, pic_w >> 1,
                pic_h >> 1, xc, yc, bitdepth);
  }
}

template <int SP, typename PIX> TK_DEV void average_rows(const Team t, PIX* d_, const PIX* a_, const PIX* b_, int stride, int w, int h) {
  const int spp = 4 / (int)sizeof(PIX);
  const uint32_t M = sizeof(PIX) == 1 ? 0x7f7f7f7fu : 0x7fff7fffu;
  const int ppr = w / spp;
  for (int k = t.rank; k < ppr * h; k += t.size) {
    const int i = k / ppr, j = k - i * ppr;
    const int o = i * stride + spp * j;
#if TK_HOST
    uint32_t x, y;
    __builtin_memcpy(&x, a_ + o, 4); __builtin_memcpy(&y, b_ + o, 4);
    const uint32_t r = (x & y) + (((x ^ y) >> 1) & M);
    __builtin_memcpy(d_ + o, &r, 4);
#else
    const uint32_t x = *(typename SpT<SP, const uint32_t>::ptr)(spc<SP>(a_) + o), y = *(typename SpT<SP, const uint32_t>::ptr)(spc<SP>(b_) + o);
    *(typename SpT<SP, uint32_t>::ptr)(spc<SP>(d_) + o) = (x & y) + (((x ^ y) >> 1) & M);
#endif
  }
}
template <int SP, typename PIX>
TK_DEV void average_yuv(const Team t, PIX* dy_, PIX* du_, PIX* dv_, const PIX* ay_, const PIX* au_, const PIX* av_,
                        const PIX* by_, const PIX* bu_, const PIX* bv_, int size, int bw, int bh) {
#ifndef TK_NOVEC
  if (tk_uniform(!((bw | size) & 7))) {
    average_rows<SP>(t, dy_, ay_, by_, size, bw, bh);
    average_rows<SP>(t, du_, au_, bu_, size >> 1, bw >> 1, bh >> 1);
    average_rows<SP>(t, dv_, av_, bv_, size >> 1, bw >> 1, bh >> 1);
    return;
  }
#endif
  const auto dy = spc<SP>(dy_); const auto du = spc<SP>(du_); const auto dv = spc<SP>(dv_);
  const auto ay = spc<SP>(ay_); const auto au = spc<SP>(au_); const auto av = spc<SP>(av_);
  const auto by = spc<SP>(by_); const auto bu = spc<SP>(bu_); const auto bv = spc<SP>(bv_);
  for (int k = t.rank; k < bw * bh; k += t.size) {
    int i, j;
    split2(mk_div(bw), k, i, j);
    int o = i * size + j;
    dy[o] = (PIX)(((int)ay[o] + (int)by[o]) >> 1);
  }
  int cw = bw >> 1, ch = bh >> 1, cs = size >> 1;
  for (int k = t.rank; k < cw * ch; k += t.size) {
    int i, j;
    split2(mk_div(cw), k, i, j);
    int o = i * cs + j;
    du[o] = (PIX)(((int)au[o] + (int)bu[o]) >> 1);
    dv[o] = (PIX)(((int)av[o] + (int)bv[o]) >> 1);
  }
}

template <typename PIX> struct IntraEdge {
  PIX left[2 * kMaxSb];
  PIX top[2 * kMaxSb];
  PIX top_left;
};

template <int SP, typename PIX>
TK_DEV void make_edges(const Team t, IntraEdge<PIX>* e, const PIX* rec_frame, int fstride, const PIX* rblock,
                       int rbstride, int i, int j, int ypos, int xpos, int size, int cb_upright, int cb_downleft,
                       int tb_split, int bitdepth) {
  e = tk_uniform_ptr(e); rec_frame = tk_uniform_ptr(rec_frame); rblock = tk_uniform_ptr(rblock); fstride = tk_uniform(fstride);
  rbstride = tk_uniform(rbstride); i = tk_uniform(i); j = tk_uniform(j); ypos = tk_uniform(ypos); xpos = tk_uniform(xpos); size = tk_uniform(size);
  cb_upright = tk_uniform(cb_upright); cb_downleft = tk_uniform(cb_downleft); tb_split = tk_uniform(tb_split); bitdepth = tk_uniform(bitdepth);
  const int len = 2 * size;
  const PIX dflt = (PIX)(128 << (bitdepth - 8));
  int downleft, upright;
  if (!tb_split) {
    downleft = cb_downleft;
    upright = cb_upright;
  } else {
    downleft = (j == 0 && (i == 0 || cb_downleft)) ? 1 : 0;
    upright = (j == 0 || (i == 0 && cb_upright)) ? 1 : 0;
  }
  const int leftlen = downleft ? size + 1 : size;
  const int toplen = upright ? size + 1 : size;
  const int top_from_block = tb_split && i != 0;
  const int left_from_block = tb_split && j != 0;
  const auto rblock_g = spc<SP>(rblock);
  const TK_GLOBAL PIX* const frame_g = gptr(rec_frame);
  const auto e_top = ldsc(e->top);
  const auto e_left = ldsc(e->left);
  const int top_dflt = (ypos + i == 0);
  const int left_dflt = (xpos + j == 0);
  for (int k = t.rank; k < len; k += t.size) {
    PIX tv, lv;
    if (top_dflt) tv = dflt;
    else {
      const int kk = k < toplen ? k : toplen - 1;
      tv = top_from_block ? rblock_g[kk - rbstride] : frame_g[kk - fstride + j];
    }
    if (left_dflt) lv = dflt;
    else {
      int kk = k < leftlen ? k : leftlen - 1;
      lv = left_from_block ? rblock_g[kk * rbstride - 1] : frame_g[(i + kk) * fstride - 1];
    }
    e_top[k] = tv;
    e_left[k] = lv;
  }
  if (t.rank == 0) {
    PIX tl;
    if (top_dflt) {
      tl = left_dflt ? dflt : (left_from_block ? rblock_g[-1] : frame_g[i * fstride - 1]);
    } else if (!top_from_block) {
      tl = xpos > 0 ? frame_g[-fstride + j - 1] : frame_g[-fstride + j];
    } else {
      tl = xpos > 0 ? (j > 0 ? rblock_g[-rbstride - 1] : frame_g[(i - 1) * fstride - 1]) : rblock_g[-rbstride];
    }
    *ldsc(&e->top_left) = tl;
  }
  t.sync();
}

template <typename PIX> TK_DEV int f121(const PIX* a, int k, int len) {
  int km = k > 0 ? k - 1 : 0, kp = k < len - 1 ? k + 1 : len - 1;
  return (a[km] + 2 * a[k] + a[kp] + 2) >> 2;
}
template <typename PIX> TK_DEV int f5(const PIX* a, int k, int size) {
  int k0 = clampi(k - 2, 0, size - 1), k1 = clampi(k - 1, 0, size - 1), k3 = clampi(k + 1, 0, size - 1),
      k4 = clampi(k + 2, 0, size - 1);
  return (int16_t)(a[k0] + 2 * a[k1] + 2 * a[k] + 2 * a[k3] + a[k4]);
}

template <int SP, typename PIX>
TK_DEV void pred_intra(const Team t, const IntraEdge<PIX>* e, int ypos, int xpos, int size, PIX* dst_, int dstride,
                       int mode, int bitdepth) {
  PIX* dst = dst_;
  e = tk_uniform_ptr(e); dst = tk_uniform_ptr(dst); ypos = tk_uniform(ypos); xpos = tk_uniform(xpos); size = tk_uniform(size);
  dstride = tk_uniform(dstride); mode = tk_uniform(mode); bitdepth = tk_uniform(bitdepth);
  typedef TK_LDS PIX lpix;
  const lpix* left = (const lpix*)ldsc(e->left);
  const lpix* top = (const lpix*)ldsc(e->top);
  const int tl = *ldsc(&e->top_left);
  const auto dsts = spc<SP>(dst);
  int dc = 0, tlF = 0, tlP = 0;
  if (mode == 0 || mode > 9) {
    const lpix* a = xpos != 0 ? left : top;
    const lpix* b = ypos != 0 ? top : left;
    unsigned sum = 0;
    for (int k = 0; k < size; k++) sum += (unsigned)a[k] + (unsigned)b[k];
    dc = (int)((sum + (unsigned)size) / (2u * (unsigned)size));
  } else if (mode == 1) {
    tlP = (int16_t)(left[1] + 2 * left[0] + 2 * tl + 2 * top[0] + top[1]);
  } else if (mode == 4 || mode == 7 || mode == 8) {
    tlF = (PIX)((2 * tl + left[0] + top[0] + 2) >> 2);
  }
  const Pow2 pw = mk_pow2(size);
  for (int k = t.rank; k < size * size; k += t.size) {
    int i, j;
    split2(pw, k, i, j);
    int v;
    switch (mode) {
      case 1:
        v = sat_pix((f5(left, i, size) + f5(top, j, size) - tlP + 4) / 8, bitdepth);
        break;
      case 2: v = left[i]; break;
      case 3: v = top[j]; break;
      case 4: {
        int d = i - j;
        v = d > 0 ? f121(left, d - 1, size) : (d == 0 ? tlF : f121(top, -d - 1, size));
      } break;
      case 5: v = f121(top, i + j + 1, 2 * size); break;
      case 6: {
        int d = i + 2 * j;
        v = (d & 1) ? f121(top, (d + 1) / 2, 2 * size) : ((f121(top, d / 2, 2 * size) + f121(top, d / 2 + 1, 2 * size)) >> 1);
      } break;
      case 7: {
        int d = i - 2 * j;
        if (d > 1) v = f121(left, d - 2, size);
        else if (d == 1) v = tlF;
        else if (d == 0) v = (tlF + f121(top, 0, size)) >> 1;
        else if (d & 1) v = f121(top, (-d) / 2, size);
        else v = (f121(top, (-d) / 2, size) + f121(top, (-d) / 2 - 1, size)) >> 1;
      } break;
      case 8: {
        int d = 2 * i - j;
        if (d < -1) v = f121(top, -d - 2, size);
        else if (d == -1) v = tlF;
        else if (d == 0) v = (tlF + f121(left, 0, size)) >> 1;
        else if (d & 1) v = f121(left, d / 2, size);
        else v = (f121(left, d / 2, size) + f121(left, d / 2 - 1, size)) >> 1;
      } break;
      case 9: {
        int d = 2 * i + j;
        v = (d & 1) ? f121(left, (d + 1) / 2, 2 * size) : ((f121(left, d / 2, 2 * size) + f121(left, d / 2 + 1, 2 * size)) >> 1);
      } break;
      default: v = dc; break;
    }
    dsts[i * dstride + j] = (PIX)v;
  }
}

}
```

Before: 164.3.

## Stage intra edge pixels in LDS once per block for intra mode trials

Before the mode-decision items run, the workgroup copies the top, left and corner neighbour pixels of Y, U and V for the current block into a small LDS buffer, along with the upright/downleft availability. Each intra trial then builds its edges from that LDS copy instead of re-reading the reconstructed frame in global memory and recomputing availability. The point is to cut repeated global loads across the many intra trials per block. It costs extra shared memory in WgShared, which may lower occupancy, and adds a validation kernel with a host binding.

```diff
diff --git a/include/thor_hip.h b/include/thor_hip.h
--- a/include/thor_hip.h
+++ b/include/thor_hip.h
@@ -160,6 +160,8 @@
 int thor_hip_kat_lds_block(void);
 int thor_hip_kat_block_cost(int n, const int* par, const double* lambda, const void* org, const void* rec, long long nsamp, int bitdepth, unsigned long long* out);
 int thor_hip_kat_intra_search(int n, const int* par, const void* plane, int width, int height, const void* org, long long nsamp, int bitdepth, int* out);
+int thor_hip_kat_intra_edges(int n, const int* par, const void* y, const void* u, const void* v, int width, int height, const void* recb, int bitdepth, void* out);
+int thor_hip_kat_intra_edges_image_bytes(int bitdepth);
 int thor_hip_kat_build_org8(int n, const int* par, const void* org, const void* pred, long long nsamp, int bitdepth, void* out_global, void* out_lds);
 int thor_hip_kat_coeff_syntax(int n, const int* par, const int16_t* coef, int words, uint32_t* buf_single, uint32_t* buf_team, int* out);
 int thor_hip_kat_block_syntax(int n, const int* par, const int16_t* pool, int npool, int words, uint32_t* buf_coop, uint32_t* buf_single, int* out);
diff --git a/thor_amd/binding.py b/thor_amd/binding.py
--- a/thor_amd/binding.py
+++ b/thor_amd/binding.py
@@ -634,6 +634,18 @@
     return out
 
 
+def kat_intra_edges(par, y, u, v, recb, bitdepth=8):
+    T = _pix(bitdepth)
+    y, u, v = (np.ascontiguousarray(a, dtype=T) for a in (y, u, v))
+    recb = np.ascontiguousarray(recb, dtype=T).ravel(); par = np.ascontiguousarray(par, dtype=np.int32)
+    assert y.ndim == 2 and u.shape == v.shape == (y.shape[0] // 2, y.shape[1] // 2) and par.ndim == 2 and par.shape[1] == 4 and len(recb) == 64 * 64 * 3 // 2
+    fn = lib().thor_hip_kat_intra_edges_image_bytes
+    fn.restype = C.c_int
+    out = np.zeros((len(par), 2, 15, fn(bitdepth)), dtype=np.uint8)
+    _kat('thor_hip_kat_intra_edges', len(par), _vp(par), _vp(y), _vp(u), _vp(v), y.shape[1], y.shape[0], _vp(recb), bitdepth, _vp(out))
+    return out
+
+
 def kat_build_org8(par, org, pred, bitdepth=8, fill=0):
     T = _pix(bitdepth)
     org = np.ascontiguousarray(org, dtype=T).ravel(); pred = np.ascontiguousarray(pred, dtype=T).ravel()
diff --git a/thor_amd/csrc/hip_kat_block.h b/thor_amd/csrc/hip_kat_block.h
--- a/thor_amd/csrc/hip_kat_block.h
+++ b/thor_amd/csrc/hip_kat_block.h
@@ -127,9 +127,35 @@
     for (int k = lane; k < n; k += 64) outl[off + k] = w.org8[k];
   }
 }
+template <typename PIX>
+__global__ __launch_bounds__(kWgThreads, (sizeof(PIX) == 1 ? (int)kOcc : 2)) void k_kat_intra_edges(const int* par, Plane3<PIX> rec, int fw, int fh, int bitdepth, const PIX* recb,
+                                                                                                    unsigned char* out) {
+  __shared__ WgShared sh;
+  __shared__ IntraEdge<PIX> edge;
+  const int lane = (int)threadIdx.x, it = (int)blockIdx.x;
+  const Team t = mk_team(lane, 64);
+  kat_edges_item<PIX>(t, &edge, (PIX*)sh.edge_raw, rec, fw, fh, bitdepth, par + kKatEdgePar * it, recb, out + (size_t)it * 2 * kKatEdgeImgs * sizeof(IntraEdge<PIX>));
+}
 }
 
 namespace {
+template <typename PIX>
+int kat_intra_edges(int n, const int* par, const PIX* y, const PIX* u, const PIX* v, int fw, int fh, const PIX* recb, int bitdepth, unsigned char* out) {
+  if (n <= 0 || n > 4096 || !par || !y || !u || !v || !recb || !out || fw < 16 || fh < 16 || fw > 4096 || fh > 4096 || fw % 16 || fh % 16) return 1;
+  for (int i = 0; i < n; i++)
+    if (int r = kat_edges_check(par + kKatEdgePar * i, fw, fh, (int)sizeof(PIX))) return r;
+  if (!ensure_init_any()) return 3;
+  const size_t ny = (size_t)fw * fh, nc = ny / 4, no = (size_t)n * 2 * kKatEdgeImgs * sizeof(IntraEdge<PIX>);
+  DevBuf<int> d_par((size_t)kKatEdgePar * n, par);
+  DevBuf<PIX> d_y(ny, y), d_u(nc, u), d_v(nc, v), d_rb((size_t)64 * 64 * 3 / 2, recb);
+  DevBuf<unsigned char> d_o(no);
+  Plane3<PIX> rec;
+  rec.y = d_y; rec.u = d_u; rec.v = d_v; rec.sy = fw; rec.sc = fw / 2;
+  hipLaunchKernelGGL(k_kat_intra_edges<PIX>, dim3(n), dim3(64), 0, g_stream, d_par, rec, fw, fh, bitdepth, d_rb, d_o);
+  HIPCHECK(hipGetLastError());
+  backend::d2h(out, d_o, no);
+  return 0;
+}
 template <typename PIX>
 int kat_intra_search(int n, const int* par, const PIX* plane, int fw, int fh, const PIX* org, long long nsamp, int bitdepth, int* out) {
   if (n <= 0 || n > 4096 || !par || !plane || !org || !out || fw < 8 || fh < 8 || fw > 4096 || fh > 4096 || fw % 8 || fh % 8 || nsamp <= 0 || nsamp > (1ll << 30)) return 1;
@@ -237,6 +263,11 @@
   KAT_BD(kat_intra_search<uint8_t>(n, par, (const uint8_t*)plane, width, height, (const uint8_t*)org, nsamp, 8, out),
          kat_intra_search<uint16_t>(n, par, (const uint16_t*)plane, width, height, (const uint16_t*)org, nsamp, bitdepth, out));
 }
+extern "C" int thor_hip_kat_intra_edges(int n, const int* par, const void* y, const void* u, const void* v, int width, int height, const void* recb, int bitdepth, void* out) {
+  KAT_BD(kat_intra_edges<uint8_t>(n, par, (const uint8_t*)y, (const uint8_t*)u, (const uint8_t*)v, width, height, (const uint8_t*)recb, 8, (unsigned char*)out),
+         kat_intra_edges<uint16_t>(n, par, (const uint16_t*)y, (const uint16_t*)u, (const uint16_t*)v, width, height, (const uint16_t*)recb, bitdepth, (unsigned char*)out));
+}
+extern "C" int thor_hip_kat_intra_edges_image_bytes(int bitdepth) { return bitdepth == 8 ? (int)sizeof(IntraEdge<uint8_t>) : (int)sizeof(IntraEdge<uint16_t>); }
 extern "C" int thor_hip_kat_build_org8(int n, const int* par, const void* org, const void* pred, long long nsamp, int bitdepth, void* out_global, void* out_lds) {
   KAT_BD(kat_build_org8<uint8_t>(n, par, (const uint8_t*)org, (const uint8_t*)pred, nsamp, 8, (uint8_t*)out_global, (uint8_t*)out_lds),
          kat_build_org8<uint16_t>(n, par, (const uint16_t*)org, (const uint16_t*)pred, nsamp, bitdepth, (uint16_t*)out_global, (uint16_t*)out_lds));
diff --git a/thor_amd/csrc/tk_block_queue.h b/thor_amd/csrc/tk_block_queue.h
--- a/thor_amd/csrc/tk_block_queue.h
+++ b/thor_amd/csrc/tk_block_queue.h
@@ -41,9 +41,9 @@
 };
 
 template <typename PIX, int SP>
-TK_DEV int par_trial(const Team t, JobR<PIX> J, WsP<PIX> ws, MdCtx<PIX>& M, BlkParam& p, unsigned order, int reuse_pred) {
+TK_DEV int par_trial(const Team t, JobR<PIX> J, WsP<PIX> ws, MdCtx<PIX>& M, BlkParam& p, unsigned order, int reuse_pred, const PIX* staged = nullptr) {
   int untouched = 0;
-  const unsigned cost = rdo_trial<PIX, SP>(t, J, ws, *M.nd, p, J.lambda, reuse_pred, 0xffffffffu, &M.sh->bestkey, order, nullptr, &untouched);
+  const unsigned cost = rdo_trial<PIX, SP>(t, J, ws, *M.nd, p, J.lambda, reuse_pred, 0xffffffffu, &M.sh->bestkey, order, nullptr, &untouched, staged);
   if (cost == (unsigned)kCostInit) return !untouched;
   const unsigned long long key = ((unsigned long long)cost << 32) | order;
   if (key < M.mykey) {
@@ -331,7 +331,8 @@
     } else if (kind == MD_INTRA) {
       BlkParam p = blank_param();
       p.mode = M_INTRA; p.intra_mode = (int8_t)ia; p.tb_param = (int8_t)ib;
-      par_trial<PIX, SP>(t, J, ws, M, p, 57u + 2u * (unsigned)ia + (unsigned)ib, 0);
+      const PIX* const staged = edges_staged<PIX>(tk_uniform(ndl->size)) ? (const PIX*)sh_->edge_raw : nullptr;
+      par_trial<PIX, SP>(t, J, ws, M, p, 57u + 2u * (unsigned)ia + (unsigned)ib, 0, staged);
     } else if (kind == MD_REF) {
       md_item_ref<PIX, SP>(t, J, ws, M, ia);
       t.sync();
@@ -430,6 +431,13 @@
     for (int w = 0; w < kWaves; w++) sh->wkey[w] = ~0ull;
     sh->cmd = WG_CMD_MD;
   }
+  const int esize = tk_uniform(nd->size);
+  if (J.num_intra_modes > 0 && edges_staged<PIX>(esize)) {
+    const int ey = tk_uniform(nd->ypos), ex = tk_uniform(nd->xpos);
+    const int ur = upright_avail(ey, ex, esize, esize, c.width, sb_size_of(c)), dl = downleft_avail(ey, ex, esize, esize, c.height, sb_size_of(c));
+    if (t.rank == 0) sh->edge_avail = ur | (dl << 1);
+    stage_edges<PIX>(t, (PIX*)sh_->edge_raw, J.rec.y, J.rec.u, J.rec.v, J.rec.sy, J.rec.sc, ey, ex, esize, ur, dl, c.bitdepth);
+  }
   t.sync();
   if (TK_PROFMD_ON(4)) TK_PROFMD_ACC(ws, 21, pqs_);
   wg.barrier();
diff --git a/thor_amd/csrc/tk_block_rd.h b/thor_amd/csrc/tk_block_rd.h
--- a/thor_amd/csrc/tk_block_rd.h
+++ b/thor_amd/csrc/tk_block_rd.h
@@ -289,7 +289,7 @@
 
 template <typename PIX, int SP>
 TK_DEVNI int encode_block(const Team t, JobR<PIX> J, WsP<PIX> ws, Node& nd_, BlkParam& p, BitSink& bs,
-                          int reuse_pred = 0, PruneCtx* pc = nullptr) {
+                          int reuse_pred = 0, PruneCtx* pc = nullptr, const PIX* staged = nullptr) {
   const auto& c = J.cfg;
   const NodePos nd = node_pos(&nd_);
   const int size = nd.size, sizeC = size >> 1;
@@ -310,17 +310,32 @@
   int cbp_y = 0, cbp_u = 0, cbp_v = 0;
 
   if (TKU(p.mode) == M_INTRA) {
-    const int ur = upright_avail(nd.ypos, nd.xpos, size, size, c.width, sb_size_of(c));
-    const int dl = downleft_avail(nd.ypos, nd.xpos, size, size, c.height, sb_size_of(c));
+    staged = tk_uniform_ptr(staged);
+    int ur, dl;
+    if (staged) {
+      const int av = TKU(*ldsc(&ws->sh->edge_avail));
+      ur = av & 1; dl = (av >> 1) & 1;
+    } else {
+      ur = upright_avail(nd.ypos, nd.xpos, size, size, c.width, sb_size_of(c));
+      dl = downleft_avail(nd.ypos, nd.xpos, size, size, c.height, sb_size_of(c));
+    }
     const PIX* fy = J.rec.y + nd.ypos * J.rec.sy + nd.xpos;
     const PIX* fu = J.rec.u + yc * J.rec.sc + xc;
     const PIX* fv = J.rec.v + yc * J.rec.sc + xc;
+    const PIX* const su = staged ? staged + staged_edge_len(size) : nullptr;
+    const PIX* const sv = staged ? su + staged_edge_len(sizeC) : nullptr;
+    auto edges = [&](const PIX* st, int cb, const PIX* frame, int fstride, const PIX* rblock, int i, int j, int ypos, int xpos, int tsize, int split) {
+      TK_PROFMD_MARK(pe_);
+      if (staged) make_edges_staged<SP>(t, ws->edgep, st, cb, rblock, cb, i, j, ypos, xpos, tsize, ur, dl, split, bd);
+      else make_edges<SP>(t, ws->edgep, frame, fstride, rblock, cb, i, j, ypos, xpos, tsize, ur, dl, split, bd);
+      if (TK_PROFMD_ON(16)) TK_PROFMD_ACC(ws, 20, pe_);
+    };
     if (tb_split) {
       const int s2 = size / 2;
       int index = 0;
       for (int i = 0; i < size; i += s2)
         for (int j = 0; j < size; j += s2) {
-          make_edges<SP>(t, ws->edgep, fy, J.rec.sy, ws->rec_y + i * size + j, size, i, j, nd.ypos, nd.xpos, s2, ur, dl, 1, bd);
+          edges(staged, size, fy, J.rec.sy, ws->rec_y + i * size + j, i, j, nd.ypos, nd.xpos, s2, 1);
           pred_intra<SP>(t, ws->edgep, nd.ypos + i, nd.xpos + j, s2, ws->pred_y + i * size + j, size, p.intra_mode, bd);
           t.sync();
           int bit = code_tu_sp<PIX, SP, SP_LDS>(t, ws->xfp, oy + i * osy + j, osy, ws->pred_y + i * size + j, size,
@@ -330,7 +345,7 @@
           index += tmin(s2, 16) * tmin(s2, 16);
         }
     } else {
-      make_edges<SP>(t, ws->edgep, fy, J.rec.sy, (const PIX*)nullptr, 0, 0, 0, nd.ypos, nd.xpos, size, ur, dl, 0, bd);
+      edges(staged, size, fy, J.rec.sy, (const PIX*)nullptr, 0, 0, nd.ypos, nd.xpos, size, 0);
       pred_intra<SP>(t, ws->edgep, nd.ypos, nd.xpos, size, ws->pred_y, size, p.intra_mode, bd);
       t.sync();
       cbp_y = code_tu_sp<PIX, SP, SP_LDS>(t, ws->xfp, oy, osy, ws->pred_y, size, ws->rec_y, size, size, qpY, ftI | 0,
@@ -343,10 +358,10 @@
       int index = 0;
       for (int i = 0; i < sizeC; i += s2)
         for (int j = 0; j < sizeC; j += s2) {
-          make_edges<SP>(t, ws->edgep, fu, J.rec.sc, ws->rec_u + i * sizeC + j, sizeC, i, j, yc, xc, s2, ur, dl, 1, bd);
+          edges(su, sizeC, fu, J.rec.sc, ws->rec_u + i * sizeC + j, i, j, yc, xc, s2, 1);
           pred_intra<SP>(t, ws->edgep, yc + i, xc + j, s2, ws->pred_u + i * sizeC + j, sizeC, p.intra_mode, bd);
           t.sync();
-          make_edges<SP>(t, ws->edgep, fv, J.rec.sc, ws->rec_v + i * sizeC + j, sizeC, i, j, yc, xc, s2, ur, dl, 1, bd);
+          edges(sv, sizeC, fv, J.rec.sc, ws->rec_v + i * sizeC + j, i, j, yc, xc, s2, 1);
           pred_intra<SP>(t, ws->edgep, yc + i, xc + j, s2, ws->pred_v + i * sizeC + j, sizeC, p.intra_mode, bd);
           t.sync();
           if (c.cfl_intra)
@@ -369,10 +384,10 @@
           index += tmin(s2, 16) * tmin(s2, 16);
         }
     } else {
-      make_edges<SP>(t, ws->edgep, fu, J.rec.sc, (const PIX*)nullptr, 0, 0, 0, yc, xc, sizeC, ur, dl, 0, bd);
+      edges(su, sizeC, fu, J.rec.sc, (const PIX*)nullptr, 0, 0, yc, xc, sizeC, 0);
       pred_intra<SP>(t, ws->edgep, yc, xc, sizeC, ws->pred_u, sizeC, p.intra_mode, bd);
       t.sync();
-      make_edges<SP>(t, ws->edgep, fv, J.rec.sc, (const PIX*)nullptr, 0, 0, 0, yc, xc, sizeC, ur, dl, 0, bd);
+      edges(sv, sizeC, fv, J.rec.sc, (const PIX*)nullptr, 0, 0, yc, xc, sizeC, 0);
       pred_intra<SP>(t, ws->edgep, yc, xc, sizeC, ws->pred_v, sizeC, p.intra_mode, bd);
       t.sync();
       if (c.cfl_intra) improve_uv<PIX, SP>(t, ws, ws->pred_y, ws->pred_u, ws->pred_v, ws->rec_y, size, size, size, bd);
@@ -418,7 +433,7 @@
 template <typename PIX, int SP>
 TK_DEV unsigned rdo_trial(const Team t, JobR<PIX> J, WsP<PIX> ws, Node& nd, BlkParam& p, double lambda,
                           int reuse_pred = 0, unsigned prune_thr = 0xffffffffu, const unsigned long long* bestkey = nullptr,
-                          unsigned order = 0, int* nbits_out = nullptr, int* untouched = nullptr) {
+                          unsigned order = 0, int* nbits_out = nullptr, int* untouched = nullptr, const PIX* staged = nullptr) {
   BitSink cnt;
   cnt.buf = nullptr; cnt.pos = 0; cnt.cap = 0; cnt.emit = 0; cnt.ovf = 0;
   PruneCtx pc;
@@ -438,7 +453,7 @@
       return kCostInit;
     }
   }
-  int nbits = encode_block<PIX, SP>(t, J, ws, nd, p, cnt, reuse_pred, &pc);
+  int nbits = encode_block<PIX, SP>(t, J, ws, nd, p, cnt, reuse_pred, &pc, staged);
   if (nbits_out) *nbits_out = nbits;
   if (pc.pruned) return kCostInit;
   return rd_cost<PIX, SP>(t, J, ws, nd, nbits, lambda, pc.ssd_y);
diff --git a/thor_amd/csrc/tk_block_ws.h b/thor_amd/csrc/tk_block_ws.h
--- a/thor_amd/csrc/tk_block_ws.h
+++ b/thor_amd/csrc/tk_block_ws.h
@@ -33,6 +33,10 @@
 enum { MD_SKIP = 0, MD_MERGE, MD_REF, MD_INTRA, MD_BIPRED, MD_TRIAL, MD_BIJOINT };
 enum { WG_CMD_EXIT = 0, WG_CMD_MD = 1 };
 struct MdItem { int8_t kind, a, b, pad; };
+#ifndef TK_EDGE_STAGE_BYTES
+#define TK_EDGE_STAGE_BYTES 536
+#endif
+enum { kEdgeStageBytes = TK_EDGE_STAGE_BYTES };
 struct WgShared {
   XformTabs tabs;
   MeLists lists;
@@ -58,7 +62,10 @@
   void* wsnap[kWaves];
   MdItem items[kMdMaxItems];
   alignas(16) unsigned char org_raw[kLdsBlk * kLdsBlk * 3];
-};
+  alignas(4) unsigned char edge_raw[kEdgeStageBytes ? kEdgeStageBytes : 4];
+  int edge_avail;
+};
+template <typename PIX> TK_DEV constexpr int edges_staged(int size) { return (4 * size + 9) * (int)sizeof(PIX) <= (int)kEdgeStageBytes; }
 template <typename PIX> struct WinExtra { enum { bytes = sizeof(PIX) == 1 ? (TK_OCC == 2 ? 7680 : 944) : 5376 }; };
 template <typename PIX> struct SmallWs {
   XformWs xf;
diff --git a/thor_amd/csrc/tk_kat_block.h b/thor_amd/csrc/tk_kat_block.h
--- a/thor_amd/csrc/tk_kat_block.h
+++ b/thor_amd/csrc/tk_kat_block.h
@@ -49,6 +49,55 @@
   if (off < 0 || off % 16 || (long long)off + size * size > nsamp) return 2;
   return 0;
 }
+enum { kKatEdgePar = 4, kKatEdgeImgs = 15, kKatEdgeFill = 0xA5 };
+template <typename PIX> TK_DEV void kat_edges_dump(const Team t, const IntraEdge<PIX>* e, unsigned char* o) {
+  t.sync();
+  for (int k = t.rank; k < (int)sizeof(IntraEdge<PIX>); k += t.size) o[k] = ((const unsigned char*)e)[k];
+  t.sync();
+}
+template <typename PIX> TK_DEV void kat_edges_clear(const Team t, IntraEdge<PIX>* e) {
+  t.sync();
+  for (int k = t.rank; k < (int)sizeof(IntraEdge<PIX>); k += t.size) ((unsigned char*)e)[k] = (unsigned char)kKatEdgeFill;
+  t.sync();
+}
+template <typename PIX>
+TK_DEV void kat_edges_item(const Team t, IntraEdge<PIX>* e, PIX* staged, const Plane3<PIX>& rec, int fw, int fh, int bitdepth, const int* q, const PIX* recb,
+                           unsigned char* out) {
+  const int ypos = tk_uniform(q[0]), xpos = tk_uniform(q[1]), size = tk_uniform(q[2]), sb = tk_uniform(q[3]);
+  const int sizeC = size >> 1, yc = ypos >> 1, xc = xpos >> 1;
+  const int ur = upright_avail(ypos, xpos, size, size, fw, sb), dl = downleft_avail(ypos, xpos, size, size, fh, sb);
+  stage_edges<PIX>(t, staged, rec.y, rec.u, rec.v, rec.sy, rec.sc, ypos, xpos, size, ur, dl, bitdepth);
+  const size_t img = sizeof(IntraEdge<PIX>);
+  for (int form = 0; form < 2; form++)
+    for (int pl = 0; pl < 3; pl++) {
+      const int cb = pl ? sizeC : size, py = pl ? yc : ypos, px = pl ? xc : xpos, fs = pl ? rec.sc : rec.sy;
+      const PIX* frame = (pl == 0 ? rec.y : (pl == 1 ? rec.u : rec.v)) + py * fs + px;
+      const PIX* st = staged + (pl == 0 ? 0 : (pl == 1 ? staged_edge_len(size) : staged_edge_len(size) + staged_edge_len(sizeC)));
+      const PIX* rb = recb + (pl == 0 ? 0 : (pl == 1 ? size * size : size * size + sizeC * sizeC));
+      unsigned char* o = out + ((size_t)form * kKatEdgeImgs) * img;
+      kat_edges_clear(t, e);
+      if (form) make_edges_staged<SP_GLOBAL>(t, e, st, cb, (const PIX*)nullptr, 0, 0, 0, py, px, cb, ur, dl, 0, bitdepth);
+      else make_edges<SP_GLOBAL>(t, e, frame, fs, (const PIX*)nullptr, 0, 0, 0, py, px, cb, ur, dl, 0, bitdepth);
+      kat_edges_dump(t, e, o + (size_t)pl * img);
+      const int s2 = cb >> 1;
+      for (int tu = 0; tu < 4; tu++) {
+        const int i = (tu >> 1) * s2, j = (tu & 1) * s2;
+        kat_edges_clear(t, e);
+        if (pl == 0 || sizeC > 4) {
+          if (form) make_edges_staged<SP_GLOBAL>(t, e, st, cb, rb + i * cb + j, cb, i, j, py, px, s2, ur, dl, 1, bitdepth);
+          else make_edges<SP_GLOBAL>(t, e, frame, fs, rb + i * cb + j, cb, i, j, py, px, s2, ur, dl, 1, bitdepth);
+        }
+        kat_edges_dump(t, e, o + (size_t)(3 + 4 * pl + tu) * img);
+      }
+    }
+}
+static inline int kat_edges_check(const int* q, int fw, int fh, int sample_bytes) {
+  const int ypos = q[0], xpos = q[1], size = q[2], sb = q[3];
+  if ((sb != 64 && sb != 128) || size < 8 || size > 64 || size > sb || (size & (size - 1))) return 1;
+  if ((4 * size + 9) * sample_bytes > (int)kEdgeStageBytes) return 1;
+  if (ypos < 0 || xpos < 0 || ypos % size || xpos % size || ypos + size > fh || xpos + size > fw) return 2;
+  return 0;
+}
 enum { kKatOrg8Par = 4 };
 static inline int kat_org8_check(const int* q, long long nsamp, int sample_bytes) {
   const int size = q[0], off = q[1], skew = q[2], stride = q[3];
diff --git a/thor_amd/csrc/tk_pred.h b/thor_amd/csrc/tk_pred.h
--- a/thor_amd/csrc/tk_pred.h
+++ b/thor_amd/csrc/tk_pred.h
@@ -499,11 +499,25 @@
   PIX top_left;
 };
 
-template <int SP, typename PIX>
-TK_DEV void make_edges(const Team t, IntraEdge<PIX>* e, const PIX* rec_frame, int fstride, const PIX* rblock,
-                       int rbstride, int i, int j, int ypos, int xpos, int size, int cb_upright, int cb_downleft,
-                       int tb_split, int bitdepth) {
-  e = tk_uniform_ptr(e); rec_frame = tk_uniform_ptr(rec_frame); rblock = tk_uniform_ptr(rblock); fstride = tk_uniform(fstride);
+template <typename PIX> struct EdgeFromFrame {
+  const TK_GLOBAL PIX* f;
+  int fstride;
+};
+template <typename PIX> TK_DEV PIX edge_top(const EdgeFromFrame<PIX>& e, int x) { return e.f[x - e.fstride]; }
+template <typename PIX> TK_DEV PIX edge_left(const EdgeFromFrame<PIX>& e, int y) { return e.f[y * e.fstride - 1]; }
+TK_DEV int staged_edge_len(int cb) { return 2 * cb + 3; }
+template <typename PIX> struct EdgeFromStaged {
+  const TK_LDS PIX* s;
+  int cb;
+};
+template <typename PIX> TK_DEV PIX edge_top(const EdgeFromStaged<PIX>& e, int x) { return e.s[1 + x]; }
+template <typename PIX> TK_DEV PIX edge_left(const EdgeFromStaged<PIX>& e, int y) { return e.s[e.cb + 2 + y]; }
+
+template <int SP, typename PIX, class SRC>
+TK_DEV void make_edges_from(const Team t, IntraEdge<PIX>* e, const SRC src, const PIX* rblock,
+                            int rbstride, int i, int j, int ypos, int xpos, int size, int cb_upright, int cb_downleft,
+                            int tb_split, int bitdepth) {
+  e = tk_uniform_ptr(e); rblock = tk_uniform_ptr(rblock);
   rbstride = tk_uniform(rbstride); i = tk_uniform(i); j = tk_uniform(j); ypos = tk_uniform(ypos); xpos = tk_uniform(xpos); size = tk_uniform(size);
   cb_upright = tk_uniform(cb_upright); cb_downleft = tk_uniform(cb_downleft); tb_split = tk_uniform(tb_split); bitdepth = tk_uniform(bitdepth);
   const int len = 2 * size;
@@ -521,7 +535,6 @@
   const int top_from_block = tb_split && i != 0;
   const int left_from_block = tb_split && j != 0;
   const auto rblock_g = spc<SP>(rblock);
-  const TK_GLOBAL PIX* const frame_g = gptr(rec_frame);
   const auto e_top = ldsc(e->top);
   const auto e_left = ldsc(e->left);
   const int top_dflt = (ypos + i == 0);
@@ -531,12 +544,12 @@
     if (top_dflt) tv = dflt;
     else {
       const int kk = k < toplen ? k : toplen - 1;
-      tv = top_from_block ? rblock_g[kk - rbstride] : frame_g[kk - fstride + j];
+      tv = top_from_block ? rblock_g[kk - rbstride] : edge_top(src, kk + j);
     }
     if (left_dflt) lv = dflt;
     else {
       int kk = k < leftlen ? k : leftlen - 1;
-      lv = left_from_block ? rblock_g[kk * rbstride - 1] : frame_g[(i + kk) * fstride - 1];
+      lv = left_from_block ? rblock_g[kk * rbstride - 1] : edge_left(src, i + kk);
     }
     e_top[k] = tv;
     e_left[k] = lv;
@@ -544,13 +557,51 @@
   if (t.rank == 0) {
     PIX tl;
     if (top_dflt) {
-      tl = left_dflt ? dflt : (left_from_block ? rblock_g[-1] : frame_g[i * fstride - 1]);
+      tl = left_dflt ? dflt : (left_from_block ? rblock_g[-1] : edge_left(src, i));
     } else if (!top_from_block) {
-      tl = xpos > 0 ? frame_g[-fstride + j - 1] : frame_g[-fstride + j];
+      tl = xpos > 0 ? edge_top(src, j - 1) : edge_top(src, j);
     } else {
-      tl = xpos > 0 ? (j > 0 ? rblock_g[-rbstride - 1] : frame_g[(i - 1) * fstride - 1]) : rblock_g[-rbstride];
+      tl = xpos > 0 ? (j > 0 ? rblock_g[-rbstride - 1] : edge_left(src, i - 1)) : rblock_g[-rbstride];
     }
     *ldsc(&e->top_left) = tl;
+  }
+  t.sync();
+}
+template <int SP, typename PIX>
+TK_DEV void make_edges(const Team t, IntraEdge<PIX>* e, const PIX* rec_frame, int fstride, const PIX* rblock,
+                       int rbstride, int i, int j, int ypos, int xpos, int size, int cb_upright, int cb_downleft,
+                       int tb_split, int bitdepth) {
+  const EdgeFromFrame<PIX> src = {gptr(tk_uniform_ptr(rec_frame)), tk_uniform(fstride)};
+  make_edges_from<SP>(t, e, src, rblock, rbstride, i, j, ypos, xpos, size, cb_upright, cb_downleft, tb_split, bitdepth);
+}
+template <int SP, typename PIX>
+TK_DEV void make_edges_staged(const Team t, IntraEdge<PIX>* e, const PIX* staged, int cb, const PIX* rblock,
+                              int rbstride, int i, int j, int ypos, int xpos, int size, int cb_upright, int cb_downleft,
+                              int tb_split, int bitdepth) {
+  const EdgeFromStaged<PIX> src = {ldsc(tk_uniform_ptr(staged)), tk_uniform(cb)};
+  make_edges_from<SP>(t, e, src, rblock, rbstride, i, j, ypos, xpos, size, cb_upright, cb_downleft, tb_split, bitdepth);
+}
+template <typename PIX>
+TK_DEV void stage_edges(const Team t, PIX* staged, const PIX* rec_y, const PIX* rec_u, const PIX* rec_v, int sy, int sc, int ypos, int xpos,
+                        int size, int upright, int downleft, int bitdepth) {
+  const auto st = ldsc(tk_uniform_ptr(staged));
+  const TK_GLOBAL PIX* const fy = gptr(tk_uniform_ptr(rec_y)) + ypos * sy + xpos;
+  const TK_GLOBAL PIX* const fu = gptr(tk_uniform_ptr(rec_u)) + (ypos >> 1) * sc + (xpos >> 1);
+  const TK_GLOBAL PIX* const fv = gptr(tk_uniform_ptr(rec_v)) + (ypos >> 1) * sc + (xpos >> 1);
+  const int nY = staged_edge_len(size), nC = staged_edge_len(size >> 1);
+  const PIX dflt = (PIX)(128 << (bitdepth - 8));
+  for (int k = t.rank; k < nY + 2 * nC; k += t.size) {
+    const int pl = k < nY ? 0 : (k < nY + nC ? 1 : 2);
+    const int q = k - (pl == 0 ? 0 : (pl == 1 ? nY : nY + nC));
+    const int s = pl ? size >> 1 : size, fs = pl ? sc : sy;
+    const TK_GLOBAL PIX* const f = pl == 0 ? fy : (pl == 1 ? fu : fv);
+    int have, off;
+    if (q == 0) { have = ypos > 0 && xpos > 0; off = -fs - 1; }
+    else if (q <= s + 1) { have = ypos > 0 && (q - 1 < s || upright); off = q - 1 - fs; }
+    else { have = xpos > 0 && (q - s - 2 < s || downleft); off = (q - s - 2) * fs - 1; }
+    PIX v = dflt;
+    if (have) v = f[off];
+    st[k] = v;
   }
   t.sync();
 }
```

Measured after the change: 163.7. About the same (-0.3%).
